# ViTAE-Transformer/LeMeViT

Measured on AMD Instinct MI355X. Metric: images/sec LeMeViT-Base 224^2 bf16 fwd+bwd, higher is better.
Workload: dtype bf16; 1 GPU; lemevit_base 224x224 bf16-autocast train step (fwd+bwd+AdamW), batch 128/GPU, drop_path 0.1, random-init weights; global_batch=128, parallelism=dp1, launch=eager, weight-gradient GEMMs on a side stream

## Files before the change

### include/lemevit_hip.h

```cpp
#ifndef LEMEVIT_HIP_H
#define LEMEVIT_HIP_H

#include <stddef.h>
#include <stdint.h>

#ifdef __cplusplus
extern "C" {
#endif

#define LMV_ABI_VERSION 14

enum { LMV_F32 = 0, LMV_BF16 = 1, LMV_U8 = 2  };
enum {
  LMV_OK = 0,
  LMV_ERR_SHAPE = -1,
  LMV_ERR_DTYPE = -2,
  LMV_ERR_WORKSPACE = -3,
  LMV_ERR_LAUNCH = -4
};

int lmv_abi_version(void);
const char* lmv_last_error(void);
int lmv_config_set(const char* key, int value);
int lmv_config_get(const char* key, int* value);
// ... 5 lines not shown
  const void* w;
  const float* bias;
  const void* res;
  const float* row_scale;
  const void* aux;
  void* out;
  void* out_pre;
  float* bias_grad;
  int64_t rows;
  int32_t rows_per_sample;
  int32_t _pad;
} lmv_linear_problem;

int lmv_linear_fwd(const lmv_linear_problem* p, int nproblems, int N, int K, int act, int dtype, void* stream);
int lmv_linear_dx(const lmv_linear_problem* p, int nproblems, int N, int K, int act, int dtype, void* stream);
size_t lmv_linear_dw_workspace_bytes(const lmv_linear_problem* p, int nproblems, int N, int K, int dtype);
int lmv_linear_dw(const lmv_linear_problem* p, int nproblems, int N, int K, void* workspace, size_t workspace_bytes, int dtype, void* stream);
#define LMV_REDUCE_MAX_SEGS 12
#define LMV_REDUCE_SLABS 0
#define LMV_REDUCE_ROWS  1
typedef struct {
  const float* ws;
  float* out_w;
  float* out_b;
  int64_t slab_stride;
  int64_t nw;
  int32_t nslabs, nb;
  int32_t kind, mode;
} lmv_reduce_seg;
int lmv_linear_dw_partial(const lmv_linear_problem* p, int nproblems, int N, int K, void* workspace, size_t workspace_bytes, int dtype, void* stream,
                          lmv_reduce_seg* segs, int* nsegs);
int lmv_reduce_batch(const lmv_reduce_seg* segs, int nsegs, void* stream);

int lmv_ln_fold(const float* w, const float* bias, const float* gamma, const float* beta, int N, int K, void* wf, float* colsum, float* bf,
                int dtype, void* stream);
int lmv_ln_linear_fwd(const lmv_linear_problem* p, int nproblems, int N, int K, float eps, int act, int dtype, void* stream);
typedef struct {
  const void* x;
  void* out;
  const float* row_scale;
  int64_t rows;
  int32_t rows_per_sample;
  int32_t _pad;
} lmv_mlp_problem;
typedef struct {
  const void* w1f; const float* colsum1; const float* b1f;
  const void* w2; const float* b2;
} lmv_mlp_weights;
int lmv_mlp_fused_supported(int C, int hidden, int dtype);
int lmv_gelu_poly_eval(const float* x, float* y, int64_t n, void* stream);
int lmv_mlp_fused_fwd(const lmv_mlp_problem* p, int nproblems, const lmv_mlp_weights* w, int C, int hidden, float eps, int dtype, void* stream);
typedef struct { const void* g; const void* u; void* dn2; int64_t rows; } lmv_mlp_dx_problem;
int lmv_mlp_dx_fused_supported(int C, int hidden, int dtype);
int lmv_mlp_dx_fused(const lmv_mlp_dx_problem* p, int nproblems, const void* fc2_wt, const void* fc1_wt, int C, int hidden, int dtype, void* stream);
int lmv_attn_out_proj_residual(const lmv_linear_problem* p, int nproblems, int C, int dtype, void* stream);

typedef struct {
  const void* x;
  void* y;
  float* stats;
  const void* dy;
  const void* dres;
  void* dx;
  int64_t rows;
  const float* dx_scale;
  void* dx_scaled;
  int64_t rows_per_sample;
} lmv_ln_segment;

int lmv_layernorm_fwd(const lmv_ln_segment* seg, int nseg, const float* gamma, const float* beta, int C, float eps,
                      int dtype, void* stream);
int lmv_layernorm_gelu_fwd(const lmv_ln_segment* seg, int nseg, const float* gamma, const float* beta, int C, float eps,
                           int dtype, void* stream);
int lmv_layernorm_gelu_bwd(const lmv_ln_segment* seg, int nseg, const float* gamma, const float* beta, float* dgamma, float* dbeta, int C,
                           void* workspace, size_t workspace_bytes, int dtype, void* stream);
size_t lmv_layernorm_bwd_workspace_bytes(int64_t total_rows, int C, int dtype);
int lmv_layernorm_bwd(const lmv_ln_segment* seg, int nseg, const float* gamma, float* dgamma, float* dbeta, int C,
                      void* workspace, size_t workspace_bytes, int dtype, void* stream);
int lmv_layernorm_bwd_partial(const lmv_ln_segment* seg, int nseg, const float* gamma, int C, void* workspace, size_t workspace_bytes,
                              int* partial_rows, int dtype, void* stream);
int lmv_layernorm_bwd_reduce(const void* workspace, int partial_rows, int C, float* dgamma, float* dbeta, void* stream);
int lmv_ln_linear_exact_fwd_supported(int N, int K, int dtype);
int lmv_ln_linear_exact_fwd(const lmv_linear_problem* p, const lmv_ln_segment* seg, int nproblems, int N, int K, const float* gamma, const float* beta,
                            float eps, int dtype, void* stream);
int lmv_linear_res_ln_fwd_supported(int N, int K, int dtype);
int lmv_linear_res_ln_fwd(const lmv_linear_problem* p, const lmv_ln_segment* seg, int nproblems, int N, int K, const float* gamma, const float* beta,
                          float eps, int dtype, void* stream);
int lmv_linear_dx_ln_bwd_supported(int C, int N, int dtype);
size_t lmv_linear_dx_ln_bwd_workspace_bytes(int64_t total_rows, int C);
int lmv_linear_dx_ln_bwd(const lmv_linear_problem* p, const lmv_ln_segment* seg, int nproblems, int C, int N, const float* gamma,
                         void* workspace, size_t workspace_bytes, int* partial_rows, int dtype, void* stream);

size_t lmv_batchnorm_workspace_bytes(int C);
int lmv_batchnorm_train_fwd(const void* x, const float* gamma, const float* beta, float* running_mean, float* running_var, float momentum,
                            float eps, int act, void* y, float* stats, int64_t rows, int C, void* workspace, size_t workspace_bytes,
                            int dtype, void* stream);
int lmv_batchnorm_train_bwd(const void* dy, const void* x, const float* gamma, const float* beta, const float* stats, int act, void* dx,
                            float* dgamma, float* dbeta, int64_t rows, int C, void* workspace, size_t workspace_bytes, int dtype,
                            void* stream);
int lmv_batchnorm_apply_fwd(const void* x, const float* gamma, const float* beta, const float* stats, int act, void* y, int64_t rows, int C,
                            int dtype, void* stream);

int lmv_dwconv3x3_residual_fwd(const void* x, const float* weight, const float* bias, void* y,
                               int B, int H, int W, int C, int dtype, void* stream);
int lmv_dwconv3x3_residual_bwd_data(const void* dy, const float* weight, void* dx,
                                    int B, int H, int W, int C, int dtype, void* stream);
size_t lmv_dwconv3x3_bwd_weight_workspace_bytes(int B, int H, int W, int C, int dtype);
int lmv_dwconv3x3_bwd_weight(const void* dy, const void* x, float* dweight, float* dbias,
                             int B, int H, int W, int C, void* workspace, size_t workspace_bytes, int dtype, void* stream);
int lmv_dwconv3x3_bwd_weight_partial(const void* dy, const void* x, int B, int H, int W, int C, void* workspace, size_t workspace_bytes,
                                     int* partial_rows, int dtype, void* stream);

typedef struct {
  const void* q; const void* k; const void* v;
  void* o;
  float* lse;
  const void* d_o;
  void* dq; void* dk; void* dv;
  int64_t q_bs, q_rs, k_bs, k_rs, v_bs, v_rs, o_bs, o_rs;
  int32_t B, H, Lq, Lk;
  float scale;
  int32_t _pad;
} lmv_attn_desc;

size_t lmv_attn_workspace_bytes(int B, int H, int Lq, int Lk, int backward);
int lmv_attn_fwd(const lmv_attn_desc* d, void* workspace, size_t workspace_bytes, int dtype, void* stream);
int lmv_attn_bwd(const lmv_attn_desc* d, void* workspace, size_t workspace_bytes, int dtype, void* stream);
int lmv_attn_fwd_pair(const lmv_attn_desc* d, void* workspace, size_t workspace_bytes, int dtype, void* stream);
int lmv_attn_bwd_pair(const lmv_attn_desc* d, void* workspace, size_t workspace_bytes, int dtype, void* stream);
int lmv_attn_probs(const lmv_attn_desc* d, float* p, int head_mean, int dtype, void* stream);

int lmv_sa_core_fwd(const void* qkv, void* o, float* lse, int B, int L, int C, void* ws, size_t ws_bytes, int dtype, void* stream);
int lmv_ca_core_fwd(const void* q, const void* kv, void* o, float* lse, int B, int M, int N, int C,
                    void* ws, size_t ws_bytes, int dtype, void* stream);
int lmv_dca_core_fwd(const void* qkv1, const void* qkv2, void* ox, void* oc, float* lse_x, float* lse_c,
                     int B, int N, int M, int C, void* ws, size_t ws_bytes, int dtype, void* stream);

int lmv_cast(const void* src, int src_dtype, void* dst, int dst_dtype, int64_t n, void* stream);
int lmv_im2col3x3s2_c3(const void* x, int x_dtype, void* patches, int dtype, int B, int H, int W, int64_t sb, int64_t sc, int64_t sh,
                       int64_t sw, void* stream);
int lmv_im2col3x3s2_nchw(const void* x, int x_dtype, void* patches, int dtype, int B, int Cin, int H, int W, int KP, int64_t sb, int64_t sc, int64_t sh, int64_t sw,
                         void* stream);
int lmv_conv3x3s2_nchw_dx(const void* dy, const void* wm, void* dx, int dx_dtype, int B, int Cin, int H, int W, int Co, int KP, int64_t sb, int64_t sc, int64_t sh,
                          int64_t sw, int dtype, void* stream);
int lmv_row_scale(const void* x, const float* scale, void* y, int64_t rows, int C, int rows_per_sample, int dtype, void* stream);
typedef struct lmv_row_scale_segment {
  const void* x; const float* scale; void* y;
  int64_t rows; int rows_per_sample;
} lmv_row_scale_segment;
int lmv_row_scale_multi(const lmv_row_scale_segment* seg, int nseg, int C, int dtype, void* stream);
#define LMV_TRANSPOSE_MAX_SEGS 48
typedef struct { const void* src; void* dst; int32_t rows, cols; } lmv_transpose_seg;
int lmv_transpose_batch(const lmv_transpose_seg* segs, int nsegs, int dtype, void* stream);
int lmv_im2col3x3s2_nhwc(const void* x, void* patches, int B, int H, int W, int C, int KP, int dtype, void* stream);
int lmv_col2im3x3s2_nhwc(const void* dpatches, void* dx, int B, int H, int W, int C, int KP, int dtype, void* stream);
int lmv_conv3x3s2_fwd(const void* x, const void* wm, const float* bias, void* y, int B, int H, int W, int Cin, int Cout, int KP, int act, int dtype, void* stream);
size_t lmv_conv3x3s2_dw_workspace_bytes(int B, int H, int W, int Cin, int Cout, int KP, int dtype);
int lmv_conv3x3s2_dw(const void* dy, const void* x, float* dwm, float* dbias, int B, int H, int W, int Cin, int Cout, int KP, void* workspace, size_t workspace_bytes, int dtype,
                     void* stream);
enum { LMV_FOLD_CI_TAP = 0, LMV_FOLD_TAP_CI = 1 };
int lmv_conv_bn_fold(const float* w, const float* b, const float* gamma, const float* beta, const float* mean, const float* var, float eps, int Co, int Cin, int KP,
                     int layout, void* wm, float* bf, float* sc, int dtype, void* stream);
int lmv_conv_bn_fold_bwd(const float* dwm, const float* dbf, const float* w, const float* b, const float* gamma, const float* mean, const float* var, float eps, int Co,
                         int Cin, int KP, int layout, float* dW, float* db, float* dgamma, float* dbeta, void* stream);
int lmv_token_mean2_fwd(const void* x, int L, const void* c, int M, int C, int B, void* out, int dtype, void* stream);
int lmv_token_mean2_bwd(const void* g, void* dx, int L, void* dc, int M, int C, int B, int dtype, void* stream);
int lmv_token_mean2_affine_fwd(const void* x, int L, const void* c, int M, int C, int B, const float* xscale, const float* xshift, void* out, int dtype,
                               void* stream);
int lmv_adamw_flat(float* param, const float* grad, float* exp_avg, float* exp_avg_sq, const float* wd_mask, void* shadow_bf16,
                   int64_t n, float lr, float beta1, float beta2, float eps, float weight_decay, int step, const int* step_dev,
                   void* stream);
typedef struct { const float* ptr; int64_t n; } lmv_norm_seg;
#define LMV_GRAD_STAT_FLOATS 8
#define LMV_NORM_CHUNK 16384
enum { LMV_NORM_SKIP_NONFINITE = 1 };
size_t lmv_grad_norm_workspace_bytes(const lmv_norm_seg* segs, int nsegs);
int lmv_grad_norm(const lmv_norm_seg* segs, int nsegs, float max_norm, int flags, float* stat, int* step_dev, void* ws, size_t ws_bytes,
                  void* stream);
int lmv_adamw_flat_clip(float* param, const float* grad, float* exp_avg, float* exp_avg_sq, const float* wd_mask, void* shadow_bf16,
                        int64_t n, float lr, float beta1, float beta2, float eps, float weight_decay, int step, const int* step_dev,
                        const float* stat, float clip_value, void* stream);
#define LMV_ADAMW_UNIT 8
#define LMV_ADAMW_MAX_GROUPS 256
typedef struct { float lr; float weight_decay; } lmv_adamw_group;
int lmv_adamw_flat_groups(float* param, const float* grad, float* exp_avg, float* exp_avg_sq, void* shadow_bf16, int64_t n,
                          const uint8_t* group_of_unit, const lmv_adamw_group* groups, int ngroups, float beta1, float beta2, float eps, int step,
                          const int* step_dev, const float* stat, float clip_value, void* stream);
int lmv_ema_flat(float* ema, const float* param, int64_t n, float decay, void* stream);

typedef struct lmv_mix_record { float w; int32_t yl, yh, xl, xh; float lam_t; } lmv_mix_record;
int lmv_mix_images(const void* x, int x_dtype, int64_t sb, int64_t sc, int64_t sh, int64_t sw, void* out, int out_dtype, int B, int C, int H, int W,
                   const lmv_mix_record* table, const lmv_mix_record* host_records, const float* scale, const float* shift, void* stream);
int lmv_soft_ce(const void* logits, int dtype, int64_t row_stride, int B, int N, const int64_t* labels, const lmv_mix_record* table, float smoothing,
                const void* target, int target_dtype, int64_t target_stride, float* row_loss, float* mean_loss, void* dlogits, void* stream);

enum { LMV_BLOCK_S = 0, LMV_BLOCK_D = 1, LMV_BLOCK_C = 2 };
enum { LMV_BLOCK_NO_JOIN = 1, LMV_BLOCK_FUSED = 2, LMV_BLOCK_DATA_ONLY = 4 };
typedef struct lmv_block_desc {
  int32_t kind, dtype, B, H, W, M, C, hidden;
  float eps;
  int32_t flags;
  const float* pos_w; const float* pos_b; const float* n1_w; const float* n1_b;
  const void* attn_w[4]; const float* attn_b[4];
  const float* n2_w; const float* n2_b; const void* fc1_w; const float* fc1_b; const void* fc2_w; const float* fc2_b;
  const float* masks[4];
  float* g_pos_w; float* g_pos_b; float* g_n1_w; float* g_n1_b;
  float* g_attn_w[4]; float* g_attn_b[4];
  float* g_n2_w; float* g_n2_b; float* g_fc1_w; float* g_fc1_b; float* g_fc2_w; float* g_fc2_b;
  const void* fold_attn_w[2]; const float* fold_attn_s[2]; const float* fold_attn_b[2];
  const void* fold_fc1_w; const float* fold_fc1_s; const float* fold_fc1_b;
  const void* fc2_wt;
  const void* fc1_wt; const void* attn_wt[2];
} lmv_block_desc;
size_t lmv_block_arena_bytes(const lmv_block_desc* d);
size_t lmv_block_bwd_scratch_bytes(const lmv_block_desc* d);
int lmv_block_fwd(const lmv_block_desc* d, const void* x, const void* c, void* x_out, void* c_out, void* arena, size_t arena_bytes, int save, void* stream);
int lmv_block_fwd_range(const lmv_block_desc* d, const void* x, const void* c, void* x_out, void* c_out, void* arena, size_t arena_bytes, int save,
                        int image0, int nimages, void* stream);
int lmv_block_bwd(const lmv_block_desc* d, const void* x, const void* c, const void* arena, size_t arena_bytes, const void* dx_out, const void* dc_out,
                  void* dx, void* dc, void* scratch, size_t scratch_bytes, void* stream, void* side_stream);
size_t lmv_block_fwd_scratch_bytes(const lmv_block_desc* d);
int lmv_block_fwd_range_scratch(const lmv_block_desc* d, const void* x, const void* c, void* x_out, void* c_out, void* arena, size_t arena_bytes, int save,
                                int image0, int nimages, void* scratch, size_t scratch_bytes, void* stream);
long long lmv_debug_wgrad_launches(void);

typedef struct lmv_sstage_block_params {
  int32_t C, heads, hidden, _pad;
  const void* qkv_w; const void* proj_w; const void* fc1_w; const void* fc2_w;
  const float* n1_w; const float* n1_b; const float* qkv_b; const float* proj_b;
  const float* n2_w; const float* n2_b; const float* fc1_b; const float* fc2_b;
  const float* pos_w; const float* pos_b;
} lmv_sstage_block_params;
typedef struct lmv_sstage_desc {
  int32_t B, H, W, M, C, heads, hidden, nblocks, dtype;
  float eps;
  const void* wpk; const float* vec;
  void* timing; int32_t timing_block, kind;
} lmv_sstage_desc;
int lmv_sstage_supported(int C, int heads, int hidden, int H, int W, int M, int dtype);
size_t lmv_sstage_wpk_bytes(int C, int hidden);
size_t lmv_sstage_vec_floats(int C, int hidden);
size_t lmv_sstage_workspace_bytes(int B, int C);
int lmv_sstage_max_images(int C);
int lmv_sstage_max_concurrent(int C);
int lmv_sstage_pack(const lmv_sstage_block_params* p, void* wpk_out, float* vec_out, void* stream);
int lmv_sstage_fwd(const lmv_sstage_desc* d, const void* x, const void* c, void* x_out, void* c_out, void* workspace, size_t workspace_bytes, void* stream);

typedef struct lmv_dstage_block_params {
  int32_t C, heads, hidden, _pad;
  const void* qkv1_w; const void* qkv2_w; const void* projx_w; const void* projc_w; const void* fc1_w; const void* fc2_w;
  const float* n1_w; const float* n1_b; const float* qkv1_b; const float* qkv2_b; const float* projx_b; const float* projc_b;
  const float* n2_w; const float* n2_b; const float* fc1_b; const float* fc2_b;
  const float* pos_w; const float* pos_b;
} lmv_dstage_block_params;
typedef lmv_sstage_desc lmv_dstage_desc;
int lmv_dstage_supported(int C, int heads, int hidden, int H, int W, int M, int dtype);
size_t lmv_dstage_wpk_bytes(int C, int hidden);
size_t lmv_dstage_vec_floats(int C, int hidden);
size_t lmv_dstage_workspace_bytes(int B, int C);
int lmv_dstage_max_concurrent(int C, int H, int kind);
int lmv_dstage_pack(const lmv_dstage_block_params* p, void* wpk_out, float* vec_out, void* stream);
int lmv_dstage_fwd(const lmv_dstage_desc* d, const void* x, const void* c, void* x_out, void* c_out, void* workspace, size_t workspace_bytes, void* stream);

int lmv_stem_supported(int H, int W, int Cm, int Co, int dtype);
size_t lmv_stem_wpk_bytes(int Cm, int Co);
int lmv_stem_pack(const void* w1m, const void* w2m, int ld2, int Cm, int Co, void* wpk_out, void* stream);
int lmv_stem_fwd(const void* x, int x_dtype, int64_t sb, int64_t sc, int64_t sh, int64_t sw, int B, int H, int W, int Cm, int Co, const void* wpk, const float* b1,
                 const float* b2, void* y, void* stream);
int lmv_stage_error_count(int reset);
int lmv_debug_stage_error_set(int value);

int lmv_debug_launch_timing(int capacity);
int lmv_debug_launch_timing_read(float* ms, double* flops, double* bytes, int* kinds, int capacity);
void lmv_stem_debug_timing(void* buf);

#ifdef __cplusplus
}
#endif
#endif
```

### lemevit_amd/_lib.py

```python
from __future__ import annotations

import ctypes as C
import os

import torch

_HERE = os.path.dirname(os.path.abspath(__file__))
LIB_PATH = os.environ.get("LMV_LIB_PATH") or os.path.join(_HERE, "csrc", "liblemevit_hip.so")

LMV_F32, LMV_BF16, LMV_U8 = 0, 1, 2
ACT_NONE, ACT_GELU, ACT_GELU_GRAD, ACT_GELU_BWD = 0, 1, 2, 3
FOLD_CI_TAP, FOLD_TAP_CI = 0, 1
ABI_VERSION = 14
BLOCK_NO_JOIN, BLOCK_FUSED, BLOCK_DATA_ONLY = 1, 2, 4
GRAD_STAT_FLOATS, NORM_CHUNK, NORM_SKIP_NONFINITE = 8, 16384, 1
ADAMW_UNIT, ADAMW_MAX_GROUPS = 8, 256


class LinearProblem(C.Structure):
    _fields_ = [("a", C.c_void_p), ("w", C.c_void_p), ("bias", C.c_void_p), ("res", C.c_void_p),
                ("row_scale", C.c_void_p), ("aux", C.c_void_p), ("out", C.c_void_p), ("out_pre", C.c_void_p),
                ("bias_grad", C.c_void_p), ("rows", C.c_int64), ("rows_per_sample", C.c_int32), ("_pad", C.c_int32)]


class MlpProblem(C.Structure):
    _fields_ = [("x", C.c_void_p), ("out", C.c_void_p), ("row_scale", C.c_void_p), ("rows", C.c_int64), ("rows_per_sample", C.c_int32), ("_pad", C.c_int32)]


class MlpDxProblem(C.Structure):
    _fields_ = [("g", C.c_void_p), ("u", C.c_void_p), ("dn2", C.c_void_p), ("rows", C.c_int64)]


class MlpWeights(C.Structure):
    _fields_ = [("w1f", C.c_void_p), ("colsum1", C.c_void_p), ("b1f", C.c_void_p), ("w2", C.c_void_p), ("b2", C.c_void_p)]


class ReduceSeg(C.Structure):
    _fields_ = [("ws", C.c_void_p), ("out_w", C.c_void_p), ("out_b", C.c_void_p), ("slab_stride", C.c_int64), ("nw", C.c_int64),
                ("nslabs", C.c_int32), ("nb", C.c_int32), ("kind", C.c_int32), ("mode", C.c_int32)]


class LnSegment(C.Structure):
    _fields_ = [("x", C.c_void_p), ("y", C.c_void_p), ("stats", C.c_void_p), ("dy", C.c_void_p), ("dres", C.c_void_p),
                ("dx", C.c_void_p), ("rows", C.c_int64), ("dx_scale", C.c_void_p), ("dx_scaled", C.c_void_p), ("rows_per_sample", C.c_int64)]


class RowScaleSegment(C.Structure):
    _fields_ = [("x", C.c_void_p), ("scale", C.c_void_p), ("y", C.c_void_p), ("rows", C.c_int64), ("rows_per_sample", C.c_int)]


class AttnDesc(C.Structure):
    _fields_ = [("q", C.c_void_p), ("k", C.c_void_p), ("v", C.c_void_p), ("o", C.c_void_p), ("lse", C.c_void_p),
                ("d_o", C.c_void_p), ("dq", C.c_void_p), ("dk", C.c_void_p), ("dv", C.c_void_p),
                ("q_bs", C.c_int64), ("q_rs", C.c_int64), ("k_bs", C.c_int64), ("k_rs", C.c_int64),
                ("v_bs", C.c_int64), ("v_rs", C.c_int64), ("o_bs", C.c_int64), ("o_rs", C.c_int64),
                ("B", C.c_int32), ("H", C.c_int32), ("Lq", C.c_int32), ("Lk", C.c_int32),
                ("scale", C.c_float), ("_pad", C.c_int32)]


class BlockDesc(C.Structure):
    _fields_ = ([(n, C.c_int32) for n in ("kind", "dtype", "B", "H", "W", "M", "C", "hidden")] + [("eps", C.c_float), ("flags", C.c_int32)] +
                [(n, C.c_void_p) for n in ("pos_w", "pos_b", "n1_w", "n1_b")] + [("attn_w", C.c_void_p * 4), ("attn_b", C.c_void_p * 4)] +
                [(n, C.c_void_p) for n in ("n2_w", "n2_b", "fc1_w", "fc1_b", "fc2_w", "fc2_b")] + [("masks", C.c_void_p * 4)] +
                [(n, C.c_void_p) for n in ("g_pos_w", "g_pos_b", "g_n1_w", "g_n1_b")] + [("g_attn_w", C.c_void_p * 4), ("g_attn_b", C.c_void_p * 4)] +
                [(n, C.c_void_p) for n in ("g_n2_w", "g_n2_b", "g_fc1_w", "g_fc1_b", "g_fc2_w", "g_fc2_b")] +
                [("fold_attn_w", C.c_void_p * 2), ("fold_attn_s", C.c_void_p * 2), ("fold_attn_b", C.c_void_p * 2)] +
                [(n, C.c_void_p) for n in ("fold_fc1_w", "fold_fc1_s", "fold_fc1_b", "fc2_wt", "fc1_wt")] + [("attn_wt", C.c_void_p * 2)])


class SStageBlockParams(C.Structure):
    _fields_ = ([(n, C.c_int32) for n in ("C", "heads", "hidden", "_pad")] +
                [(n, C.c_void_p) for n in ("qkv_w", "proj_w", "fc1_w", "fc2_w", "n1_w", "n1_b", "qkv_b", "proj_b", "n2_w", "n2_b", "fc1_b", "fc2_b", "pos_w", "pos_b")])


class SStageDesc(C.Structure):
    _fields_ = ([(n, C.c_int32) for n in ("B", "H", "W", "M", "C", "heads", "hidden", "nblocks", "dtype")] + [("eps", C.c_float), ("wpk", C.c_void_p), ("vec", C.c_void_p), ("timing", C.c_void_p), ("timing_block", C.c_int32), ("kind", C.c_int32)])


class DStageBlockParams(C.Structure):
    _fields_ = ([(n, C.c_int32) for n in ("C", "heads", "hidden", "_pad")] +
                [(n, C.c_void_p) for n in ("qkv1_w", "qkv2_w", "projx_w", "projc_w", "fc1_w", "fc2_w", "n1_w", "n1_b", "qkv1_b", "qkv2_b", "projx_b", "projc_b",
                                           "n2_w", "n2_b", "fc1_b", "fc2_b", "pos_w", "pos_b")])


class TransposeSeg(C.Structure):
    _fields_ = [("src", C.c_void_p), ("dst", C.c_void_p), ("rows", C.c_int32), ("cols", C.c_int32)]


class NormSeg(C.Structure):
    _fields_ = [("ptr", C.c_void_p), ("n", C.c_int64)]


class AdamWGroup(C.Structure):
    _fields_ = [("lr", C.c_float), ("weight_decay", C.c_float)]


class MixRecord(C.Structure):
    _fields_ = [("w", C.c_float), ("yl", C.c_int32), ("yh", C.c_int32), ("xl", C.c_int32), ("xh", C.c_int32), ("lam_t", C.c_float)]


_P, _I, _L, _F, _Z = C.c_void_p, C.c_int, C.c_int64, C.c_float, C.c_size_t

SIGNATURES = {
    "lmv_abi_version": (_I, []),
    "lmv_config_set": (_I, [C.c_char_p, _I]),
    "lmv_config_get": (_I, [C.c_char_p, C.POINTER(C.c_int)]),
    "lmv_last_error": (C.c_char_p, []),
    "lmv_linear_fwd": (_I, [C.POINTER(LinearProblem), _I, _I, _I, _I, _I, _P]),
    "lmv_linear_dx": (_I, [C.POINTER(LinearProblem), _I, _I, _I, _I, _I, _P]),
    "lmv_linear_dw_workspace_bytes": (_Z, [C.POINTER(LinearProblem), _I, _I, _I, _I]),
    "lmv_linear_dw": (_I, [C.POINTER(LinearProblem), _I, _I, _I, _P, _Z, _I, _P]),
    "lmv_linear_dw_partial": (_I, [C.POINTER(LinearProblem), _I, _I, _I, _P, _Z, _I, _P, C.POINTER(ReduceSeg), C.POINTER(C.c_int)]),
    "lmv_reduce_batch": (_I, [C.POINTER(ReduceSeg), _I, _P]),
    "lmv_ln_fold": (_I, [_P, _P, _P, _P, _I, _I, _P, _P, _P, _I, _P]),
    "lmv_ln_linear_fwd": (_I, [C.POINTER(LinearProblem), _I, _I, _I, _F, _I, _I, _P]),
    "lmv_mlp_fused_supported": (_I, [_I, _I, _I]),
    "lmv_gelu_poly_eval": (_I, [_P, _P, C.c_int64, _P]),
    "lmv_mlp_fused_fwd": (_I, [C.POINTER(MlpProblem), _I, C.POINTER(MlpWeights), _I, _I, _F, _I, _P]),
    "lmv_mlp_dx_fused_supported": (_I, [_I, _I, _I]),
    "lmv_mlp_dx_fused": (_I, [C.POINTER(MlpDxProblem), _I, _P, _P, _I, _I, _I, _P]),
    "lmv_attn_out_proj_residual": (_I, [C.POINTER(LinearProblem), _I, _I, _I, _P]),
    "lmv_layernorm_fwd": (_I, [C.POINTER(LnSegment), _I, _P, _P, _I, _F, _I, _P]),
    "lmv_layernorm_gelu_fwd": (_I, [C.POINTER(LnSegment), _I, _P, _P, _I, _F, _I, _P]),
    "lmv_layernorm_gelu_bwd": (_I, [C.POINTER(LnSegment), _I, _P, _P, _P, _P, _I, _P, _Z, _I, _P]),
    "lmv_layernorm_bwd_workspace_bytes": (_Z, [_L, _I, _I]),
    "lmv_layernorm_bwd": (_I, [C.POINTER(LnSegment), _I, _P, _P, _P, _I, _P, _Z, _I, _P]),
    "lmv_layernorm_bwd_partial": (_I, [C.POINTER(LnSegment), _I, _P, _I, _P, _Z, C.POINTER(C.c_int), _I, _P]),
    "lmv_layernorm_bwd_reduce": (_I, [_P, _I, _I, _P, _P, _P]),
    "lmv_ln_linear_exact_fwd_supported": (_I, [_I, _I, _I]),
    "lmv_ln_linear_exact_fwd": (_I, [C.POINTER(LinearProblem), C.POINTER(LnSegment), _I, _I, _I, _P, _P, _F, _I, _P]),
    "lmv_linear_res_ln_fwd_supported": (_I, [_I, _I, _I]),
    "lmv_linear_res_ln_fwd": (_I, [C.POINTER(LinearProblem), C.POINTER(LnSegment), _I, _I, _I, _P, _P, _F, _I, _P]),
    "lmv_linear_dx_ln_bwd_supported": (_I, [_I, _I, _I]),
    "lmv_linear_dx_ln_bwd_workspace_bytes": (_Z, [_L, _I]),
    "lmv_linear_dx_ln_bwd": (_I, [C.POINTER(LinearProblem), C.POINTER(LnSegment), _I, _I, _I, _P, _P, _Z, C.POINTER(C.c_int), _I, _P]),
    "lmv_batchnorm_workspace_bytes": (_Z, [_I]),
    "lmv_batchnorm_train_fwd": (_I, [_P, _P, _P, _P, _P, _F, _F, _I, _P, _P, _L, _I, _P, _Z, _I, _P]),
    "lmv_batchnorm_train_bwd": (_I, [_P, _P, _P, _P, _P, _I, _P, _P, _P, _L, _I, _P, _Z, _I, _P]),
    "lmv_batchnorm_apply_fwd": (_I, [_P, _P, _P, _P, _I, _P, _L, _I, _I, _P]),
    "lmv_dwconv3x3_residual_fwd": (_I, [_P, _P, _P, _P, _I, _I, _I, _I, _I, _P]),
    "lmv_dwconv3x3_residual_bwd_data": (_I, [_P, _P, _P, _I, _I, _I, _I, _I, _P]),
    "lmv_dwconv3x3_bwd_weight_workspace_bytes": (_Z, [_I, _I, _I, _I, _I]),
    "lmv_dwconv3x3_bwd_weight": (_I, [_P, _P, _P, _P, _I, _I, _I, _I, _P, _Z, _I, _P]),
    "lmv_dwconv3x3_bwd_weight_partial": (_I, [_P, _P, _I, _I, _I, _I, _P, _Z, C.POINTER(C.c_int), _I, _P]),
    "lmv_attn_workspace_bytes": (_Z, [_I, _I, _I, _I, _I]),
    "lmv_attn_fwd": (_I, [C.POINTER(AttnDesc), _P, _Z, _I, _P]),
    "lmv_attn_bwd": (_I, [C.POINTER(AttnDesc), _P, _Z, _I, _P]),
    "lmv_attn_fwd_pair": (_I, [C.POINTER(AttnDesc), _P, _Z, _I, _P]),
    "lmv_attn_bwd_pair": (_I, [C.POINTER(AttnDesc), _P, _Z, _I, _P]),
    "lmv_attn_probs": (_I, [C.POINTER(AttnDesc), _P, _I, _I, _P]),
    "lmv_sa_core_fwd": (_I, [_P, _P, _P, _I, _I, _I, _P, _Z, _I, _P]),
    "lmv_ca_core_fwd": (_I, [_P, _P, _P, _P, _I, _I, _I, _I, _P, _Z, _I, _P]),
    "lmv_dca_core_fwd": (_I, [_P, _P, _P, _P, _P, _P, _I, _I, _I, _I, _P, _Z, _I, _P]),
    "lmv_cast": (_I, [_P, _I, _P, _I, _L, _P]),
    "lmv_im2col3x3s2_c3": (_I, [_P, _I, _P, _I, _I, _I, _I, _L, _L, _L, _L, _P]),
    "lmv_im2col3x3s2_nchw": (_I, [_P, _I, _P, _I, _I, _I, _I, _I, _I, _L, _L, _L, _L, _P]),
    "lmv_conv3x3s2_nchw_dx": (_I, [_P, _P, _P, _I, _I, _I, _I, _I, _I, _I, _L, _L, _L, _L, _I, _P]),
    "lmv_row_scale_multi": (_I, [_P, _I, _I, _I, _P]),
    "lmv_transpose_batch": (_I, [C.POINTER(TransposeSeg), _I, _I, _P]),
    "lmv_row_scale": (_I, [_P, _P, _P, _L, _I, _I, _I, _P]),
    "lmv_im2col3x3s2_nhwc": (_I, [_P, _P, _I, _I, _I, _I, _I, _I, _P]),
    "lmv_conv3x3s2_fwd": (_I, [_P, _P, _P, _P, _I, _I, _I, _I, _I, _I, _I, _I, _P]),
    "lmv_conv3x3s2_dw_workspace_bytes": (_Z, [_I, _I, _I, _I, _I, _I, _I]),
    "lmv_conv3x3s2_dw": (_I, [_P, _P, _P, _P, _I, _I, _I, _I, _I, _I, _P, _Z, _I, _P]),
    "lmv_conv_bn_fold": (_I, [_P, _P, _P, _P, _P, _P, _F, _I, _I, _I, _I, _P, _P, _P, _I, _P]),
    "lmv_conv_bn_fold_bwd": (_I, [_P, _P, _P, _P, _P, _P, _P, _F, _I, _I, _I, _I, _P, _P, _P, _P, _P]),
    "lmv_col2im3x3s2_nhwc": (_I, [_P, _P, _I, _I, _I, _I, _I, _I, _P]),
    "lmv_token_mean2_fwd": (_I, [_P, _I, _P, _I, _I, _I, _P, _I, _P]),
    "lmv_token_mean2_affine_fwd": (_I, [_P, _I, _P, _I, _I, _I, _P, _P, _P, _I, _P]),
    "lmv_token_mean2_bwd": (_I, [_P, _P, _I, _P, _I, _I, _I, _I, _P]),
    "lmv_adamw_flat": (_I, [_P, _P, _P, _P, _P, _P, _L, _F, _F, _F, _F, _F, _I, _P, _P]),
    "lmv_grad_norm_workspace_bytes": (_Z, [C.POINTER(NormSeg), _I]),
    "lmv_grad_norm": (_I, [C.POINTER(NormSeg), _I, _F, _I, _P, _P, _P, _Z, _P]),
    "lmv_adamw_flat_clip": (_I, [_P, _P, _P, _P, _P, _P, _L, _F, _F, _F, _F, _F, _I, _P, _P, _F, _P]),
    "lmv_adamw_flat_groups": (_I, [_P, _P, _P, _P, _P, _L, _P, _P, _I, _F, _F, _F, _I, _P, _P, _F, _P]),
    "lmv_ema_flat": (_I, [_P, _P, _L, _F, _P]),
    "lmv_mix_images": (_I, [_P, _I, _L, _L, _L, _L, _P, _I, _I, _I, _I, _I, _P, _P, _P, _P, _P]),
    "lmv_soft_ce": (_I, [_P, _I, _L, _I, _I, _P, _P, _F, _P, _I, _L, _P, _P, _P, _P]),
    "lmv_block_arena_bytes": (_Z, [C.POINTER(BlockDesc)]),
    "lmv_block_bwd_scratch_bytes": (_Z, [C.POINTER(BlockDesc)]),
    "lmv_block_fwd": (_I, [C.POINTER(BlockDesc), _P, _P, _P, _P, _P, _Z, _I, _P]),
    "lmv_block_fwd_range": (_I, [C.POINTER(BlockDesc), _P, _P, _P, _P, _P, _Z, _I, _I, _I, _P]),
    "lmv_block_bwd": (_I, [C.POINTER(BlockDesc), _P, _P, _P, _Z, _P, _P, _P, _P, _P, _Z, _P, _P]),
    "lmv_block_fwd_scratch_bytes": (_Z, [C.POINTER(BlockDesc)]),
    "lmv_block_fwd_range_scratch": (_I, [C.POINTER(BlockDesc), _P, _P, _P, _P, _P, _Z, _I, _I, _I, _P, _Z, _P]),
    "lmv_debug_wgrad_launches": (C.c_longlong, []),
    "lmv_sstage_supported": (_I, [_I, _I, _I, _I, _I, _I, _I]),
    "lmv_sstage_wpk_bytes": (_Z, [_I, _I]),
    "lmv_sstage_vec_floats": (_Z, [_I, _I]),
    "lmv_sstage_workspace_bytes": (_Z, [_I, _I]),
    "lmv_sstage_max_images": (_I, [_I]),
    "lmv_sstage_max_concurrent": (_I, [_I]),
    "lmv_sstage_pack": (_I, [C.POINTER(SStageBlockParams), _P, _P, _P]),
    "lmv_sstage_fwd": (_I, [C.POINTER(SStageDesc), _P, _P, _P, _P, _P, _Z, _P]),
    "lmv_stem_supported": (_I, [_I, _I, _I, _I, _I]),
    "lmv_stem_wpk_bytes": (_Z, [_I, _I]),
    "lmv_stem_pack": (_I, [_P, _P, _I, _I, _I, _P, _P]),
    "lmv_stem_fwd": (_I, [_P, _I, _L, _L, _L, _L, _I, _I, _I, _I, _I, _P, _P, _P, _P, _P]),
    "lmv_stem_debug_timing": (None, [_P]),
    "lmv_stage_error_count": (_I, [_I]),
    "lmv_debug_stage_error_set": (_I, [_I]),
    "lmv_debug_launch_timing": (_I, [_I]),
    "lmv_debug_launch_timing_read": (_I, [_P, _P, _P, _P, _I]),
    "lmv_dstage_supported": (_I, [_I, _I, _I, _I, _I, _I, _I]),
    "lmv_dstage_wpk_bytes": (_Z, [_I, _I]),
    "lmv_dstage_vec_floats": (_Z, [_I, _I]),
    "lmv_dstage_workspace_bytes": (_Z, [_I, _I]),
    "lmv_dstage_max_concurrent": (_I, [_I, _I, _I]),
    "lmv_dstage_pack": (_I, [C.POINTER(DStageBlockParams), _P, _P, _P]),
    "lmv_dstage_fwd": (_I, [C.POINTER(SStageDesc), _P, _P, _P, _P, _P, _Z, _P]),
}


def _load():
    if not os.path.exists(LIB_PATH):
        raise RuntimeError(
            f"lemevit_amd: HIP kernel library not found at {LIB_PATH}. There is no CPU/PyTorch fallback; "
            "build it with `make -C lemevit_amd/csrc` (hipcc, --offload-arch=gfx950).")
    try:
        lib = C.CDLL(LIB_PATH)
    except OSError as e:
        raise RuntimeError(f"lemevit_amd: cannot load {LIB_PATH}: {e}") from e
    for name, (res, args) in SIGNATURES.items():
        fn = getattr(lib, name)
        fn.restype = res
        fn.argtypes = args
    v = lib.lmv_abi_version()
    if v != ABI_VERSION:
        raise RuntimeError(f"lemevit_amd: ABI version mismatch (library {v}, binding {ABI_VERSION}); rebuild csrc")
    return lib


lib = _load()


def config_set(key: str, value: int) -> None:
    if lib.lmv_config_set(key.encode(), int(value)):
        raise RuntimeError(f"lmv_config_set: {lib.lmv_last_error().decode(errors='replace')}")


def config_get(key: str) -> int:
    v = C.c_int(0)
    if lib.lmv_config_get(key.encode(), C.byref(v)):
        raise RuntimeError(f"lmv_config_get: {lib.lmv_last_error().decode(errors='replace')}")
    return int(v.value)


def check(rc: int, what: str) -> None:
    if rc != 0:
        raise RuntimeError(f"{what} failed (code {rc}): {lib.lmv_last_error().decode(errors='replace')}")
```

### lemevit_amd/csrc/block.hip

```cpp
#include <math.h>
#include <mutex>
#include "common.h"

namespace {

struct Bump {
  unsigned char* base; size_t off, cap;
  void* take(size_t n) {
    const size_t a = (off + 255) & ~(size_t)255;
    off = a + n;
    return base ? (void*)(base + a) : (void*)(uintptr_t)256;
  }
};

struct Dims {
  int kind, dtype, B, H, W, N, M, C, Hd, heads;
  size_t es;
  int64_t rows[2];
};

int dims_of(const lmv_block_desc* d, Dims* o) {
  if (!d) LMV_FAIL(LMV_ERR_SHAPE, "block: null descriptor");
  if (d->kind < LMV_BLOCK_S || d->kind > LMV_BLOCK_C) LMV_FAIL(LMV_ERR_SHAPE, "block: kind %d (0 = S, 1 = D, 2 = C)", d->kind);
  if (d->dtype != LMV_F32 && d->dtype != LMV_BF16) LMV_FAIL(LMV_ERR_DTYPE, "block: unsupported dtype %d", d->dtype);
  if (d->B <= 0 || d->H <= 0 || d->W <= 0 || d->M <= 0 || d->C <= 0 || (d->C % 32)) LMV_FAIL(LMV_ERR_SHAPE, "block: bad dims B=%d H=%d W=%d M=%d C=%d", d->B, d->H, d->W, d->M, d->C);
  o->kind = d->kind; o->dtype = d->dtype; o->B = d->B; o->H = d->H; o->W = d->W; o->N = d->H * d->W; o->M = d->M; o->C = d->C;
  o->Hd = d->hidden > 0 ? d->hidden : 4 * d->C; o->heads = d->C / 32;
  o->es = d->dtype == LMV_BF16 ? 2 : 4;
  o->rows[0] = (int64_t)d->B * o->N; o->rows[1] = (int64_t)d->B * d->M;
  return LMV_OK;
}

inline int proj_w(const Dims& D, int s) { return D.kind == LMV_BLOCK_C ? (s == 0 ? 2 * D.C : D.C) : 3 * D.C; }

struct Fwd {
  void *xp, *n1[2], *pj[2], *ao[2], *t2[2], *n2[2], *u[2], *h[2], *ws;
  float *st1[2], *lse[2], *st2[2];
  size_t ws_bytes;
};

inline size_t fwd_ws_attn(const Dims& D, int b) {
  size_t w, w2 = 0;
  if (D.kind == LMV_BLOCK_C) w = lmv_attn_workspace_bytes(b, D.heads, D.M, D.N, 0);
  else if (D.kind == LMV_BLOCK_D) { w = lmv_attn_workspace_bytes(b, D.heads, D.N, D.M, 0); w2 = lmv_attn_workspace_bytes(b, D.heads, D.M, D.N, 0); }
  else { w = lmv_attn_workspace_bytes(b, D.heads, D.N, D.N, 0); w2 = lmv_attn_workspace_bytes(b, D.heads, D.M, D.M, 0); }
  if (w2 > w) w = w2;
  return w < 256 ? 256 : w;
}
inline size_t fwd_ws_off(const Dims& D, int i0) { return i0 <= 0 ? 0 : fwd_ws_attn(D, i0) + (size_t)512 * i0; }
inline size_t fwd_ws_bytes(const Dims& D, int b) { return fwd_ws_attn(D, b) + (size_t)512 * b + 256; }

inline bool data_only(const lmv_block_desc* d) { return (d->flags & LMV_BLOCK_DATA_ONLY) != 0; }

void layout_transient(const Dims& D, Bump& t, Fwd* f) {
  const bool cb = D.kind == LMV_BLOCK_C;
  for (int s = 0; s < 2; ++s) {
    const bool has = !(cb && s == 0);
    f->n1[s] = t.take(D.rows[s] * D.C * D.es);
    f->n2[s] = has ? t.take(D.rows[s] * D.C * D.es) : nullptr;
    f->h[s] = has ? t.take(D.rows[s] * D.Hd * D.es) : nullptr;
  }
}

void layout_fwd(const Dims& D, Bump& a, Fwd* f, bool dataonly = false, Bump* tr = nullptr) {
  const bool cb = D.kind == LMV_BLOCK_C;
  if (dataonly) {
    for (int s = 0; s < 2; ++s) f->n1[s] = f->n2[s] = f->h[s] = nullptr;
    if (tr) layout_transient(D, *tr, f);
    f->xp = a.take(D.rows[0] * D.C * D.es);
    for (int s = 0; s < 2; ++s) {
      f->st1[s] = (float*)a.take(D.rows[s] * 2 * sizeof(float));
      f->pj[s] = a.take(D.rows[s] * proj_w(D, s) * D.es);
      const bool has = !(cb && s == 0);
      f->ao[s] = has ? a.take(D.rows[s] * D.C * D.es) : nullptr;
      f->lse[s] = has ? (float*)a.take((size_t)D.B * D.heads * (s == 0 ? D.N : D.M) * sizeof(float)) : nullptr;
      f->t2[s] = has ? a.take(D.rows[s] * D.C * D.es) : nullptr;
      f->st2[s] = has ? (float*)a.take(D.rows[s] * 2 * sizeof(float)) : nullptr;
      f->u[s] = has ? a.take(D.rows[s] * D.Hd * D.es) : nullptr;
    }
    f->ws_bytes = fwd_ws_bytes(D, D.B);
    f->ws = a.take(f->ws_bytes);
    return;
  }
  f->xp = a.take(D.rows[0] * D.C * D.es);
  for (int s = 0; s < 2; ++s) {
    f->n1[s] = a.take(D.rows[s] * D.C * D.es);
    f->st1[s] = (float*)a.take(D.rows[s] * 2 * sizeof(float));
    f->pj[s] = a.take(D.rows[s] * proj_w(D, s) * D.es);
    const bool has = !(cb && s == 0);
    f->ao[s] = has ? a.take(D.rows[s] * D.C * D.es) : nullptr;
    f->lse[s] = has ? (float*)a.take((size_t)D.B * D.heads * (s == 0 ? D.N : D.M) * sizeof(float)) : nullptr;
    f->t2[s] = has ? a.take(D.rows[s] * D.C * D.es) : nullptr;
    f->n2[s] = has ? a.take(D.rows[s] * D.C * D.es) : nullptr;
    f->st2[s] = has ? (float*)a.take(D.rows[s] * 2 * sizeof(float)) : nullptr;
    f->u[s] = has ? a.take(D.rows[s] * D.Hd * D.es) : nullptr;
    f->h[s] = has ? a.take(D.rows[s] * D.Hd * D.es) : nullptr;
  }
  f->ws_bytes = fwd_ws_bytes(D, D.B);
  f->ws = a.take(f->ws_bytes);
}

void attn_desc(lmv_attn_desc* a, const Dims& D, const void* q, int qw, int qo, const void* k, int kw, int ko, const void* v, int vw, int vo,
               void* o, float* lse, int Lq, int Lk, float scale) {
  *a = lmv_attn_desc{};
  a->q = (const unsigned char*)q + qo * D.es; a->k = (const unsigned char*)k + ko * D.es; a->v = (const unsigned char*)v + vo * D.es;
  a->o = o; a->lse = lse;
  a->q_bs = (int64_t)Lq * qw; a->q_rs = qw; a->k_bs = (int64_t)Lk * kw; a->k_rs = kw; a->v_bs = (int64_t)Lk * vw; a->v_rs = vw;
  a->o_bs = (int64_t)Lq * D.C; a->o_rs = D.C;
  a->B = D.B; a->H = D.heads; a->Lq = Lq; a->Lk = Lk; a->scale = scale;
}
void attn_grads(lmv_attn_desc* a, const Dims& D, const void* d_o, void* dq, int qo, void* dk, int ko, void* dv, int vo) {
  a->d_o = d_o;
  a->dq = (unsigned char*)dq + qo * D.es; a->dk = (unsigned char*)dk + ko * D.es; a->dv = (unsigned char*)dv + vo * D.es;
}

lmv_linear_problem prob(const void* a, const void* w, void* out, int64_t rows) {
  lmv_linear_problem p{};
  p.a = a; p.w = w; p.out = out; p.rows = rows;
  return p;
}

#define LMV_TRY(expr) do { const int rc__ = (expr); if (rc__) return rc__; } while (0)

const float SDPA_SCALE = 0.17677669529663687f;
inline void dca_scales(const Dims& D, float* sx, float* sc) {
  const double base = pow((double)D.C, -0.5);
  *sx = (float)(log((double)D.M) / log((double)D.N) * base);
  *sc = (float)base;
}

inline bool fused_on(const lmv_block_desc* d, const Dims& D, int save) {
  return (d->flags & LMV_BLOCK_FUSED) && !save && D.dtype == LMV_BF16 && d->fold_fc1_w && d->fold_fc1_s && d->fold_fc1_b && d->fold_attn_w[0] && d->fold_attn_s[0] &&
         d->fold_attn_b[0] && (D.kind == LMV_BLOCK_S || (d->fold_attn_w[1] && d->fold_attn_s[1] && d->fold_attn_b[1]));
}
inline bool fold_qkv(const Dims& D) { return D.C >= 192; }

inline bool mlp_split384(const Dims& D) { const int64_t r = D.rows[0] + D.rows[1]; return D.C == 384 && D.Hd == 1536 && r >= 16384 && r <= 65536; }
inline bool res_ln_ok(const lmv_block_desc* d, const Dims& D, int save) {
  if (D.kind != LMV_BLOCK_S || D.dtype != LMV_BF16 || D.rows[0] + D.rows[1] < 16384 || D.rows[0] + D.rows[1] > 32768) return false;
  if (!lmv_linear_res_ln_fwd_supported(D.C, D.C, D.dtype)) return false;
  return !(fused_on(d, D, save) && !mlp_split384(D));
}

int mlp_fwd(const lmv_block_desc* d, const Dims& D, const Fwd& f, int s0, void* const* outs, const float* const* ds, int save, void* st, bool ln_done = false) {
  const int ns = 2 - s0;
  const bool split384 = mlp_split384(D);
  if (fused_on(d, D, save) && !split384) {
    if (lmv_mlp_fused_supported(D.C, D.Hd, D.dtype)) {
      lmv_mlp_problem q[2] = {};
      for (int i = 0; i < ns; ++i) { const int s = s0 + i; q[i].x = f.t2[s]; q[i].out = outs[s]; q[i].row_scale = ds[s]; q[i].rows = D.rows[s]; q[i].rows_per_sample = s == 0 ? D.N : D.M; }
      lmv_mlp_weights w{d->fold_fc1_w, d->fold_fc1_s, d->fold_fc1_b, d->fc2_w, d->fc2_b};
      return lmv_mlp_fused_fwd(q, ns, &w, D.C, D.Hd, d->eps, D.dtype, st);
    }
    lmv_linear_problem p[2];
    for (int i = 0; i < ns; ++i) { const int s = s0 + i; p[i] = prob(f.t2[s], d->fold_fc1_w, f.h[s], D.rows[s]); p[i].bias = d->fold_fc1_b; p[i].aux = d->fold_fc1_s; }
    LMV_TRY(lmv_ln_linear_fwd(p, ns, D.Hd, D.C, d->eps, LMV_ACT_GELU, D.dtype, st));
    for (int i = 0; i < ns; ++i) {
      const int s = s0 + i;
      p[i] = prob(f.h[s], d->fc2_w, outs[s], D.rows[s]); p[i].bias = d->fc2_b; p[i].res = f.t2[s]; p[i].row_scale = ds[s];
      p[i].rows_per_sample = s == 0 ? D.N : D.M;
    }
    return lmv_linear_fwd(p, ns, D.C, D.Hd, LMV_ACT_NONE, D.dtype, st);
  }
  if (!ln_done) {
    lmv_ln_segment seg[2] = {};
    for (int i = 0; i < ns; ++i) { const int s = s0 + i; seg[i].x = f.t2[s]; seg[i].y = f.n2[s]; seg[i].stats = save ? f.st2[s] : nullptr; seg[i].rows = D.rows[s]; }
    LMV_TRY(lmv_layernorm_fwd(seg, ns, d->n2_w, d->n2_b, D.C, d->eps, D.dtype, st));
  }
  lmv_linear_problem p[2];
  for (int i = 0; i < ns; ++i) { const int s = s0 + i; p[i] = prob(f.n2[s], d->fc1_w, f.h[s], D.rows[s]); p[i].bias = d->fc1_b; p[i].out_pre = save ? f.u[s] : nullptr; }
  LMV_TRY(lmv_linear_fwd(p, ns, D.Hd, D.C, LMV_ACT_GELU, D.dtype, st));
  for (int i = 0; i < ns; ++i) {
    const int s = s0 + i;
    p[i] = prob(f.h[s], d->fc2_w, outs[s], D.rows[s]); p[i].bias = d->fc2_b; p[i].res = f.t2[s]; p[i].row_scale = ds[s];
    p[i].rows_per_sample = s == 0 ? D.N : D.M;
  }
  return lmv_linear_fwd(p, ns, D.C, D.Hd, LMV_ACT_NONE, D.dtype, st);
}

struct Side {
  hipStream_t main, side; hipEvent_t fork, join; bool used;
  void* ws; size_t ws_bytes;
  void* ws_tail; size_t ws_tail_bytes;
  lmv_reduce_seg segs[LMV_REDUCE_MAX_SEGS]; int nsegs = 0;
  bool dataonly = false;
  hipStream_t begin() {
    if (!side) return main;
    lmv_count_wgrad();
    (void)hipEventRecord(fork, main);
    (void)hipStreamWaitEvent(side, fork, 0);
    used = true;
    return side;
  }
  void finish() {
    if (side && used) { (void)hipEventRecord(join, side); (void)hipStreamWaitEvent(main, join, 0); used = false; }
  }
};

struct EventPool {
  std::mutex mu;
  hipEvent_t free_ev[64][32];
  int nfree[64] = {};
  int take(hipEvent_t* fork, hipEvent_t* join) {
    int dev = 0;
    (void)hipGetDevice(&dev);
    dev &= 63;
    hipEvent_t out[2];
    int got = 0;
    {
      std::lock_guard<std::mutex> lk(mu);
      while (got < 2 && nfree[dev] > 0) out[got++] = free_ev[dev][--nfree[dev]];
    }
    for (; got < 2; ++got)
      if (hipEventCreateWithFlags(&out[got], hipEventDisableTiming) != hipSuccess) {
        give(dev, out, got);
        LMV_FAIL(LMV_ERR_LAUNCH, "block_bwd: cannot create stream events");
      }
    *fork = out[0]; *join = out[1];
    return LMV_OK;
  }
  void give(int dev, const hipEvent_t* ev, int n) {
    std::lock_guard<std::mutex> lk(mu);
    for (int i = 0; i < n; ++i) {
      if (nfree[dev] < 32) free_ev[dev][nfree[dev]++] = ev[i];
      else (void)hipEventDestroy(ev[i]);
    }
  }
  void give(hipEvent_t fork, hipEvent_t join) {
    int dev = 0;
    (void)hipGetDevice(&dev);
    const hipEvent_t ev[2] = {fork, join};
    give(dev & 63, ev, 2);
  }
};
EventPool& event_pool() { static EventPool p; return p; }

int dw(Side& sd, const lmv_linear_problem* p, int np, int N, int K, int dtype) {
  lmv_count_wgrad();
  const size_t need = lmv_linear_dw_workspace_bytes(p, np, N, K, dtype);
  if (need > sd.ws_bytes) LMV_FAIL(LMV_ERR_WORKSPACE, "block_bwd: weight-gradient workspace %zu > %zu bytes", need, sd.ws_bytes);
  return lmv_linear_dw(p, np, N, K, sd.ws, sd.ws_bytes, dtype, sd.begin());
}
int flush_reduces(Side& sd) {
  if (!sd.nsegs) return LMV_OK;
  lmv_count_wgrad();
  const int rc = lmv_reduce_batch(sd.segs, sd.nsegs, sd.begin());
  sd.nsegs = 0;
  return rc;
}

struct Bwd {
  void *g[2], *du[2], *dn2[2], *dt2[2], *g2[2], *dao[2], *dpj[2], *dn1[2], *dxp, *ws_main, *ws_side, *ws_conv, *ws_ln[2];
  size_t ws_main_bytes, ws_side_bytes, ws_conv_bytes, ws_ln_bytes;
};

size_t max_dw_ws(const Dims& D) {
  const void* fake = (const void*)(uintptr_t)256;
  size_t m = 256;
  auto one = [&](int np, int64_t r0, int64_t r1, int N, int K, bool shared) {
    lmv_linear_problem p[2];
    float* o0 = (float*)(uintptr_t)256; float* o1 = shared ? o0 : (float*)(uintptr_t)512;
    p[0] = prob(fake, fake, o0, r0); p[0].bias_grad = (float*)(uintptr_t)1024;
    p[1] = prob(fake, fake, o1, r1); p[1].bias_grad = shared ? p[0].bias_grad : (float*)(uintptr_t)2048;
    const size_t w = lmv_linear_dw_workspace_bytes(p, np, N, K, D.dtype);
    if (w > m) m = w;
  };
  const int C = D.C, Hd = D.Hd;
  if (D.kind == LMV_BLOCK_C) {
    one(1, D.rows[1], 0, C, Hd, true); one(1, D.rows[1], 0, Hd, C, true);
    one(1, D.rows[1], 0, C, C, true); one(1, D.rows[1], 0, C, C, true); one(1, D.rows[0], 0, 2 * C, C, true);
  } else {
    const bool sh = D.kind == LMV_BLOCK_S;
    one(2, D.rows[0], D.rows[1], C, Hd, true); one(2, D.rows[0], D.rows[1], Hd, C, true);
    one(2, D.rows[0], D.rows[1], C, C, sh); one(2, D.rows[0], D.rows[1], 3 * C, C, sh);
  }
  return (m + 255) & ~(size_t)255;
}

void layout_bwd(const Dims& D, Bump& a, Bwd* b) {
  const bool cb = D.kind == LMV_BLOCK_C;
  for (int s = 0; s < 2; ++s) {
    const bool has = !(cb && s == 0);
    b->g[s] = has ? a.take(D.rows[s] * D.C * D.es) : nullptr;
    b->du[s] = has ? a.take(D.rows[s] * D.Hd * D.es) : nullptr;
    b->dn2[s] = has ? a.take(D.rows[s] * D.C * D.es) : nullptr;
    b->dt2[s] = has ? a.take(D.rows[s] * D.C * D.es) : nullptr;
    b->g2[s] = has ? a.take(D.rows[s] * D.C * D.es) : nullptr;
    b->dao[s] = has ? a.take(D.rows[s] * D.C * D.es) : nullptr;
    b->dpj[s] = a.take(D.rows[s] * proj_w(D, s) * D.es);
    b->dn1[s] = a.take(D.rows[s] * D.C * D.es);
  }
  b->dxp = a.take(D.rows[0] * D.C * D.es);
  size_t w = lmv_layernorm_bwd_workspace_bytes(D.rows[0] + D.rows[1], D.C, D.dtype);
  size_t w2;
  if (cb) w2 = lmv_attn_workspace_bytes(D.B, D.heads, D.M, D.N, 1);
  else if (D.kind == LMV_BLOCK_D) { w2 = lmv_attn_workspace_bytes(D.B, D.heads, D.N, D.M, 1); const size_t w3 = lmv_attn_workspace_bytes(D.B, D.heads, D.M, D.N, 1); if (w3 > w2) w2 = w3; }
  else { w2 = lmv_attn_workspace_bytes(D.B, D.heads, D.N, D.N, 1); const size_t w3 = lmv_attn_workspace_bytes(D.B, D.heads, D.M, D.M, 1); if (w3 > w2) w2 = w3; }
  if (w2 > w) w = w2;
  if (w < 256) w = 256;
  b->ws_main_bytes = w; b->ws_main = a.take(w);
  b->ws_side_bytes = max_dw_ws(D); b->ws_side = a.take(b->ws_side_bytes);
  b->ws_conv_bytes = lmv_dwconv3x3_bwd_weight_workspace_bytes(D.B, D.H, D.W, D.C, D.dtype); b->ws_conv = a.take(b->ws_conv_bytes);
  b->ws_ln_bytes = lmv_layernorm_bwd_workspace_bytes(D.rows[0] + D.rows[1], D.C, D.dtype);
  { const size_t w2 = lmv_linear_dx_ln_bwd_workspace_bytes(D.rows[0] + D.rows[1], D.C); if (w2 > b->ws_ln_bytes) b->ws_ln_bytes = w2; }
  for (int i = 0; i < 2; ++i) b->ws_ln[i] = a.take(b->ws_ln_bytes);
}

int ln_bwd(Side& sd, const lmv_ln_segment* seg, int nseg, const float* gamma, float* dgamma, float* dbeta, const Dims& D, void* ws, size_t ws_bytes) {
  if (sd.dataonly) return lmv_layernorm_bwd_partial(seg, nseg, gamma, D.C, nullptr, 0, nullptr, D.dtype, sd.main);
  int rows = 0;
  LMV_TRY(lmv_layernorm_bwd_partial(seg, nseg, gamma, D.C, ws, ws_bytes, &rows, D.dtype, sd.main));
  if (sd.nsegs + 1 > LMV_REDUCE_MAX_SEGS) LMV_FAIL(LMV_ERR_WORKSPACE, "block_bwd: too many deferred reductions");
  lmv_reduce_seg& sg = sd.segs[sd.nsegs++];
  sg = lmv_reduce_seg{};
  sg.ws = (const float*)ws; sg.out_w = dgamma; sg.out_b = dbeta; sg.slab_stride = 2 * D.C; sg.nw = D.C; sg.nslabs = rows; sg.nb = D.C;
  sg.kind = LMV_REDUCE_ROWS; sg.mode = 0;
  return LMV_OK;
}

inline bool dx_ln_fused_ok(const Dims& D, const void* wt, int N) {
  const int64_t rows = D.rows[0] + D.rows[1];
  return wt && D.dtype == LMV_BF16 && lmv_linear_dx_ln_bwd_supported(D.C, N, D.dtype) && rows >= 16384 && rows <= 32768;
}
int dx_ln_bwd(Side& sd, const lmv_linear_problem* p, const lmv_ln_segment* seg, int nseg, int N, const float* gamma, float* dgamma, float* dbeta, const Dims& D,
              void* ws, size_t ws_bytes) {
  if (sd.dataonly) return lmv_linear_dx_ln_bwd(p, seg, nseg, D.C, N, gamma, nullptr, 0, nullptr, D.dtype, sd.main);
  int rows = 0;
  LMV_TRY(lmv_linear_dx_ln_bwd(p, seg, nseg, D.C, N, gamma, ws, ws_bytes, &rows, D.dtype, sd.main));
  if (sd.nsegs + 1 > LMV_REDUCE_MAX_SEGS) LMV_FAIL(LMV_ERR_WORKSPACE, "block_bwd: too many deferred reductions");
  lmv_reduce_seg& sg = sd.segs[sd.nsegs++];
  sg = lmv_reduce_seg{};
  sg.ws = (const float*)ws; sg.out_w = dgamma; sg.out_b = dbeta; sg.slab_stride = 2 * D.C; sg.nw = D.C; sg.nslabs = rows; sg.nb = D.C;
  sg.kind = LMV_REDUCE_ROWS; sg.mode = 0;
  return LMV_OK;
}

inline bool mlp_dx_fused_on(const lmv_block_desc* d, const Dims& D) {
  const int mode = lmv_config().mlp_dx_fused;
  if (mode == 0 || D.dtype != LMV_BF16 || !d->fc2_wt || !d->fc1_wt || !lmv_mlp_dx_fused_supported(D.C, D.Hd, D.dtype)) return false;
  return mode == 2;
}

int mlp_bwd(const lmv_block_desc* d, const Dims& D, const Fwd& f, const Bwd& b, int s0, const void* const* douts, const float* const* ds, const float* const* nds,
            const void** g2_out, Side& sd) {
  const int ns = 2 - s0;
  hipStream_t st = sd.main;
  const void* g[2];
  lmv_row_scale_segment rs[2]; int nrs = 0;
  for (int s = s0; s < 2; ++s) {
    g[s] = douts[s];
    if (ds[s]) { rs[nrs].x = douts[s]; rs[nrs].scale = ds[s]; rs[nrs].y = b.g[s]; rs[nrs].rows = D.rows[s]; rs[nrs].rows_per_sample = s == 0 ? D.N : D.M; ++nrs; g[s] = b.g[s]; }
  }
  if (nrs) LMV_TRY(lmv_row_scale_multi(rs, nrs, D.C, D.dtype, st));
  lmv_linear_problem p[2];
  lmv_ln_segment seg[2] = {};
  for (int i = 0; i < ns; ++i) {
    const int s = s0 + i;
    seg[i].x = f.t2[s]; seg[i].dy = b.dn2[s]; seg[i].stats = f.st2[s]; seg[i].dres = douts[s]; seg[i].dx = b.dt2[s]; seg[i].rows = D.rows[s];
    g2_out[s] = b.dt2[s];
    if (nds && nds[s]) { seg[i].dx_scale = nds[s]; seg[i].dx_scaled = b.g2[s]; seg[i].rows_per_sample = s == 0 ? D.N : D.M; g2_out[s] = b.g2[s]; }
  }
  if (sd.dataonly && mlp_dx_fused_on(d, D)) {
    lmv_mlp_dx_problem q[2] = {};
    for (int i = 0; i < ns; ++i) { const int s = s0 + i; q[i].g = g[s]; q[i].u = f.u[s]; q[i].dn2 = b.dn2[s]; q[i].rows = D.rows[s]; }
    LMV_TRY(lmv_mlp_dx_fused(q, ns, d->fc2_wt, d->fc1_wt, D.C, D.Hd, D.dtype, st));
    return ln_bwd(sd, seg, ns, d->n2_w, d->g_n2_w, d->g_n2_b, D, b.ws_ln[0], b.ws_ln_bytes);
  }
  if (!sd.dataonly) {
    for (int i = 0; i < ns; ++i) { const int s = s0 + i; p[i] = prob(g[s], f.h[s], d->g_fc2_w, D.rows[s]); p[i].bias_grad = d->g_fc2_b; }
    LMV_TRY(dw(sd, p, ns, D.C, D.Hd, D.dtype));
  }
  if (d->fc2_wt && D.dtype == LMV_BF16) {
    for (int i = 0; i < ns; ++i) { const int s = s0 + i; p[i] = prob(g[s], d->fc2_wt, b.du[s], D.rows[s]); p[i].aux = f.u[s]; }
    LMV_TRY(lmv_linear_fwd(p, ns, D.Hd, D.C, LMV_ACT_GELU_GRAD, D.dtype, st));
  } else {
    for (int i = 0; i < ns; ++i) { const int s = s0 + i; p[i] = prob(g[s], d->fc2_w, b.du[s], D.rows[s]); p[i].aux = f.u[s]; }
    LMV_TRY(lmv_linear_dx(p, ns, D.C, D.Hd, LMV_ACT_GELU_GRAD, D.dtype, st));
  }
  if (!sd.dataonly) {
    for (int i = 0; i < ns; ++i) { const int s = s0 + i; p[i] = prob(b.du[s], f.n2[s], d->g_fc1_w, D.rows[s]); p[i].bias_grad = d->g_fc1_b; }
    LMV_TRY(dw(sd, p, ns, D.Hd, D.C, D.dtype));
  }
  const bool fuse2 = dx_ln_fused_ok(D, d->fc1_wt, D.Hd);
  if (fuse2) {
  } else if (d->fc1_wt && D.dtype == LMV_BF16) {
    for (int i = 0; i < ns; ++i) { const int s = s0 + i; p[i] = prob(b.du[s], d->fc1_wt, b.dn2[s], D.rows[s]); }
    LMV_TRY(lmv_linear_fwd(p, ns, D.C, D.Hd, LMV_ACT_NONE, D.dtype, st));
  } else {
// ... 49 lines not shown
  Bwd b;
  layout_bwd(D, a, &b);
  return a.off + 256;
}

namespace {
int block_fwd_body(const lmv_block_desc* d, const Dims& D, const Fwd& f, const void* x, const void* c, void* x_out, void* c_out, int save, void* stream);
}

extern "C" int lmv_block_fwd_range(const lmv_block_desc* d, const void* x, const void* c, void* x_out, void* c_out, void* arena, size_t arena_bytes, int save,
                                   int image0, int nimages, void* stream) {
  return lmv_block_fwd_range_scratch(d, x, c, x_out, c_out, arena, arena_bytes, save, image0, nimages, nullptr, 0, stream);
}

extern "C" int lmv_block_fwd_range_scratch(const lmv_block_desc* d, const void* x, const void* c, void* x_out, void* c_out, void* arena, size_t arena_bytes, int save,
                                           int image0, int nimages, void* scratch, size_t scratch_bytes, void* stream) {
  Dims DF;
  LMV_TRY(dims_of(d, &DF));
  LMV_TRY(check_ptrs(d, false));
  const bool cb = DF.kind == LMV_BLOCK_C;
  if (!x || !c || !c_out || (!cb && !x_out) || !arena || !lmv_aligned16(arena)) LMV_FAIL(LMV_ERR_SHAPE, "block_fwd: null / misaligned tensor");
  if (image0 < 0 || nimages <= 0 || image0 + nimages > DF.B) LMV_FAIL(LMV_ERR_SHAPE, "block_fwd: images [%d, %d) outside the batch of %d", image0, image0 + nimages, DF.B);
  const bool dataonly = data_only(d);
  if (dataonly && (!scratch || !lmv_aligned16(scratch))) LMV_FAIL(LMV_ERR_SHAPE, "block_fwd: LMV_BLOCK_DATA_ONLY needs the transient buffer of lmv_block_fwd_range_scratch");
  Bump a{(unsigned char*)arena, 0, arena_bytes};
  Bump t{(unsigned char*)scratch, 0, scratch_bytes};
  Fwd f;
  layout_fwd(DF, a, &f, dataonly, &t);
  if (a.off > arena_bytes) LMV_FAIL(LMV_ERR_WORKSPACE, "block_fwd: arena %zu < %zu bytes", arena_bytes, a.off);
  if (dataonly && t.off > scratch_bytes) LMV_FAIL(LMV_ERR_WORKSPACE, "block_fwd: transient buffer %zu < %zu bytes", scratch_bytes, t.off);
  if (image0 == 0 && nimages == DF.B) return block_fwd_body(d, DF, f, x, c, x_out, c_out, save, stream);
  lmv_block_desc dr = *d;
  dr.B = nimages;
  for (int k = 0; k < 4; ++k) if (dr.masks[k]) dr.masks[k] += image0;
  Dims D;
  LMV_TRY(dims_of(&dr, &D));
  const size_t es = D.es;
  auto adv = [&](void* ptr, int s, size_t width_bytes) -> void* { return ptr ? (void*)((unsigned char*)ptr + (size_t)image0 * (s == 0 ? D.N : D.M) * width_bytes) : nullptr; };
  f.xp = adv(f.xp, 0, D.C * es);
  for (int s = 0; s < 2; ++s) {
    f.n1[s] = adv(f.n1[s], s, D.C * es); f.st1[s] = (float*)adv(f.st1[s], s, 2 * sizeof(float)); f.pj[s] = adv(f.pj[s], s, proj_w(D, s) * es);
    f.ao[s] = adv(f.ao[s], s, D.C * es); f.lse[s] = (float*)adv(f.lse[s], s, D.heads * sizeof(float)); f.t2[s] = adv(f.t2[s], s, D.C * es);
    f.n2[s] = adv(f.n2[s], s, D.C * es); f.st2[s] = (float*)adv(f.st2[s], s, 2 * sizeof(float)); f.u[s] = adv(f.u[s], s, D.Hd * es); f.h[s] = adv(f.h[s], s, D.Hd * es);
  }
  const size_t w0 = fwd_ws_off(DF, image0), w1 = fwd_ws_attn(DF, nimages);
  if (w0 + w1 > f.ws_bytes) LMV_FAIL(LMV_ERR_WORKSPACE, "block_fwd: attention workspace slice [%zu, %zu) outside %zu bytes", w0, w0 + w1, f.ws_bytes);
  f.ws = (unsigned char*)f.ws + w0; f.ws_bytes = w1;
  return block_fwd_body(&dr, D, f, adv(const_cast<void*>(x), 0, D.C * es), adv(const_cast<void*>(c), 1, D.C * es), adv(x_out, 0, D.C * es), adv(c_out, 1, D.C * es), save, stream);
}

extern "C" int lmv_block_fwd(const lmv_block_desc* d, const void* x, const void* c, void* x_out, void* c_out, void* arena, size_t arena_bytes, int save, void* stream) {
  return lmv_block_fwd_range(d, x, c, x_out, c_out, arena, arena_bytes, save, 0, d ? d->B : 0, stream);
}

namespace {

int block_fwd_body(const lmv_block_desc* d, const Dims& D, const Fwd& f, const void* x, const void* c, void* x_out, void* c_out, int save, void* stream) {
  const bool cb = D.kind == LMV_BLOCK_C;
  const int C = D.C, N = D.N, M = D.M;
  LMV_TRY(lmv_dwconv3x3_residual_fwd(x, d->pos_w, d->pos_b, f.xp, D.B, D.H, D.W, C, D.dtype, stream));
  const bool fq = fused_on(d, D, save) && fold_qkv(D);
  const bool ex = !fq && D.dtype == LMV_BF16 && D.kind != LMV_BLOCK_S &&
                  lmv_ln_linear_exact_fwd_supported(cb ? 2 * D.C : 3 * D.C, D.C, D.dtype) && lmv_ln_linear_exact_fwd_supported(D.C, D.C, D.dtype);
  const void* src[2] = {f.xp, c};
  if (!fq && !ex) {
    lmv_ln_segment seg[2] = {};
    seg[0].x = f.xp; seg[0].y = f.n1[0]; seg[0].stats = save ? f.st1[0] : nullptr; seg[0].rows = D.rows[0];
    seg[1].x = c; seg[1].y = f.n1[1]; seg[1].stats = save ? f.st1[1] : nullptr; seg[1].rows = D.rows[1];
    LMV_TRY(lmv_layernorm_fwd(seg, 2, d->n1_w, d->n1_b, C, d->eps, D.dtype, stream));
    src[0] = f.n1[0]; src[1] = f.n1[1];
  }
  auto project = [&](lmv_linear_problem* p, int np, const int* streams, const int* slots, int width) -> int {
    for (int i = 0; i < np; ++i) {
      const int s = streams[i], k = slots[i];
      p[i] = prob(src[s], fq ? d->fold_attn_w[k] : d->attn_w[k], f.pj[s], D.rows[s]);
      p[i].bias = fq ? d->fold_attn_b[k] : d->attn_b[k];
      if (fq) p[i].aux = d->fold_attn_s[k];
    }
    if (ex) {
      lmv_ln_segment seg[2] = {};
      for (int i = 0; i < np; ++i) { const int s = streams[i]; seg[i].y = save ? f.n1[s] : nullptr; seg[i].stats = save ? f.st1[s] : nullptr; seg[i].rows = D.rows[s]; }
      return lmv_ln_linear_exact_fwd(p, seg, np, width, C, d->n1_w, d->n1_b, d->eps, D.dtype, stream);
    }
    return fq ? lmv_ln_linear_fwd(p, np, width, C, d->eps, LMV_ACT_NONE, D.dtype, stream) : lmv_linear_fwd(p, np, width, C, LMV_ACT_NONE, D.dtype, stream);
  };
  lmv_linear_problem p[2];
  lmv_attn_desc ad[2];
  void* outs[2] = {x_out, c_out};
  bool ln2_done = false;
  if (D.kind == LMV_BLOCK_S) {
    { const int st_[2] = {0, 1}, sl_[2] = {0, 0}; LMV_TRY(project(p, 2, st_, sl_, 3 * C)); }
    for (int s = 0; s < 2; ++s) { const int L = s == 0 ? N : M; attn_desc(&ad[s], D, f.pj[s], 3 * C, 0, f.pj[s], 3 * C, C, f.pj[s], 3 * C, 2 * C, f.ao[s], save ? f.lse[s] : nullptr, L, L, SDPA_SCALE); }
    LMV_TRY(lmv_attn_fwd_pair(ad, f.ws, f.ws_bytes, D.dtype, stream));
    for (int s = 0; s < 2; ++s) {
      p[s] = prob(f.ao[s], d->attn_w[1], f.t2[s], D.rows[s]); p[s].bias = d->attn_b[1]; p[s].res = s == 0 ? f.xp : c;
      p[s].row_scale = d->masks[s == 0 ? 0 : 2]; p[s].rows_per_sample = s == 0 ? N : M;
    }
    if (res_ln_ok(d, D, save)) {
      lmv_ln_segment seg[2] = {};
      for (int s = 0; s < 2; ++s) { seg[s].y = f.n2[s]; seg[s].stats = save ? f.st2[s] : nullptr; seg[s].rows = D.rows[s]; }
      LMV_TRY(lmv_linear_res_ln_fwd(p, seg, 2, C, C, d->n2_w, d->n2_b, d->eps, D.dtype, stream));
      ln2_done = true;
    } else {
      LMV_TRY(lmv_linear_fwd(p, 2, C, C, LMV_ACT_NONE, D.dtype, stream));
    }
  } else if (D.kind == LMV_BLOCK_D) {
    float sx, sc;
    dca_scales(D, &sx, &sc);
    { const int st_[2] = {0, 1}, sl_[2] = {0, 1}; LMV_TRY(project(p, 2, st_, sl_, 3 * C)); }
    attn_desc(&ad[0], D, f.pj[0], 3 * C, 0, f.pj[1], 3 * C, C, f.pj[1], 3 * C, 2 * C, f.ao[0], save ? f.lse[0] : nullptr, N, M, sx);
    attn_desc(&ad[1], D, f.pj[1], 3 * C, 0, f.pj[0], 3 * C, C, f.pj[0], 3 * C, 2 * C, f.ao[1], save ? f.lse[1] : nullptr, M, N, sc);
    LMV_TRY(lmv_attn_fwd(&ad[0], f.ws, f.ws_bytes, D.dtype, stream));
    LMV_TRY(lmv_attn_fwd(&ad[1], f.ws, f.ws_bytes, D.dtype, stream));
    for (int s = 0; s < 2; ++s) {
      p[s] = prob(f.ao[s], d->attn_w[2 + s], f.t2[s], D.rows[s]); p[s].bias = d->attn_b[2 + s]; p[s].res = s == 0 ? f.xp : c;
      p[s].row_scale = d->masks[s == 0 ? 0 : 2]; p[s].rows_per_sample = s == 0 ? N : M;
    }
    LMV_TRY(lmv_linear_fwd(p, 2, C, C, LMV_ACT_NONE, D.dtype, stream));
  } else {
    { const int st_[1] = {0}, sl_[1] = {1}; LMV_TRY(project(p, 1, st_, sl_, 2 * C)); }
    { const int st_[1] = {1}, sl_[1] = {0}; LMV_TRY(project(p, 1, st_, sl_, C)); }
    attn_desc(&ad[0], D, f.pj[1], C, 0, f.pj[0], 2 * C, 0, f.pj[0], 2 * C, C, f.ao[1], save ? f.lse[1] : nullptr, M, N, SDPA_SCALE);
    LMV_TRY(lmv_attn_fwd(&ad[0], f.ws, f.ws_bytes, D.dtype, stream));
    p[0] = prob(f.ao[1], d->attn_w[2], f.t2[1], D.rows[1]); p[0].bias = d->attn_b[2]; p[0].res = c; p[0].row_scale = d->masks[0]; p[0].rows_per_sample = M;
    LMV_TRY(lmv_linear_fwd(p, 1, C, C, LMV_ACT_NONE, D.dtype, stream));
  }
  const float* ds[2] = {cb ? nullptr : d->masks[1], cb ? d->masks[1] : d->masks[3]};
  return mlp_fwd(d, D, f, cb ? 1 : 0, outs, ds, save, stream, ln2_done);
}

}

extern "C" int lmv_block_bwd(const lmv_block_desc* d, const void* x, const void* c, const void* arena, size_t arena_bytes, const void* dx_out, const void* dc_out, void* dx, void* dc,
                             void* scratch, size_t scratch_bytes, void* stream, void* side_stream) {
  Dims D;
  LMV_TRY(dims_of(d, &D));
  const bool dataonly = data_only(d);
  LMV_TRY(check_ptrs(d, !dataonly));
  const bool cb = D.kind == LMV_BLOCK_C;
  if (dataonly) side_stream = nullptr;
  if ((!x && !dataonly) || !c || !arena || !dc_out || (!cb && !dx_out) || !dx || !dc || !scratch || !lmv_aligned16(scratch)) LMV_FAIL(LMV_ERR_SHAPE, "block_bwd: null / misaligned tensor");
  Bump a{(unsigned char*)const_cast<void*>(arena), 0, arena_bytes};
  Fwd f;
  layout_fwd(D, a, &f, dataonly);
  if (a.off > arena_bytes) LMV_FAIL(LMV_ERR_WORKSPACE, "block_bwd: arena %zu < %zu bytes", arena_bytes, a.off);
  Bump s{(unsigned char*)scratch, 0, scratch_bytes};
  Bwd b;
  layout_bwd(D, s, &b);
  if (s.off > scratch_bytes) LMV_FAIL(LMV_ERR_WORKSPACE, "block_bwd: scratch %zu < %zu bytes", scratch_bytes, s.off);
  Side sd{};
  sd.main = (hipStream_t)stream; sd.side = (hipStream_t)side_stream; sd.ws = b.ws_side; sd.ws_bytes = b.ws_side_bytes;
  sd.ws_tail = b.ws_conv; sd.ws_tail_bytes = b.ws_conv_bytes;
  sd.dataonly = dataonly;
  if (side_stream) LMV_TRY(event_pool().take(&sd.fork, &sd.join));
  hipStream_t st = sd.main;
  const int C = D.C, N = D.N, M = D.M;
  lmv_linear_problem p[2];
  lmv_attn_desc ad[2];
  const void* g2[2] = {nullptr, nullptr};
  int rc = LMV_OK;
  auto body = [&]() -> int {
    if (cb) {
      const void* douts[2] = {nullptr, dc_out};
      const float* ds[2] = {nullptr, d->masks[1]};
      LMV_TRY(mlp_bwd(d, D, f, b, 1, douts, ds, nullptr, g2, sd));
      const void* dc1 = b.dt2[1];
      const void* g = dc1;
      if (d->masks[0]) { LMV_TRY(lmv_row_scale(dc1, d->masks[0], b.g2[1], D.rows[1], C, M, D.dtype, st)); g = b.g2[1]; }
      if (!dataonly) {
        p[0] = prob(g, f.ao[1], d->g_attn_w[2], D.rows[1]); p[0].bias_grad = d->g_attn_b[2];
        LMV_TRY(dw(sd, p, 1, C, C, D.dtype));
      }
      p[0] = prob(g, d->attn_w[2], b.dao[1], D.rows[1]);
      LMV_TRY(lmv_linear_dx(p, 1, C, C, LMV_ACT_NONE, D.dtype, st));
      attn_desc(&ad[0], D, f.pj[1], C, 0, f.pj[0], 2 * C, 0, f.pj[0], 2 * C, C, f.ao[1], f.lse[1], M, N, SDPA_SCALE);
      attn_grads(&ad[0], D, b.dao[1], b.dpj[1], 0, b.dpj[0], 0, b.dpj[0], C);
      LMV_TRY(lmv_attn_bwd(&ad[0], b.ws_main, b.ws_main_bytes, D.dtype, st));
      if (!dataonly) {
        p[0] = prob(b.dpj[1], f.n1[1], d->g_attn_w[0], D.rows[1]); p[0].bias_grad = d->g_attn_b[0];
        LMV_TRY(dw(sd, p, 1, C, C, D.dtype));
        p[0] = prob(b.dpj[0], f.n1[0], d->g_attn_w[1], D.rows[0]); p[0].bias_grad = d->g_attn_b[1];
        LMV_TRY(dw(sd, p, 1, 2 * C, C, D.dtype));
      }
      p[0] = prob(b.dpj[1], d->attn_w[0], b.dn1[1], D.rows[1]);
      LMV_TRY(lmv_linear_dx(p, 1, C, C, LMV_ACT_NONE, D.dtype, st));
      p[0] = prob(b.dpj[0], d->attn_w[1], b.dn1[0], D.rows[0]);
      LMV_TRY(lmv_linear_dx(p, 1, 2 * C, C, LMV_ACT_NONE, D.dtype, st));
      lmv_ln_segment seg[2] = {};
      seg[0].x = c; seg[0].dy = b.dn1[1]; seg[0].stats = f.st1[1]; seg[0].dres = dc1; seg[0].dx = dc; seg[0].rows = D.rows[1];
      seg[1].x = f.xp; seg[1].dy = b.dn1[0]; seg[1].stats = f.st1[0]; seg[1].dres = nullptr; seg[1].dx = b.dxp; seg[1].rows = D.rows[0];
      LMV_TRY(ln_bwd(sd, seg, 2, d->n1_w, d->g_n1_w, d->g_n1_b, D, b.ws_ln[1], b.ws_ln_bytes));
    } else {
      const void* douts[2] = {dx_out, dc_out};
      const float* ds[2] = {d->masks[1], d->masks[3]};
      const float* nds[2] = {d->masks[0], d->masks[2]};
      LMV_TRY(mlp_bwd(d, D, f, b, 0, douts, ds, nds, g2, sd));
      const bool sh = D.kind == LMV_BLOCK_S;
      if (!dataonly) {
        for (int s2 = 0; s2 < 2; ++s2) { p[s2] = prob(g2[s2], f.ao[s2], sh ? d->g_attn_w[1] : d->g_attn_w[2 + s2], D.rows[s2]); p[s2].bias_grad = sh ? d->g_attn_b[1] : d->g_attn_b[2 + s2]; }
        LMV_TRY(dw(sd, p, 2, C, C, D.dtype));
      }
      if (sh && d->attn_wt[1] && D.dtype == LMV_BF16) {
        for (int s2 = 0; s2 < 2; ++s2) p[s2] = prob(g2[s2], d->attn_wt[1], b.dao[s2], D.rows[s2]);
        LMV_TRY(lmv_linear_fwd(p, 2, C, C, LMV_ACT_NONE, D.dtype, st));
      } else {
        for (int s2 = 0; s2 < 2; ++s2) p[s2] = prob(g2[s2], sh ? d->attn_w[1] : d->attn_w[2 + s2], b.dao[s2], D.rows[s2]);
        LMV_TRY(lmv_linear_dx(p, 2, C, C, LMV_ACT_NONE, D.dtype, st));
      }
      if (sh) {
        for (int s2 = 0; s2 < 2; ++s2) {
          const int L = s2 == 0 ? N : M;
          attn_desc(&ad[s2], D, f.pj[s2], 3 * C, 0, f.pj[s2], 3 * C, C, f.pj[s2], 3 * C, 2 * C, f.ao[s2], f.lse[s2], L, L, SDPA_SCALE);
          attn_grads(&ad[s2], D, b.dao[s2], b.dpj[s2], 0, b.dpj[s2], C, b.dpj[s2], 2 * C);
        }
        LMV_TRY(lmv_attn_bwd_pair(ad, b.ws_main, b.ws_main_bytes, D.dtype, st));
      } else {
        float sx, sc;
        dca_scales(D, &sx, &sc);
        attn_desc(&ad[0], D, f.pj[0], 3 * C, 0, f.pj[1], 3 * C, C, f.pj[1], 3 * C, 2 * C, f.ao[0], f.lse[0], N, M, sx);
        attn_grads(&ad[0], D, b.dao[0], b.dpj[0], 0, b.dpj[1], C, b.dpj[1], 2 * C);
        attn_desc(&ad[1], D, f.pj[1], 3 * C, 0, f.pj[0], 3 * C, C, f.pj[0], 3 * C, 2 * C, f.ao[1], f.lse[1], M, N, sc);
        attn_grads(&ad[1], D, b.dao[1], b.dpj[1], 0, b.dpj[0], C, b.dpj[0], 2 * C);
        LMV_TRY(lmv_attn_bwd(&ad[0], b.ws_main, b.ws_main_bytes, D.dtype, st));
        LMV_TRY(lmv_attn_bwd(&ad[1], b.ws_main, b.ws_main_bytes, D.dtype, st));
      }
      if (!dataonly) {
        for (int s2 = 0; s2 < 2; ++s2) { p[s2] = prob(b.dpj[s2], f.n1[s2], sh ? d->g_attn_w[0] : d->g_attn_w[s2], D.rows[s2]); p[s2].bias_grad = sh ? d->g_attn_b[0] : d->g_attn_b[s2]; }
        LMV_TRY(dw(sd, p, 2, 3 * C, C, D.dtype));
      }
      const bool fuse1 = sh && dx_ln_fused_ok(D, d->attn_wt[0], 3 * C);
      if (fuse1) {
      } else if (sh && d->attn_wt[0] && D.dtype == LMV_BF16) {
        for (int s2 = 0; s2 < 2; ++s2) p[s2] = prob(b.dpj[s2], d->attn_wt[0], b.dn1[s2], D.rows[s2]);
        LMV_TRY(lmv_linear_fwd(p, 2, C, 3 * C, LMV_ACT_NONE, D.dtype, st));
      } else {
        for (int s2 = 0; s2 < 2; ++s2) p[s2] = prob(b.dpj[s2], sh ? d->attn_w[0] : d->attn_w[s2], b.dn1[s2], D.rows[s2]);
        LMV_TRY(lmv_linear_dx(p, 2, 3 * C, C, LMV_ACT_NONE, D.dtype, st));
      }
      lmv_ln_segment seg[2] = {};
      seg[0].x = f.xp; seg[0].dy = b.dn1[0]; seg[0].stats = f.st1[0]; seg[0].dres = b.dt2[0]; seg[0].dx = b.dxp; seg[0].rows = D.rows[0];
      seg[1].x = c; seg[1].dy = b.dn1[1]; seg[1].stats = f.st1[1]; seg[1].dres = b.dt2[1]; seg[1].dx = dc; seg[1].rows = D.rows[1];
      if (fuse1) {
        for (int s2 = 0; s2 < 2; ++s2) p[s2] = prob(b.dpj[s2], d->attn_wt[0], b.dn1[s2], D.rows[s2]);
        LMV_TRY(dx_ln_bwd(sd, p, seg, 2, 3 * C, d->n1_w, d->g_n1_w, d->g_n1_b, D, b.ws_ln[1], b.ws_ln_bytes));
      } else {
        LMV_TRY(ln_bwd(sd, seg, 2, d->n1_w, d->g_n1_w, d->g_n1_b, D, b.ws_ln[1], b.ws_ln_bytes));
      }
    }
    if (!dataonly) {
      void* ws = sd.ws_tail;
      if (sd.nsegs + 1 > LMV_REDUCE_MAX_SEGS) LMV_FAIL(LMV_ERR_WORKSPACE, "block_bwd: too many deferred reductions");
      int rows = 0;
      lmv_count_wgrad();
      LMV_TRY(lmv_dwconv3x3_bwd_weight_partial(b.dxp, x, D.B, D.H, D.W, C, ws, sd.ws_tail_bytes, &rows, D.dtype, sd.begin()));
      lmv_reduce_seg& sg = sd.segs[sd.nsegs++];
      sg = lmv_reduce_seg{};
      sg.ws = (const float*)ws; sg.out_w = d->g_pos_w; sg.out_b = d->g_pos_b; sg.slab_stride = 10 * C; sg.nw = C; sg.nslabs = rows; sg.nb = C;
      sg.kind = LMV_REDUCE_ROWS; sg.mode = 1;
    }
    LMV_TRY(flush_reduces(sd));
    return lmv_dwconv3x3_residual_bwd_data(b.dxp, d->pos_w, dx, D.B, D.H, D.W, C, D.dtype, st);
  };
  rc = body();
  if (rc || !(d->flags & LMV_BLOCK_NO_JOIN)) sd.finish();
  if (side_stream) event_pool().give(sd.fork, sd.join);
  return rc;
}
```

### lemevit_amd/csrc/misc.hip

```cpp
#include <stdarg.h>
#include <string.h>
#include <atomic>
#include <mutex>
#include <vector>
#include "common.h"

static thread_local char g_err[512] = "";

void lmv_set_error(const char* fmt, ...) {
  va_list ap;
  va_start(ap, fmt);
  vsnprintf(g_err, sizeof(g_err), fmt, ap);
  va_end(ap);
}
extern "C" const char* lmv_last_error(void) { return g_err; }

namespace {
struct ErrWord { unsigned* host = nullptr; unsigned* dev = nullptr; };
ErrWord g_errword[64];
std::mutex g_errword_mu;
}
unsigned* lmv_stage_errword(void* stream) {
  int dev = 0;
  (void)hipGetDevice(&dev);
// ... 651 lines not shown
  const float bc1 = 1.f - powf(beta1, t);
  const float bc2_sqrt = sqrtf(1.f - powf(beta2, t));
  hipLaunchKernelGGL(adamw_kernel, dim3(grid_for(n / 4)), dim3(TPB), 0, (hipStream_t)stream, param, grad, exp_avg, exp_avg_sq, wd_mask,
                     reinterpret_cast<bf16_t*>(shadow_bf16), step_dev, n, lr, beta1, beta2, eps, weight_decay, bc1, bc2_sqrt);
  LMV_CHECK_LAUNCH("adamw_flat");
  return LMV_OK;
}

static int64_t grad_norm_chunks(const lmv_norm_seg* segs, int nsegs) {
  if (!segs) LMV_FAIL(-1, "grad_norm: segs is NULL");
  if (nsegs < 1) LMV_FAIL(-1, "grad_norm: nsegs=%d must be >= 1", nsegs);
  int64_t chunks = 0;
  for (int i = 0; i < nsegs; ++i) {
    if (segs[i].n < 0) LMV_FAIL(-1, "grad_norm: segment %d has negative length %lld", i, (long long)segs[i].n);
    if (segs[i].n > 0 && (!segs[i].ptr || ((uintptr_t)segs[i].ptr & 3u))) LMV_FAIL(-1, "grad_norm: segment %d is null or not 4-byte aligned", i);
    chunks += (segs[i].n + LMV_NORM_CHUNK - 1) / LMV_NORM_CHUNK;
  }
  if (chunks >= (int64_t)1 << 31) LMV_FAIL(-1, "grad_norm: too many elements");
  return chunks;
}

extern "C" size_t lmv_grad_norm_workspace_bytes(const lmv_norm_seg* segs, int nsegs) {
  const int64_t chunks = grad_norm_chunks(segs, nsegs);
  return chunks < 0 ? 0 : (size_t)chunks * sizeof(float);
}

extern "C" int lmv_grad_norm(const lmv_norm_seg* segs, int nsegs, float max_norm, int flags, float* stat, int* step_dev, void* ws, size_t ws_bytes,
                             void* stream) {
  const int64_t chunks = grad_norm_chunks(segs, nsegs);
  if (chunks < 0) return LMV_ERR_SHAPE;
  if (!stat || !lmv_aligned16(stat)) LMV_FAIL(LMV_ERR_SHAPE, "grad_norm: stat is null or not 16-byte aligned");
  if (max_norm != max_norm) LMV_FAIL(LMV_ERR_SHAPE, "grad_norm: max_norm is NaN");
  if (ws_bytes < (size_t)chunks * sizeof(float) || (chunks > 0 && (!ws || ((uintptr_t)ws & 3u))))
    LMV_FAIL(LMV_ERR_SHAPE, "grad_norm: workspace of %zu bytes is null, misaligned or shorter than the %zu bytes of lmv_grad_norm_workspace_bytes", ws_bytes,
             (size_t)chunks * sizeof(float));
  hipStream_t st = (hipStream_t)stream;
  float* partial = reinterpret_cast<float*>(ws);
  int64_t part0 = 0;
  for (int s0 = 0; s0 < nsegs; s0 += NORM_MAX_SEGS) {
    NormTable tb{};
    tb.n = nsegs - s0 < NORM_MAX_SEGS ? nsegs - s0 : NORM_MAX_SEGS;
    tb.part0 = (int)part0;
    int64_t c = 0;
    for (int i = 0; i < tb.n; ++i) {
      tb.s[i].p = segs[s0 + i].ptr; tb.s[i].n = segs[s0 + i].n; tb.s[i].chunk0 = c;
      c += (segs[s0 + i].n + LMV_NORM_CHUNK - 1) / LMV_NORM_CHUNK;
    }
    if (c > 0) hipLaunchKernelGGL(grad_norm_partial_kernel, dim3((unsigned)c), dim3(TPB), 0, st, tb, partial);
    part0 += c;
  }
  hipLaunchKernelGGL(grad_norm_final_kernel, dim3(1), dim3(TPB), 0, st, partial, (int)chunks, max_norm, flags, stat, step_dev);
  LMV_CHECK_LAUNCH("grad_norm");
  return LMV_OK;
}

extern "C" int lmv_adamw_flat_clip(float* param, const float* grad, float* exp_avg, float* exp_avg_sq, const float* wd_mask, void* shadow_bf16,
                                   int64_t n, float lr, float beta1, float beta2, float eps, float weight_decay, int step, const int* step_dev,
                                   const float* stat, float clip_value, void* stream) {
  if (n <= 0) return LMV_OK;
  if (n % 4) LMV_FAIL(LMV_ERR_SHAPE, "adamw_flat_clip: n=%lld must be a multiple of 4 (pad the flat buffer)", (long long)n);
  if (!step_dev && step < 1) LMV_FAIL(LMV_ERR_SHAPE, "adamw_flat_clip: step must be >= 1");
  if (!param || !grad || !exp_avg || !exp_avg_sq || !lmv_aligned16(param) || !lmv_aligned16(grad) || !lmv_aligned16(exp_avg) || !lmv_aligned16(exp_avg_sq) ||
      !lmv_aligned16(wd_mask) || ((uintptr_t)shadow_bf16 & 7u) || ((uintptr_t)stat & 3u))
    LMV_FAIL(LMV_ERR_SHAPE, "adamw_flat_clip: null or misaligned buffer");
  if (!(clip_value >= 0.f)) LMV_FAIL(LMV_ERR_SHAPE, "adamw_flat_clip: clip_value must be >= 0 (0: no clamp)");
  const float t = step_dev ? 1.f : (float)step;
  const float bc1 = 1.f - powf(beta1, t);
  const float bc2_sqrt = sqrtf(1.f - powf(beta2, t));
  hipLaunchKernelGGL(adamw_clip_kernel, dim3(grid_for(n / 4)), dim3(TPB), 0, (hipStream_t)stream, param, grad, exp_avg, exp_avg_sq, wd_mask,
                     reinterpret_cast<bf16_t*>(shadow_bf16), step_dev, n, lr, beta1, beta2, eps, weight_decay, bc1, bc2_sqrt, stat, clip_value);
  LMV_CHECK_LAUNCH("adamw_flat_clip");
  return LMV_OK;
}

extern "C" int lmv_adamw_flat_groups(float* param, const float* grad, float* exp_avg, float* exp_avg_sq, void* shadow_bf16, int64_t n,
                                     const uint8_t* group_of_unit, const lmv_adamw_group* groups, int ngroups, float beta1, float beta2, float eps,
                                     int step, const int* step_dev, const float* stat, float clip_value, void* stream) {
  if (n <= 0) return LMV_OK;
  if (n % LMV_ADAMW_UNIT) LMV_FAIL(LMV_ERR_SHAPE, "adamw_flat_groups: n=%lld must be a multiple of %d (one group byte per %d elements)", (long long)n, LMV_ADAMW_UNIT, LMV_ADAMW_UNIT);
  if (ngroups < 1 || ngroups > LMV_ADAMW_MAX_GROUPS) LMV_FAIL(LMV_ERR_SHAPE, "adamw_flat_groups: ngroups=%d must be 1..%d", ngroups, LMV_ADAMW_MAX_GROUPS);
  if (!step_dev && step < 1) LMV_FAIL(LMV_ERR_SHAPE, "adamw_flat_groups: step must be >= 1");
  if (!param || !grad || !exp_avg || !exp_avg_sq || !group_of_unit || !groups || !lmv_aligned16(param) || !lmv_aligned16(grad) || !lmv_aligned16(exp_avg) ||
      !lmv_aligned16(exp_avg_sq) || ((uintptr_t)groups & 7u) || ((uintptr_t)shadow_bf16 & 7u) || ((uintptr_t)stat & 3u) || ((uintptr_t)step_dev & 3u))
    LMV_FAIL(LMV_ERR_SHAPE, "adamw_flat_groups: null or misaligned buffer");
  if (!(clip_value >= 0.f)) LMV_FAIL(LMV_ERR_SHAPE, "adamw_flat_groups: clip_value must be >= 0 (0: no clamp)");
  const float t = step_dev ? 1.f : (float)step;
  const float bc1 = 1.f - powf(beta1, t);
  const float bc2_sqrt = sqrtf(1.f - powf(beta2, t));
  if (stat || clip_value > 0.f)
    hipLaunchKernelGGL(adamw_groups_clip_kernel, dim3(grid_for(n / 4)), dim3(TPB), 0, (hipStream_t)stream, param, grad, exp_avg, exp_avg_sq,
                       reinterpret_cast<bf16_t*>(shadow_bf16), step_dev, n, group_of_unit, groups, ngroups, beta1, beta2, eps, bc1, bc2_sqrt, stat, clip_value);
  else
    hipLaunchKernelGGL(adamw_groups_kernel, dim3(grid_for(n / 4)), dim3(TPB), 0, (hipStream_t)stream, param, grad, exp_avg, exp_avg_sq,
                       reinterpret_cast<bf16_t*>(shadow_bf16), step_dev, n, group_of_unit, groups, ngroups, beta1, beta2, eps, bc1, bc2_sqrt);
  LMV_CHECK_LAUNCH("adamw_flat_groups");
  return LMV_OK;
}

extern "C" int lmv_ema_flat(float* ema, const float* param, int64_t n, float decay, void* stream) {
  if (!ema || !param || n <= 0 || (n % 4) || !lmv_aligned16(ema) || !lmv_aligned16(param)) LMV_FAIL(LMV_ERR_SHAPE, "ema_flat: null / misaligned buffer or n %% 4 != 0");
  if (!(decay >= 0.f && decay <= 1.f)) LMV_FAIL(LMV_ERR_SHAPE, "ema_flat: decay must be in [0, 1]");
  hipLaunchKernelGGL(ema_kernel, dim3(grid_for(n / 4)), dim3(TPB), 0, (hipStream_t)stream, ema, param, n, decay);
  LMV_CHECK_LAUNCH("ema_flat");
  return LMV_OK;
}

namespace {
struct TrSegDev { const unsigned short* src; unsigned short* dst; int rows, cols, tiles_c, tile0; };
struct TrBatch { TrSegDev s[LMV_TRANSPOSE_MAX_SEGS]; int n; };
__global__ __launch_bounds__(256) void transpose16_batch_kernel(const TrBatch tb) {
  __shared__ unsigned short tile[64][66];
  int si = 0;
#pragma unroll 1
  for (int k = 1; k < tb.n; ++k) if ((int)blockIdx.x >= tb.s[k].tile0) si = k;
  const TrSegDev g = tb.s[si];
  const int t = blockIdx.x - g.tile0, tr = t / g.tiles_c, tc = t % g.tiles_c;
  const int r0 = tr * 64, c0 = tc * 64;
  const int tx = threadIdx.x & 63, ty = threadIdx.x >> 6;
#pragma unroll
  for (int i = 0; i < 16; ++i) {
    const int r = r0 + ty * 16 + i, c = c0 + tx;
    tile[ty * 16 + i][tx] = (r < g.rows && c < g.cols) ? g.src[(int64_t)r * g.cols + c] : (unsigned short)0;
  }
  __syncthreads();
#pragma unroll
  for (int i = 0; i < 16; ++i) {
    const int c = c0 + ty * 16 + i, r = r0 + tx;
    if (r < g.rows && c < g.cols) g.dst[(int64_t)c * g.rows + r] = tile[tx][ty * 16 + i];
  }
}
}
extern "C" int lmv_transpose_batch(const lmv_transpose_seg* segs, int nsegs, int dtype, void* stream) {
  if (nsegs <= 0) return LMV_OK;
  if (!segs) LMV_FAIL(LMV_ERR_SHAPE, "transpose_batch: segs is NULL");
  if (dtype != LMV_BF16) LMV_FAIL(LMV_ERR_DTYPE, "transpose_batch: 2-byte elements (bf16) only");
  hipStream_t st = (hipStream_t)stream;
  for (int s0 = 0; s0 < nsegs; s0 += LMV_TRANSPOSE_MAX_SEGS) {
    TrBatch tb{};
    tb.n = nsegs - s0 < LMV_TRANSPOSE_MAX_SEGS ? nsegs - s0 : LMV_TRANSPOSE_MAX_SEGS;
    int tiles = 0;
    for (int i = 0; i < tb.n; ++i) {
      const lmv_transpose_seg& q = segs[s0 + i];
      if (!q.src || !q.dst || q.rows <= 0 || q.cols <= 0 || q.src == q.dst) LMV_FAIL(LMV_ERR_SHAPE, "transpose_batch: bad segment %d", s0 + i);
      TrSegDev& d = tb.s[i];
      d.src = (const unsigned short*)q.src; d.dst = (unsigned short*)q.dst; d.rows = q.rows; d.cols = q.cols;
      d.tiles_c = (q.cols + 63) / 64; d.tile0 = tiles;
      tiles += ((q.rows + 63) / 64) * d.tiles_c;
    }
    hipLaunchKernelGGL(transpose16_batch_kernel, dim3(tiles), dim3(256), 0, st, tb);
  }
  LMV_CHECK_LAUNCH("transpose_batch");
  return LMV_OK;
}
```

### lemevit_amd/model.py

```python
from __future__ import annotations

import math
import operator
import os
import threading
import weakref
from collections import OrderedDict
from typing import Dict, List, Optional, Sequence, Tuple

import torch
import torch.nn as nn
import torch.nn.functional as F

from . import ops
from .blocks import BLOCK_LN_EPS, PARAM_NAMES, attention_state, block_backward, block_forward
from .ops import Prob

Tensor = torch.Tensor


def _cfg(url: str = "", **kwargs) -> dict:
    return dict(url=url, num_classes=1000, input_size=(3, 224, 224), pool_size=None, crop_pct=0.9, interpolation="bicubic",
                fixed_input_size=True, mean=(0.485, 0.456, 0.406), std=(0.229, 0.224, 0.225),
                first_conv="patch_embed.proj", classifier="head", **kwargs)
# ... 244 lines not shown
        conv, bn = ctx.mods
        need_x = ctx.needs_input_grad[0]
        sv = list(ctx.saved_tensors)
        saved = sv.pop(0) if need_p or gelu else None
        Wm, bf = (sv.pop(0), sv.pop(0)) if need_x or gelu else (None, None)
        Co = conv.weight.shape[0]
        g = dy.permute(0, 2, 3, 1).contiguous().view(-1, Co)
        if g.dtype != cd:
            g = g.to(cd)
        if gelu:
            dz = torch.empty_like(g)
            ops.linear_fwd([Prob(saved, Wm, dz, bias=bf, aux=g)], Co, KP, ops.ACT_GELU_BWD)
            g = dz
        grads = [None, None, None, None]
        if need_p:
            dwm = torch.zeros(Co, KP, device=g.device, dtype=torch.float32)
            dbf = torch.zeros(Co, device=g.device, dtype=torch.float32)
            if implicit:
                ops.conv3x3s2_dw(g, saved, dwm, dbf)
            else:
                ops.linear_dw([Prob(g, saved, dwm, bias_grad=dbf)], Co, KP)
            want = [bool(n) for n in ctx.needs_input_grad[1:5]]
            want[1] = want[1] and conv.bias is not None
            grads = list(ops.conv_bn_fold_bwd(dwm, dbf, conv.weight.detach(), None if conv.bias is None else conv.bias.detach(), bn.weight.detach(), bn.running_mean,
                                              bn.running_var, eps, layout, want))
        dx = None
        if need_x and stem1:
            dx = ops.conv3x3s2_nchw_dx(g, Wm, like=sv.pop(0))
        elif need_x:
            dp = torch.empty(g.shape[0], KP, device=g.device, dtype=g.dtype)
            ops.linear_dx([Prob(g, Wm, dp)], Co, KP)
            dx = ops.col2im3x3s2_nhwc(dp, B, H, W, Ci).permute(0, 3, 1, 2).to(xdt)
        return (dx, *grads, None, None, None, None)


class _BNActFn(torch.autograd.Function):

    @staticmethod
    def forward(ctx, x, weight, bias, running_mean, running_var, momentum, eps, gelu):
        y, x2d, stats, g32, b32 = _bn_train_fwd(x, weight, bias, running_mean, running_var, momentum, eps, gelu)
        ctx.save_for_backward(x2d, stats, g32, b32)
        ctx.meta = (gelu, tuple(x.shape), weight.dtype, bias.dtype)
        return y

    @staticmethod
    def backward(ctx, dy):
        return _bn_bwd(ctx, dy) + (None, None, None, None, None)


def _bn_train_fwd(x, weight, bias, running_mean, running_var, momentum, eps, gelu):
    B, C, H, W = x.shape
    x2d = x.detach().permute(0, 2, 3, 1).contiguous().view(B * H * W, C)
    g32, b32 = compute_copy(weight, torch.float32), compute_copy(bias, torch.float32)
    y, stats = ops.batchnorm_train_fwd(x2d, g32, b32, running_mean, running_var, momentum, eps, gelu)
    return y.view(B, H, W, C).permute(0, 3, 1, 2), x2d, stats, g32, b32


def _bn_bwd(ctx, dy):
    x2d, stats, g32, b32 = ctx.saved_tensors
    gelu, (B, C, H, W), wdt, bdt = ctx.meta
    g = dy.permute(0, 2, 3, 1).contiguous().view(B * H * W, C)
    if g.dtype != x2d.dtype:
        g = g.to(x2d.dtype)
    dx, dgamma, dbeta = ops.batchnorm_train_bwd(g, x2d, g32, b32, stats, gelu)
    return dx.view(B, H, W, C).permute(0, 3, 1, 2), dgamma.to(wdt), dbeta.to(bdt)


class _BNApplyFn(torch.autograd.Function):

    @staticmethod
    def forward(ctx, x, weight, bias, stats, gelu):
        B, C, H, W = x.shape
        x2d = x.detach().permute(0, 2, 3, 1).contiguous().view(B * H * W, C)
        g32, b32 = compute_copy(weight, torch.float32), compute_copy(bias, torch.float32)
        y = ops.batchnorm_apply_fwd(x2d, g32, b32, stats, gelu)
        ctx.save_for_backward(x2d, stats, g32, b32)
        ctx.meta = (gelu, (B, C, H, W), weight.dtype, bias.dtype)
        return y.view(B, H, W, C).permute(0, 3, 1, 2)

    @staticmethod
    def backward(ctx, dy):
        return _bn_bwd(ctx, dy) + (None, None)



def _bn_native(m: nn.Module, x: Tensor) -> bool:
    return (isinstance(m, nn.BatchNorm2d) and m.training and m.affine and m.track_running_stats and m.momentum is not None and x.is_cuda
            and x.dim() == 4 and x.dtype in (torch.float32, torch.bfloat16) and x.shape[1] % 8 == 0 and x.shape[1] <= 1024
            and x.shape[0] * x.shape[2] * x.shape[3] > 1 and m.weight.dtype == torch.float32)


def _bn_train(m: nn.BatchNorm2d, x: Tensor, gelu: bool = False, ck: Optional[dict] = None, key: int = 0) -> Tensor:
    if ck is not None and ck["recompute"]:
        return _BNApplyFn.apply(x, m.weight, m.bias, ck["stats"][key], gelu)
    if m.num_batches_tracked is not None:
        m.num_batches_tracked.add_(1)
    if ck is not None:
        y, _, ck["stats"][key], _, _ = _bn_train_fwd(x, m.weight, m.bias, m.running_mean, m.running_var, float(m.momentum), float(m.eps), gelu)
        return y
    return _BNActFn.apply(x, m.weight, m.bias, m.running_mean, m.running_var, float(m.momentum), float(m.eps), gelu)


class _MetaMLPFn(torch.autograd.Function):

    @staticmethod
    def forward(ctx, c, w1, b1, g1, be1, w2, b2, g2, be2, eps1, eps2, cd):
        cin, hid, cout = w1.shape[1], w1.shape[0], w2.shape[0]
        x = c.detach().to(cd).contiguous().view(-1, cin)
        R = x.shape[0]
        W1, W2 = compute_copy(w1, cd), compute_copy(w2, cd)
        f32 = lambda p: compute_copy(p, torch.float32)
        h1 = torch.empty(R, hid, device=x.device, dtype=cd)
        ops.linear_fwd([Prob(x, W1, h1, bias=f32(b1))], hid, cin)
        (a1,), (st1,) = ops.layernorm_fwd_multi([h1], f32(g1), f32(be1), eps1, want_stats=True, gelu=True)
        h2 = torch.empty(R, cout, device=x.device, dtype=cd)
        ops.linear_fwd([Prob(a1, W2, h2, bias=f32(b2))], cout, hid)
        (y,), (st2,) = ops.layernorm_fwd_multi([h2], f32(g2), f32(be2), eps2, want_stats=True)
        ctx.saved = (x, h1, st1, a1, h2, st2, W1, W2, f32(g1), f32(be1), f32(g2))
        ctx.meta = (c.shape, c.dtype, [(p.shape, p.dtype) for p in (w1, b1, g1, be1, w2, b2, g2, be2)])
        return y.view(c.shape[:-1] + (cout,))

    @staticmethod
    def backward(ctx, dy):
        x, h1, st1, a1, h2, st2, W1, W2, g1, be1, g2 = ctx.saved
        cshape, cdtype, pmeta = ctx.meta
        cin, hid, cout = W1.shape[1], W1.shape[0], W2.shape[0]
        dy = dy.contiguous().view(-1, cout)
        if dy.dtype != x.dtype:
            dy = dy.to(x.dtype)
        need = ctx.needs_input_grad[1:9]
        pairs = [any(need[i:i + 2]) for i in (0, 2, 4, 6)]
        sizes = [int(torch.Size(sh).numel()) if pairs[i // 2] else 0 for i, (sh, _) in enumerate(pmeta)]
        pad = [(n + 3) // 4 * 4 for n in sizes]
        flat = torch.zeros(sum(pad), device=x.device, dtype=torch.float32) if any(pairs) else None
        G, off = [], 0
        for (sh, _), n, pd in zip(pmeta, sizes, pad):
            G.append(flat[off:off + n].view(sh) if n else None); off += pd
        dW1, db1, dg1, dbe1, dW2, db2, dg2, dbe2 = G
        (dh2,) = ops.layernorm_bwd_multi([dy], [h2], [st2], g2, dg2, dbe2, [None])
        if pairs[2]:
            ops.linear_dw([Prob(dh2, a1, dW2, bias_grad=db2)], cout, hid)
        da1 = torch.empty_like(a1)
        ops.linear_dx([Prob(dh2, W2, da1)], cout, hid)
        (dh1,) = ops.layernorm_bwd_multi([da1], [h1], [st1], g1, dg1, dbe1, [None], gelu_beta=be1)
        if pairs[0]:
            ops.linear_dw([Prob(dh1, x, dW1, bias_grad=db1)], hid, cin)
        dc = None
        if ctx.needs_input_grad[0]:
            dx = torch.empty_like(x)
            ops.linear_dx([Prob(dh1, W1, dx)], hid, cin)
            dc = dx.view(cshape).to(cdtype)
        ctx.saved = None
        return (dc, *[None if not nd else (g if dt == torch.float32 else g.to(dt)) for g, (_, dt), nd in zip(G, pmeta, need)], None, None, None)


class _TailFn(torch.autograd.Function):

    @staticmethod
    def forward(ctx, x, c, g, b, eps, hw, hb, cd, bn_w=None, bn_b=None, bn_mean=None, bn_var=None, bn_eps=0.0):
        xc = x.detach().to(cd).contiguous()
        cc = c.detach().to(cd).contiguous()
        f32 = lambda p: compute_copy(p, torch.float32)
        (cn,), (st,) = ops.layernorm_fwd_multi([cc], f32(g), f32(b), eps, want_stats=True)
        ctx.bn = None
        if bn_w is not None:
            r = torch.rsqrt(bn_var + bn_eps)
            a = (bn_w.detach() * r).contiguous()
            pooled = ops.token_mean2_affine_fwd(xc, cn, a, (bn_b.detach() - bn_mean * a).contiguous())
            ctx.bn = (xc if (ctx.needs_input_grad[8] or ctx.needs_input_grad[9]) else None, a, r, bn_mean)
        else:
            pooled = ops.token_mean2_fwd(xc, cn)
        ctx.dims = (xc.shape[1], cc.shape[1])
        ctx.meta = (x.dtype, c.dtype, g.dtype, b.dtype, None if hw is None else hw.dtype, None if hb is None else hb.dtype, None if hw is None else hw.shape)
        if hw is None:
            ctx.saved = (cc, st, f32(g), None, None)
            return pooled
        W = compute_copy(hw, cd)
        N, K = W.shape
        Np = (N + 7) // 8 * 8
        if Np != N:
            Wp = torch.zeros((Np, K), device=W.device, dtype=cd); Wp[:N] = W
            bp = None
            if hb is not None:
                bp = torch.zeros((Np,), device=W.device, dtype=torch.float32); bp[:N] = f32(hb)
        else:
            Wp, bp = W, (None if hb is None else f32(hb))
        out = torch.empty((pooled.shape[0], Np), device=pooled.device, dtype=cd)
        ops.linear_fwd([Prob(pooled, Wp, out, bias=bp)], Np, K)
        ctx.saved = (cc, st, f32(g), pooled, Wp)
        return out[:, :N] if Np != N else out

    @staticmethod
    def backward(ctx, dout):
        cc, st, g32, pooled, Wp = ctx.saved
        L, M = ctx.dims
        xdt, cdt, gdt, bdt, hwdt, hbdt, hwshape = ctx.meta
        dW = db = None
        if Wp is not None:
            Np, K = Wp.shape
            N = hwshape[0]
            d = dout.contiguous()
            if d.dtype != pooled.dtype:
                d = d.to(pooled.dtype)
            if Np != N:
                dp = torch.zeros((d.shape[0], Np), device=d.device, dtype=d.dtype); dp[:, :N] = d
                d = dp
            need_w, need_b = ctx.needs_input_grad[5], hbdt is not None and ctx.needs_input_grad[6]
            if need_w or need_b:
                dWf = torch.zeros((Np, K), device=d.device, dtype=torch.float32); dbf = torch.zeros((Np,), device=d.device, dtype=torch.float32)
                ops.linear_dw([Prob(d, pooled, dWf, bias_grad=dbf)], Np, K)
                dW = dWf[:N].to(hwdt) if need_w else None
                db = dbf[:N].to(hbdt) if need_b else None
            dpooled = torch.empty_like(pooled)
            ops.linear_dx([Prob(d, Wp, dpooled)], Np, K)
        else:
            dpooled = dout.contiguous().to(cc.dtype)
        dbn_w = dbn_b = None
        if ctx.bn is not None:
            xc, a, r, mu = ctx.bn
            dp32 = dpooled.float()
            dx, _ = ops.token_mean2_bwd((dp32 * a).to(dpooled.dtype), L, 0)
            _, dcn = ops.token_mean2_bwd(dpooled, 1, M)
            if ctx.needs_input_grad[8]:
                dbn_w = (dp32 * (ops.token_mean2_fwd(xc, None).float() - mu) * r).sum(0)
            if ctx.needs_input_grad[9]:
                dbn_b = dp32.sum(0)
            ctx.bn = None
        else:
            dx, dcn = ops.token_mean2_bwd(dpooled, L, M)
        dg = dbeta = None
        if ctx.needs_input_grad[2] or ctx.needs_input_grad[3]:
            dg = torch.zeros_like(g32); dbeta = torch.zeros_like(g32)
        (dc,) = ops.layernorm_bwd_multi([dcn], [cc], [st], g32, dg, dbeta, [None])
        ctx.saved = None
        dg = dg.to(gdt) if ctx.needs_input_grad[2] else None
        dbeta = dbeta.to(bdt) if ctx.needs_input_grad[3] else None
        return dx.to(xdt), dc.to(cdt), dg, dbeta, None, dW, db, None, dbn_w, dbn_b, None, None, None


def _tail_infer(norm_c: nn.LayerNorm, bn: nn.BatchNorm2d, head: nn.Linear, xt: Tensor, c: Tensor, cd: torch.dtype) -> Tensor:
    def build():
        a = torch.rsqrt(bn.running_var.float() + bn.eps)
        if bn.weight is not None:
            a = a * bn.weight.float()
        b = -bn.running_mean.float() * a
        if bn.bias is not None:
            b = b + bn.bias.float()
        N, K = head.weight.shape
        Np = (N + 7) // 8 * 8
        Wp = torch.zeros((Np, K), device=xt.device, dtype=cd); Wp[:N] = head.weight.detach().to(cd)
        bp = torch.zeros((Np,), device=xt.device, dtype=torch.float32)
        if head.bias is not None:
            bp[:N] = head.bias.detach().float()
        return a.contiguous(), b.contiguous(), norm_c.weight.detach().float().contiguous(), norm_c.bias.detach().float().contiguous(), Wp, bp, N
    src = (bn.weight, bn.bias, bn.running_mean, bn.running_var, norm_c.weight, norm_c.bias, head.weight, head.bias)
    a, b, g32, b32, Wp, bp, N = derived(head, ("tail", cd), src, build)
    cc = c.detach().to(cd).contiguous()
    (cn,), _ = ops.layernorm_fwd_multi([cc], g32, b32, float(norm_c.eps), want_stats=False)
    pooled = ops.token_mean2_affine_fwd(xt.detach().to(cd).contiguous(), cn, a, b)
    Np, K = Wp.shape
    out = torch.empty((pooled.shape[0], Np), device=pooled.device, dtype=cd)
    ops.linear_fwd([Prob(pooled, Wp, out, bias=bp)], Np, K)
    return out[:, :N] if Np != N else out


def _tail_native(norm_c: nn.Module, head: Optional[nn.Module], xt: Tensor, c: Tensor, cd: torch.dtype) -> bool:
    ok = (isinstance(norm_c, nn.LayerNorm) and norm_c.elementwise_affine and norm_c.bias is not None and xt.is_cuda and cd in (torch.float32, torch.bfloat16)
          and xt.shape[-1] % 8 == 0 and norm_c.weight.dtype == torch.float32)
    if head is not None:
        ok = ok and isinstance(head, nn.Linear) and head.in_features % 8 == 0 and head.weight.dtype == torch.float32
    return ok


def _is_meta_mlp(seq: nn.Module, c: Tensor, cd: torch.dtype) -> bool:
    if not (isinstance(seq, nn.Sequential) and len(seq) == 5 and c.is_cuda and cd in (torch.float32, torch.bfloat16)):
        return False
    l1, n1, act, l2, n2 = seq
    return (isinstance(l1, nn.Linear) and isinstance(n1, nn.LayerNorm) and isinstance(act, nn.GELU) and getattr(act, "approximate", "none") == "none"
            and isinstance(l2, nn.Linear) and isinstance(n2, nn.LayerNorm) and l1.bias is not None and l2.bias is not None
            and n1.elementwise_affine and n2.elementwise_affine and n1.bias is not None and n2.bias is not None
            and l1.in_features % 8 == 0 and l1.out_features % 8 == 0 and l2.out_features % 8 == 0 and l1.out_features <= 2048
            and l1.weight.dtype == torch.float32 and c.dtype in (torch.float32, torch.bfloat16))


def _meta_mlp(mlp: nn.Module, c: Tensor, cd: torch.dtype) -> Tensor:
    if _is_meta_mlp(mlp, c, cd):
        l1, n1, _, l2, n2 = mlp
        return _MetaMLPFn.apply(c, l1.weight, l1.bias, n1.weight, n1.bias, l2.weight, l2.bias, n2.weight, n2.bias, n1.eps, n2.eps, cd)
    return mlp(c)


def _is_stem_conv1(m: nn.Module, x: Tensor) -> bool:
    return (isinstance(m, nn.Conv2d) and 1 <= m.in_channels <= 32 and m.in_channels % 8 != 0 and m.kernel_size == (3, 3) and m.stride == (2, 2) and m.padding == (1, 1)
            and m.dilation == (1, 1) and m.groups == 1 and m.out_channels % 8 == 0 and m.padding_mode == "zeros"
            and x.dtype in (torch.float32, torch.bfloat16))


def _conv_bn_sources(conv: nn.Conv2d, bn: nn.BatchNorm2d):
    return conv.weight, conv.bias, bn.weight, bn.bias, bn.running_mean, bn.running_var


def _fold_conv_bn(conv: nn.Conv2d, bn: nn.BatchNorm2d, dtype: torch.dtype):
    s = (bn.running_var.float() + bn.eps).rsqrt()
    if bn.weight is not None:
        s = s * bn.weight.float()
    w = conv.weight.float() * s[:, None, None, None]
# ... 990 lines not shown
        dps = [grads.pop(0) if n else None for n in need_p]
        ctx.mods = ctx.ck = ctx.params = None
        return (None, dx, None, None, *dps)


class LeMeViT(nn.Module):

    def __init__(self, depth=[2, 3, 4, 8, 3], in_chans=3, num_classes=1000, embed_dim=[64, 64, 128, 320, 512], head_dim=64,
                 mlp_ratios=[4, 4, 4, 4, 4], qkv_bias=True, qk_scale=None, drop_rate=0.0, attn_drop=0.0, drop_path_rate=0.0,
                 attn_type=["C", "D", "D", "S", "S"], queries_len=128, qk_dims=None, cpe_ks=3, pre_norm=True, mlp_dwconv=False,
                 representation_size=None, layer_scale_init_value=-1, use_checkpoint_stages=[], dense_blocks=False):
        super().__init__()
        if representation_size:
            raise NotImplementedError("representation_size is unused by every registered variant")
        if head_dim != ops.HEAD_DIM:
            raise NotImplementedError("lemevit_amd kernels are built for head_dim 32 (all registered variants)")
        if queries_len > 16:
            raise NotImplementedError("lemevit_amd kernels are built for <= 16 meta tokens (all registered variants use 16)")
        self.num_classes = num_classes
        self.num_features = self.embed_dim = embed_dim
        qk_dims = qk_dims or embed_dim
        self.num_stages = len(attn_type)
        self.attn_type = list(attn_type)
        self.depth = list(depth)

        self.downsample_layers = nn.ModuleList()
        self.downsample_layers.append(nn.Sequential(
            nn.Conv2d(in_chans, embed_dim[0] // 2, kernel_size=(3, 3), stride=(2, 2), padding=(1, 1)), nn.BatchNorm2d(embed_dim[0] // 2), nn.GELU(),
            nn.Conv2d(embed_dim[0] // 2, embed_dim[0], kernel_size=(3, 3), stride=(2, 2), padding=(1, 1)), nn.BatchNorm2d(embed_dim[0])))
        for i in range(self.num_stages - 1):
            if attn_type[i] == "C":
                self.downsample_layers.append(nn.Identity())
            else:
                self.downsample_layers.append(nn.Sequential(
                    nn.Conv2d(embed_dim[i], embed_dim[i + 1], kernel_size=(3, 3), stride=(2, 2), padding=(1, 1)), nn.BatchNorm2d(embed_dim[i + 1])))

        self.queries_len = queries_len
        self.meta_tokens = nn.Parameter(torch.randn(self.queries_len, embed_dim[0]), requires_grad=True)
        self.meta_token_downsample = nn.ModuleList()
        for i in range(self.num_stages):
            cin = embed_dim[0] if i == 0 else embed_dim[i - 1]
            self.meta_token_downsample.append(nn.Sequential(
                nn.Linear(cin, cin * 4), nn.LayerNorm(cin * 4), nn.GELU(), nn.Linear(cin * 4, embed_dim[i]), nn.LayerNorm(embed_dim[i])))

        self.stages = nn.ModuleList()
        nheads = [dim // head_dim for dim in qk_dims]
        dp_rates = [x.item() for x in torch.linspace(0, drop_path_rate, sum(depth))]
        cur = 0
        for i in range(self.num_stages):
            self.stages.append(nn.ModuleList([
                LeMeBlock(dim=embed_dim[i], attn_drop=attn_drop, proj_drop=drop_rate, drop_path=dp_rates[cur + j], attn_type=attn_type[i],
                          layer_scale_init_value=layer_scale_init_value, num_heads=nheads[i], qk_dim=qk_dims[i], mlp_ratio=mlp_ratios[i],
                          mlp_dwconv=mlp_dwconv, cpe_ks=cpe_ks, pre_norm=pre_norm, dense=dense_blocks) for j in range(depth[i])]))
            cur += depth[i]

        self.norm = nn.BatchNorm2d(embed_dim[-1])
        self.norm_c = nn.LayerNorm(embed_dim[-1])
        self.pre_logits = nn.Identity()
        self.head = nn.Linear(embed_dim[-1], num_classes) if num_classes > 0 else nn.Identity()
        self.apply(self._init_weights)
        self.default_cfg = _cfg()
        self._set_checkpoint_stages(use_checkpoint_stages)

    def _set_checkpoint_stages(self, stages) -> None:
        idx = []
        for i in stages:
            try:
                j = None if isinstance(i, bool) else operator.index(i)
            except TypeError:
                j = None
            if j is None or not 0 <= j < self.num_stages:
                raise ValueError(f"use_checkpoint_stages: {i!r} is not a stage index in range({self.num_stages})")
            idx.append(j)
        self.use_checkpoint_stages = sorted(set(idx))
        self.grad_checkpointing = bool(idx)
        for i, stage in enumerate(self.stages):
            for blk in stage:
                blk.grad_checkpointing = i in idx

    @torch.jit.ignore
    def set_grad_checkpointing(self, enable: bool = True) -> None:
        self._set_checkpoint_stages(range(self.num_stages) if enable else [])

    def _init_weights(self, m):
        if isinstance(m, nn.Linear):
            nn.init.trunc_normal_(m.weight, mean=0.0, std=0.02, a=-2.0, b=2.0)
            if m.bias is not None:
                nn.init.constant_(m.bias, 0)
        elif isinstance(m, nn.LayerNorm):
            nn.init.constant_(m.bias, 0)
            nn.init.constant_(m.weight, 1.0)

    @torch.jit.ignore
    def no_weight_decay(self):
        return {"pos_embed", "cls_token"}

    def get_classifier(self):
        return self.head

    def reset_classifier(self, num_classes, global_pool=""):
        self.num_classes = num_classes
        self.head = nn.Linear(self.embed_dim[-1], num_classes) if num_classes > 0 else nn.Identity()

    @staticmethod
    def _to_tokens(x: Tensor, dtype) -> Tuple[Tensor, int, int]:
        B, C, H, W = x.shape
        return x.permute(0, 2, 3, 1).reshape(B, H * W, C).to(dtype).contiguous(), H, W

    @staticmethod
    def _to_nchw(xt: Tensor, H: int, W: int) -> Tensor:
        B, N, C = xt.shape
        return xt.view(B, H, W, C).permute(0, 3, 1, 2)

    def _run_downsample(self, seq: nn.Module, x: Tensor) -> Tensor:
        if not isinstance(seq, nn.Sequential):
            return seq(x)
        cd = x.dtype if not torch.is_autocast_enabled() else torch.get_autocast_dtype("cuda")
        fold = not (self.training or torch.is_grad_enabled())
        mods = list(seq)
        if fold and _stem_applies(mods, x, cd):
            return _stem_fused(mods, x, cd)
        if getattr(self, "grad_checkpointing", False) and torch.is_grad_enabled():
            params = [p for m in mods for p in m.parameters(recurse=False)]
            if x.requires_grad or any(p.requires_grad for p in params):
                return _CkptDownsampleFn.apply(mods, x, cd, torch.is_autocast_enabled(), *params)
        return _downsample_mods(mods, x, cd, fold)

    def _draw_drop_path(self, B: int, device) -> Dict[int, List[Optional[Tensor]]]:
        if not self.training:
            return {}
        plan = [(blk, 2 if blk.kind in ("C", "Sx") else 4) for st in self.stages for blk in st if blk.drop_prob > 0.0 and type(blk)._masks is LeMeBlock._masks
                and "_masks" not in blk.__dict__]
        if not plan:
            return {}
        probs = [1.0 - blk.drop_prob for blk, n in plan for _ in range(n)]
        ent = self.__dict__.get("_dp_keep")
        if ent is None or ent[0] != probs or ent[1].device != torch.device(device):
            ent = self._dp_keep = (probs, torch.tensor(probs, dtype=torch.float32, device=device))
        keep = ent[1]
        u = torch.rand((keep.shape[0], B), device=device, dtype=torch.float32)
        scale = (u < keep[:, None]).to(torch.float32) / keep[:, None]
        out, r = {}, 0
        for blk, n in plan:
            out[id(blk)] = [scale[r + q] for q in range(n)] + [None] * (4 - n)
            r += n
        return out

    def forward_features(self, x: Tensor, c: Optional[Tensor] = None, head=False) -> Tensor:
        cd = _resolve_dtype(x)
        self._tail_done = False
        B = x.shape[0]
        if torch.is_grad_enabled():
            new_training_pass()
        hoist = c is None
        if hoist:
            c = self.meta_tokens.unsqueeze(0)
        infer = not (self.training or torch.is_grad_enabled())
        mapping = _map_pass.rec is not None
        st = {"cd": cd, "masks": self._draw_drop_path(B, x.device), "head": head, "checked": False, "infer": infer,
              "side": infer and _INFER_SIDE and launches.concurrent == 1 and x.is_cuda and not mapping,
              "tail_parts": _INFER_TAIL_PARTS if (infer and launches.concurrent == 1 and x.is_cuda and B >= 32 and not mapping) else 1,
              "key": (tuple(x.shape[1:]), cd), "whole": [False] * self.num_stages}
        out = self._stages_from(0, x, None, 0, 0, c, hoist, st)
        if infer and launches.concurrent == 1 and not mapping:
            self.__dict__.setdefault("_whole_seen", {})[st["key"]] = tuple(st["whole"])
        return out

    def _meta_tokens_for(self, i: int, c: Tensor, hoist: bool, B: int, cd: torch.dtype) -> Tensor:
        mlp = self.meta_token_downsample[i]
        if hoist and not torch.is_grad_enabled() and not self.training:
            c = derived(self, ("meta0", cd), [self.meta_tokens, *mlp.parameters()], lambda: _meta_mlp(mlp, c, cd).detach())
        else:
            c = _meta_mlp(mlp, c, cd)
        if hoist:
            c = c.expand(B, -1, -1)
        return c.to(cd).contiguous()

    def _stages_from(self, i0: int, x: Optional[Tensor], xt: Optional[Tensor], H: int, W: int, c: Tensor, hoist: bool, st: dict) -> Tensor:
        cd, head = st["cd"], st["head"]
        B = x.shape[0] if xt is None else xt.shape[0]
        for i in range(i0, self.num_stages):
            down = i == 0 or not isinstance(self.downsample_layers[i], nn.Identity)
            if st["tail_parts"] > 1 and i > i0 and xt is not None:
                seen = self.__dict__.get("_whole_seen", {}).get(st["key"])
                if seen is not None and seen[i - 1] and not any(seen[i:]):
                    return self._tail_split(i, xt, H, W, c, st)
            cur = torch.cuda.current_stream(c.device) if st["side"] else None
            if st["side"] and down and i > 0 and not hoist:
                from .blocks import aux_streams
                side = aux_streams(c.device, 1)[0]
                side.wait_stream(cur)
                with torch.cuda.stream(side):
                    c_in, c = c, self._meta_tokens_for(i, c, False, B, cd)
                    c_in.record_stream(side)
                x = self._run_downsample(self.downsample_layers[i], self._to_nchw(xt, H, W))
                xt, H, W = self._to_tokens(x, cd)
                cur.wait_stream(side)
                c.record_stream(cur)
            else:
                if down:
                    x = self._run_downsample(self.downsample_layers[i], x if xt is None else self._to_nchw(xt, H, W))
                    xt, H, W = self._to_tokens(x, cd)
                c = self._meta_tokens_for(i, c, hoist, B, cd)
            hoist = False
            whole = _sstage_applies(self.stages[i], xt, c, H, W)
            if whole is not None:
                st["whole"][i] = True
                if not st["checked"]:
                    ops.check_stage_errors("found by LeMeViT.forward_features; raised by an earlier call", sync=False)
                    st["checked"] = True
                xt, c = _whole_stage_fwd(whole, xt.contiguous(), c, _sstage_packed(self.stages[i], whole), H, W)
                continue
            all_masks = st["masks"]
            with image_ranges(xt.device, B):
                for blk in self.stages[i]:
                    xt, c = blk.forward_tokens(xt, c, H, W, masks=all_masks.get(id(blk)) if all_masks else None)
        return self._tail(xt, H, W, c, st)

    def _tail_split(self, i: int, xt: Tensor, H: int, W: int, c: Tensor, st: dict) -> Tensor:
        from .blocks import aux_streams
        parts = max(1, min(st["tail_parts"], xt.shape[0]))
        cur = torch.cuda.current_stream(xt.device)
        xs, cs = xt.chunk(parts), c.chunk(parts)
        streams = aux_streams(xt.device, len(xs) - 1)
        sub = dict(st, tail_parts=1, side=False)
        fork = cur.record_event()
        fills = cache_fills()
        ys = [self._stages_from(i, None, xs[0].contiguous(), H, W, cs[0].contiguous(), False, sub)]
        cold = cache_fills() != fills
        for k, s in enumerate(streams):
            if cold:
                s.wait_stream(cur)
            else:
                s.wait_event(fork)
            with torch.cuda.stream(s):
                ys.append(self._stages_from(i, None, xs[k + 1].contiguous(), H, W, cs[k + 1].contiguous(), False, sub))
            xt.record_stream(s); c.record_stream(s)
        for s, y in zip(streams, ys[1:]):
            cur.wait_stream(s)
            y.record_stream(cur)
        return torch.cat(ys)

    def _tail(self, xt: Tensor, H: int, W: int, c: Tensor, st: dict) -> Tensor:
        cd, head = st["cd"], st["head"]
        B = xt.shape[0]
        bn = self.norm
        if head is not False and isinstance(self.pre_logits, nn.Identity) and (self.training or torch.is_grad_enabled()) and _tail_native(self.norm_c, head, xt, c, cd):
            hw, hb = (None, None) if head is None else (head.weight, head.bias)
            if _bn_frozen(bn) and bn.num_features == xt.shape[-1]:
                self._tail_done = head is not None
                return _TailFn.apply(xt, c, self.norm_c.weight, self.norm_c.bias, float(self.norm_c.eps), hw, hb, cd, bn.weight, bn.bias, bn.running_mean, bn.running_var,
                                     float(bn.eps))
            xn = self._to_nchw(xt, H, W)
            xn = _bn_train(bn, xn) if _bn_native(bn, xn) else bn(xn)
            xb = xn.permute(0, 2, 3, 1).reshape(B, H * W, -1)
            self._tail_done = head is not None
            return _TailFn.apply(xb, c, self.norm_c.weight, self.norm_c.bias, float(self.norm_c.eps), hw, hb, cd)
        if (head is not False and head is not None and not bn.training and bn.track_running_stats and isinstance(self.pre_logits, nn.Identity)
                and not torch.is_grad_enabled() and _tail_native(self.norm_c, head, xt, c, cd) and bn.running_var is not None):
            self._tail_done = True
            return _tail_infer(self.norm_c, bn, head, xt, c, cd)
        cn = self.pre_logits(self.norm_c(c))
        if not bn.training and bn.track_running_stats and isinstance(self.pre_logits, nn.Identity):
            pooled = xt.float().mean(dim=1)
            scale = bn.weight.float() * torch.rsqrt(bn.running_var.float() + bn.eps) if bn.affine else torch.rsqrt(bn.running_var.float() + bn.eps)
            xm = (pooled - bn.running_mean.float()) * scale + (bn.bias.float() if bn.affine else 0.0)
            return xm.to(cn.dtype) + cn.mean(dim=1)
        xn = self._to_nchw(xt, H, W)
        xn = _bn_train(bn, xn) if _bn_native(bn, xn) else bn(xn)
        xn = self.pre_logits(xn)
        return xn.flatten(2).mean(-1) + cn.mean(dim=1)

    def _map_plan(self, img_shape, blocks=None, heads: str = "mean", image_queries=None):
        if heads not in ("mean", "all"):
            raise ValueError(f"attention_maps: heads must be 'mean' or 'all', got {heads!r}")
        if len(img_shape) != 4:
            raise ValueError(f"attention_maps: the image must be [B, C, H, W], got shape {tuple(img_shape)}")
        names = OrderedDict((f"stages.{i}.{j}", (i, blk)) for i, stage in enumerate(self.stages) for j, blk in enumerate(stage))
        if blocks is None:
            want = set(names)
        else:
            want = set([blocks] if isinstance(blocks, str) else blocks)
            unknown = sorted(n for n in want if n not in names)
            if unknown:
                raise ValueError(f"attention_maps: unknown block name(s) {unknown}; blocks are named 'stages.<stage>.<block>', e.g. {list(names)[:3]}")
        B, _, H, W = (int(v) for v in img_shape)
        grids = []
        for i in range(self.num_stages):
            if i == 0:
                H, W = ((H + 1) // 2 + 1) // 2, ((W + 1) // 2 + 1) // 2
            elif not isinstance(self.downsample_layers[i], nn.Identity):
                H, W = (H + 1) // 2, (W + 1) // 2
            grids.append((H, W))
        plan, total = [], 0
        for name, (i, blk) in names.items():
            if name not in want:
                continue
            h, w = grids[i]
            shapes = map_shapes(blk.kind, B, None if heads == "mean" else blk.attn.num_heads, self.queries_len, h, w, map_query_rows(image_queries, h, w))
            total += 4 * sum(math.prod(s) for s in shapes.values())
            plan.append((name, blk, (h, w), shapes))
        return plan, total

    def attention_maps(self, img: Tensor, blocks=None, heads: str = "mean", image_queries=None, max_bytes: int = 1 << 30):
        plan, total = self._map_plan(tuple(img.shape), blocks, heads, image_queries)
        if total > max_bytes:
            raise ValueError(f"attention_maps: the requested maps take {total} bytes (max_bytes = {max_bytes}); pass blocks= to select blocks or image_queries= "
                             "a short list of query positions instead of 'all', or raise max_bytes")
        rec = _MapRecorder(plan, heads == "mean")
        rec.queries = image_queries
        training = [m for m in self.modules() if m.training]
        prev = _map_pass.rec
        try:
            for m in training:
                m.training = False
            _map_pass.rec = rec
            with torch.no_grad():
                out = self(img)
        finally:
            _map_pass.rec = prev
            for m in training:
                m.training = True
        return out, rec.maps

    def forward(self, x: Tensor) -> Tensor:
        head = self.head if isinstance(self.head, nn.Linear) else None
        x = self.forward_features(x, None, head=head)
        return x if self._tail_done else self.head(x)


class LayerNorm2d(nn.LayerNorm):

    def forward(self, x: Tensor) -> Tensor:
        return F.layer_norm(x.permute(0, 2, 3, 1), self.normalized_shape, self.weight, self.bias, self.eps).permute(0, 3, 1, 2)


class LeMeViTBackbone(LeMeViT):

    def __init__(self, depth=[2, 3, 4, 8, 3], in_chans=3, num_classes=1000, embed_dim=[64, 64, 128, 320, 512], head_dim=64,
                 mlp_ratios=[4, 4, 4, 4, 4], qkv_bias=True, qk_scale=None, drop_rate=0.0, attn_drop=0.0, drop_path_rate=0.0,
                 attn_type=["C", "D", "D", "S", "S"], queries_len=128, qk_dims=None, cpe_ks=3, pre_norm=True, mlp_dwconv=False,
                 representation_size=None, layer_scale_init_value=-1, use_checkpoint_stages=[], frozen_stages=[-1], pretrained=None):
        super().__init__(depth=depth, in_chans=in_chans, num_classes=0, embed_dim=embed_dim, head_dim=head_dim, mlp_ratios=mlp_ratios,
                         qkv_bias=qkv_bias, qk_scale=qk_scale, drop_rate=drop_rate, attn_drop=attn_drop, drop_path_rate=drop_path_rate,
                         attn_type=attn_type, queries_len=queries_len, qk_dims=qk_dims, cpe_ks=cpe_ks, pre_norm=pre_norm, mlp_dwconv=mlp_dwconv,
                         representation_size=representation_size, layer_scale_init_value=layer_scale_init_value,
                         use_checkpoint_stages=use_checkpoint_stages, dense_blocks=True)
        self.num_classes = num_classes
        self.frozen_stages = list(frozen_stages)
        self.extra_norms = nn.ModuleList([LayerNorm2d(embed_dim[i + 1]) for i in range(self.num_stages - 1)])
        del self.head
# ... 45 lines not shown
```

### lemevit_amd/ops.py

```python
from __future__ import annotations

import ctypes as C
import math
from typing import List, Optional, Sequence, Tuple

import torch

from . import _lib
from ._lib import ACT_GELU, ACT_GELU_BWD, ACT_GELU_GRAD, ACT_NONE, FOLD_CI_TAP, FOLD_TAP_CI, AttnDesc, LinearProblem, LnSegment, check, lib

Tensor = torch.Tensor
HEAD_DIM = 32


def dtype_code(t: Tensor) -> int:
    if t.dtype == torch.float32:
        return _lib.LMV_F32
    if t.dtype == torch.bfloat16:
        return _lib.LMV_BF16
    raise TypeError(f"lemevit_amd: unsupported dtype {t.dtype} (float32 and bfloat16 only)")


_raw_stream = getattr(torch._C, "_cuda_getCurrentRawStream", None)

# ... 417 lines not shown
def cast(src: Tensor, dtype: torch.dtype) -> Tensor:
    dst = torch.empty(src.shape, device=src.device, dtype=dtype)
    check(lib.lmv_cast(_ptr(src), dtype_code(src), _ptr(dst), dtype_code(dst), src.numel(), _stream()), "lmv_cast")
    return dst


def im2col3x3s2_c3(x: Tensor, dtype: torch.dtype) -> Tensor:
    B, C, H, W = x.shape
    if C != 3:
        raise ValueError("im2col3x3s2_c3: 3 input channels expected")
    out = torch.empty(B * ((H + 1) // 2) * ((W + 1) // 2), 32, device=x.device, dtype=dtype)
    sb, sc, sh, sw = x.stride()
    if not x.is_cuda:
        raise RuntimeError("lemevit_amd: tensors must be on the GPU (no CPU fallback exists)")
    check(lib.lmv_im2col3x3s2_c3(x.data_ptr(), dtype_code(x), _ptr(out), dtype_code(out), B, H, W, sb, sc, sh, sw, _stream()), "lmv_im2col3x3s2_c3")
    return out


def im2col3x3s2_nchw(x: Tensor, dtype: torch.dtype, KP: Optional[int] = None) -> Tensor:
    B, C_, H, W = x.shape
    KP = (9 * C_ + 31) // 32 * 32 if KP is None else KP
    if not x.is_cuda:
        raise RuntimeError("lemevit_amd: tensors must be on the GPU (no CPU fallback exists)")
    out = torch.empty(B * ((H + 1) // 2) * ((W + 1) // 2), KP, device=x.device, dtype=dtype)
    sb, sc, sh, sw = x.stride()
    check(lib.lmv_im2col3x3s2_nchw(x.data_ptr(), dtype_code(x), _ptr(out), dtype_code(out), B, C_, H, W, KP, sb, sc, sh, sw, _stream()), "lmv_im2col3x3s2_nchw")
    return out


def conv3x3s2_nchw_dx(dy: Tensor, wm: Tensor, like: Tensor) -> Tensor:
    B, C_, H, W = like.shape
    Co, KP = wm.shape
    if dy.dtype != wm.dtype or dy.shape != (B * ((H + 1) // 2) * ((W + 1) // 2), Co):
        raise ValueError(f"conv3x3s2_nchw_dx: dy {tuple(dy.shape)} {dy.dtype} does not match wm {tuple(wm.shape)} {wm.dtype} and the image {tuple(like.shape)}")
    dx = torch.empty_like(like, memory_format=torch.preserve_format)
    sb, sc, sh, sw = dx.stride()
    check(lib.lmv_conv3x3s2_nchw_dx(_ptr(dy), _ptr(wm), dx.data_ptr(), dtype_code(dx), B, C_, H, W, Co, KP, sb, sc, sh, sw, dtype_code(dy), _stream()), "lmv_conv3x3s2_nchw_dx")
    return dx


def im2col3x3s2_nhwc(x: Tensor, KP: int) -> Tensor:
    B, H, W, C_ = x.shape
    out = torch.empty(B * ((H + 1) // 2) * ((W + 1) // 2), KP, device=x.device, dtype=x.dtype)
    check(lib.lmv_im2col3x3s2_nhwc(_ptr(x), _ptr(out), B, H, W, C_, KP, dtype_code(x), _stream()), "lmv_im2col3x3s2_nhwc")
    return out


def conv3x3s2_implicit_ok(x: Tensor, Cout: int, KP: int) -> bool:
    B, H, W, C_ = x.shape
    Ho, Wo = (H + 1) // 2, (W + 1) // 2
    rows = B * Ho * Wo
    return (x.is_cuda and x.dtype == torch.bfloat16 and x.is_contiguous() and x.data_ptr() % 16 == 0 and min(B, H, W, C_, Cout) > 0 and C_ % 8 == 0 and Cout % 8 == 0
            and KP % 64 == 0 and KP >= 9 * C_ and rows % 64 == 0 and rows < (1 << 22) and KP < (1 << 13) and Ho * Wo < (1 << 19) and x.numel() < (1 << 31))


def conv3x3s2_fwd(x: Tensor, wm: Tensor, bias: Optional[Tensor], act: int = ACT_NONE) -> Tensor:
    B, H, W, C_ = x.shape
    Co, KP = wm.shape
    y = torch.empty(B * ((H + 1) // 2) * ((W + 1) // 2), Co, device=x.device, dtype=x.dtype)
    check(lib.lmv_conv3x3s2_fwd(_ptr(x), _ptr(wm), None if bias is None else _f32(bias), _ptr(y), B, H, W, C_, Co, KP, act, dtype_code(x), _stream()), "lmv_conv3x3s2_fwd")
    return y


def conv3x3s2_dw(dy: Tensor, x: Tensor, dwm: Tensor, dbias: Optional[Tensor]) -> None:
    B, H, W, C_ = x.shape
    Co, KP = dwm.shape
    st = _stream()
    ws = _workspace(lib.lmv_conv3x3s2_dw_workspace_bytes(B, H, W, C_, Co, KP, dtype_code(x)), x.device, st)
    check(lib.lmv_conv3x3s2_dw(_ptr(dy), _ptr(x), _f32(dwm), None if dbias is None else _f32(dbias), B, H, W, C_, Co, KP, ws.data_ptr(), ws.numel(), dtype_code(x), st), "lmv_conv3x3s2_dw")


def conv_bn_fold(weight: Tensor, bias: Optional[Tensor], gamma: Tensor, beta: Tensor, mean: Tensor, var: Tensor, eps: float, dtype: torch.dtype, KP: int,
                 layout: int) -> Tuple[Tensor, Tensor, Tensor]:
    Co, Cin = weight.shape[0], weight.shape[1]
    if weight.dtype != torch.float32 or tuple(weight.shape[2:]) != (3, 3):
        raise TypeError("conv_bn_fold: takes the fp32 master weight [Co, Cin, 3, 3]")
    wm = torch.empty((Co, KP), device=weight.device, dtype=dtype)
    bf = torch.empty(Co, device=weight.device, dtype=torch.float32)
    s = torch.empty(Co, device=weight.device, dtype=torch.float32)
    check(lib.lmv_conv_bn_fold(_f32(weight), _f32(bias), _f32(gamma), _f32(beta), _f32(mean), _f32(var), eps, Co, Cin, KP, layout, _ptr(wm), _ptr(bf), _ptr(s),
                               dtype_code(wm), _stream()), "lmv_conv_bn_fold")
    return wm, bf, s


def conv_bn_fold_bwd(dwm: Tensor, dbf: Tensor, weight: Tensor, bias: Optional[Tensor], gamma: Tensor, mean: Tensor, var: Tensor, eps: float, layout: int,
                     want: Sequence[bool] = (True, True, True, True)):
    Co, Cin = weight.shape[0], weight.shape[1]
    if dwm.shape[0] != Co or dbf.numel() != Co:
        raise ValueError(f"conv_bn_fold_bwd: dwm {tuple(dwm.shape)} / dbf {tuple(dbf.shape)} do not match the weight {tuple(weight.shape)}")
    new = lambda w, shape: torch.empty(shape, device=weight.device, dtype=torch.float32) if w else None
    dW, db, dg, dbe = new(want[0], weight.shape), new(want[1], (Co,)), new(want[2], (Co,)), new(want[3], (Co,))
    check(lib.lmv_conv_bn_fold_bwd(_f32(dwm), _f32(dbf), _f32(weight), _f32(bias), _f32(gamma), _f32(mean), _f32(var), eps, Co, Cin, dwm.shape[1], layout,
                                   _ptr(dW), _ptr(db), _ptr(dg), _ptr(dbe), _stream()), "lmv_conv_bn_fold_bwd")
    return dW, db, dg, dbe


def col2im3x3s2_nhwc(dpatches: Tensor, B: int, H: int, W: int, C_: int) -> Tensor:
    dx = torch.empty((B, H, W, C_), device=dpatches.device, dtype=dpatches.dtype)
    check(lib.lmv_col2im3x3s2_nhwc(_ptr(dpatches), _ptr(dx), B, H, W, C_, dpatches.shape[1], dtype_code(dpatches), _stream()), "lmv_col2im3x3s2_nhwc")
    return dx


def token_mean2_fwd(x: Tensor, c: Optional[Tensor]) -> Tensor:
    B, L, C_ = x.shape
    out = torch.empty((B, C_), device=x.device, dtype=x.dtype)
    check(lib.lmv_token_mean2_fwd(_ptr(x), L, _ptr(c), 0 if c is None else c.shape[1], C_, B, _ptr(out), dtype_code(x), _stream()), "lmv_token_mean2_fwd")
    return out


def token_mean2_affine_fwd(x: Tensor, c: Optional[Tensor], xscale: Tensor, xshift: Tensor) -> Tensor:
    B, L, C_ = x.shape
    if xscale.dtype != torch.float32 or xshift.dtype != torch.float32 or xscale.numel() != C_ or xshift.numel() != C_:
        raise TypeError("token_mean2_affine_fwd: xscale / xshift must be float32 [C]")
    out = torch.empty((B, C_), device=x.device, dtype=x.dtype)
    check(lib.lmv_token_mean2_affine_fwd(_ptr(x), L, _ptr(c), 0 if c is None else c.shape[1], C_, B, _ptr(xscale), _ptr(xshift), _ptr(out), dtype_code(x), _stream()),
          "lmv_token_mean2_affine_fwd")
    return out


def token_mean2_bwd(g: Tensor, L: int, M: int) -> Tuple[Tensor, Optional[Tensor]]:
    B, C_ = g.shape
    dx = torch.empty((B, L, C_), device=g.device, dtype=g.dtype)
    dc = torch.empty((B, M, C_), device=g.device, dtype=g.dtype) if M else None
    check(lib.lmv_token_mean2_bwd(_ptr(g), _ptr(dx), L, _ptr(dc), M, C_, B, dtype_code(g), _stream()), "lmv_token_mean2_bwd")
    return dx, dc


def row_scale(x: Tensor, scale: Tensor, rows_per_sample: int) -> Tensor:
    y = torch.empty_like(x)
    C_ = x.shape[-1]
    check(lib.lmv_row_scale(_ptr(x), _f32(scale), _ptr(y), x.numel() // C_, C_, rows_per_sample, dtype_code(x), _stream()), "lmv_row_scale")
    return y


def row_scale_multi(xs: Sequence[Tensor], scales: Sequence[Optional[Tensor]]) -> List[Tensor]:
    todo = [(x, s) for x, s in zip(xs, scales) if s is not None]
    if not todo:
        return list(xs)
    if len(todo) > 2 or len({x.shape[-1] for x, _ in todo}) != 1 or len({x.dtype for x, _ in todo}) != 1:
        return [x if s is None else row_scale(x, s, x.shape[1]) for x, s in zip(xs, scales)]
    from ._lib import RowScaleSegment
    arr = (RowScaleSegment * len(todo))()
    outs = []
    for seg, (x, s) in zip(arr, todo):
        y = torch.empty_like(x)
        seg.x, seg.scale, seg.y = _ptr(x), _f32(s), _ptr(y)
        seg.rows, seg.rows_per_sample = x.numel() // x.shape[-1], x.shape[1]
        outs.append(y)
    check(lib.lmv_row_scale_multi(arr, len(todo), todo[0][0].shape[-1], dtype_code(todo[0][0]), _stream()), "lmv_row_scale_multi")
    it = iter(outs)
    return [x if s is None else next(it) for x, s in zip(xs, scales)]


def transpose_batch(pairs: Sequence[Tuple[Tensor, Tensor]]) -> None:
    if not pairs:
        return
    arr = (_lib.TransposeSeg * len(pairs))()
    for sg, (src, dst) in zip(arr, pairs):
        if src.dtype != torch.bfloat16 or dst.dtype != torch.bfloat16 or src.dim() != 2 or dst.shape != (src.shape[1], src.shape[0]) \
                or not src.is_contiguous() or not dst.is_contiguous():
            raise TypeError("transpose_batch: contiguous bfloat16 [R, C] -> [C, R] pairs")
        sg.src, sg.dst, sg.rows, sg.cols = _ptr(src), _ptr(dst), src.shape[0], src.shape[1]
    check(lib.lmv_transpose_batch(arr, len(pairs), _lib.LMV_BF16, _stream()), "lmv_transpose_batch")


def adamw_flat(param: Tensor, grad: Tensor, exp_avg: Tensor, exp_avg_sq: Tensor, wd_mask: Optional[Tensor], lr: float, beta1: float,
               beta2: float, eps: float, weight_decay: float, step: int, shadow: Optional[Tensor] = None, step_dev: Optional[Tensor] = None,
               stat: Optional[Tensor] = None, clip_value: float = 0.0) -> None:
    if shadow is not None and (shadow.dtype != torch.bfloat16 or shadow.numel() != param.numel()):
        raise TypeError("adamw_flat: shadow must be a bfloat16 tensor of the parameter buffer's length")
    if step_dev is not None and step_dev.dtype != torch.int32:
        raise TypeError("adamw_flat: step_dev must be an int32 device scalar")
    if stat is not None or clip_value:
        if stat is not None and (stat.dtype != torch.float32 or stat.numel() < GRAD_STAT_FLOATS):
            raise TypeError(f"adamw_flat: stat must be a float32 tensor of {GRAD_STAT_FLOATS} elements")
        check(lib.lmv_adamw_flat_clip(_f32(param), _f32(grad), _f32(exp_avg), _f32(exp_avg_sq), _f32(wd_mask), _ptr(shadow), param.numel(), lr, beta1, beta2, eps,
                                      weight_decay, step, _ptr(step_dev), _ptr(stat), float(clip_value), _stream()), "lmv_adamw_flat_clip")
        return
    check(lib.lmv_adamw_flat(_f32(param), _f32(grad), _f32(exp_avg), _f32(exp_avg_sq), _f32(wd_mask), _ptr(shadow), param.numel(), lr, beta1, beta2, eps,
                             weight_decay, step, _ptr(step_dev), _stream()), "lmv_adamw_flat")


def adamw_flat_groups(param: Tensor, grad: Tensor, exp_avg: Tensor, exp_avg_sq: Tensor, group_of_unit: Tensor, groups: Tensor, beta1: float, beta2: float,
                      eps: float, step: int, shadow: Optional[Tensor] = None, step_dev: Optional[Tensor] = None, stat: Optional[Tensor] = None,
                      clip_value: float = 0.0) -> None:
    n = param.numel()
    if n % ADAMW_UNIT:
        raise ValueError(f"adamw_flat_groups: the buffer length {n} must be a multiple of {ADAMW_UNIT}")
    if group_of_unit.dtype != torch.uint8 or group_of_unit.numel() != n // ADAMW_UNIT:
        raise TypeError(f"adamw_flat_groups: group_of_unit must be a uint8 tensor of n / {ADAMW_UNIT} = {n // ADAMW_UNIT} elements")
    if groups.dtype != torch.float32 or groups.dim() != 2 or groups.shape[1] != 2 or not 1 <= groups.shape[0] <= ADAMW_MAX_GROUPS:
        raise TypeError(f"adamw_flat_groups: groups must be a float32 tensor [G, 2] (lr, weight_decay) with 1 <= G <= {ADAMW_MAX_GROUPS}")
    if any(t.numel() != n for t in (grad, exp_avg, exp_avg_sq)):
        raise TypeError("adamw_flat_groups: grad, exp_avg and exp_avg_sq must have the parameter buffer's length")
    if shadow is not None and (shadow.dtype != torch.bfloat16 or shadow.numel() != n):
        raise TypeError("adamw_flat_groups: shadow must be a bfloat16 tensor of the parameter buffer's length")
    if step_dev is not None and step_dev.dtype != torch.int32:
        raise TypeError("adamw_flat_groups: step_dev must be an int32 device scalar")
    if stat is not None and (stat.dtype != torch.float32 or stat.numel() < GRAD_STAT_FLOATS):
        raise TypeError(f"adamw_flat_groups: stat must be a float32 tensor of {GRAD_STAT_FLOATS} elements")
    check(lib.lmv_adamw_flat_groups(_f32(param), _f32(grad), _f32(exp_avg), _f32(exp_avg_sq), _ptr(shadow), n, _ptr(group_of_unit), _ptr(groups),
                                    groups.shape[0], beta1, beta2, eps, step, _ptr(step_dev), _ptr(stat), float(clip_value), _stream()), "lmv_adamw_flat_groups")


GRAD_STAT_FLOATS = _lib.GRAD_STAT_FLOATS
ADAMW_UNIT, ADAMW_MAX_GROUPS = _lib.ADAMW_UNIT, _lib.ADAMW_MAX_GROUPS
NORM_CHUNK = _lib.NORM_CHUNK


def grad_norm(segments: Sequence[Tensor], max_norm: float, stat: Tensor, skip_nonfinite: bool = False, step_dev: Optional[Tensor] = None) -> Tensor:
    if stat.dtype != torch.float32 or stat.numel() != GRAD_STAT_FLOATS:
        raise TypeError(f"grad_norm: stat must be a float32 tensor of {GRAD_STAT_FLOATS} elements")
    if step_dev is not None and step_dev.dtype != torch.int32:
        raise TypeError("grad_norm: step_dev must be an int32 device scalar")
    if not segments:
        raise ValueError("grad_norm: no segments")
    arr = (_lib.NormSeg * len(segments))()
    for sg, t in zip(arr, segments):
        sg.ptr, sg.n = _f32(t), t.numel()
    ws = _workspace(int(lib.lmv_grad_norm_workspace_bytes(arr, len(arr))), stat.device)
    check(lib.lmv_grad_norm(arr, len(arr), float(max_norm), _lib.NORM_SKIP_NONFINITE if skip_nonfinite else 0, _ptr(stat), _ptr(step_dev), _ptr(ws),
                            ws.numel(), _stream()), "lmv_grad_norm")
    return stat


def ema_flat(ema: Tensor, param: Tensor, decay: float) -> None:
    if ema.dtype != torch.float32 or param.dtype != torch.float32 or ema.numel() != param.numel():
        raise TypeError("lemevit_amd: ema_flat takes two fp32 buffers of the same length")
    check(lib.lmv_ema_flat(_ptr(ema), _ptr(param), ema.numel(), float(decay), _stream()), "lmv_ema_flat")


MIX_RECORD_WORDS = C.sizeof(_lib.MixRecord) // 4


def _mix_table(table: Tensor, B: int, fn: str) -> int:
    if table.dtype != torch.int32 or table.dim() != 2 or tuple(table.shape) != (B, MIX_RECORD_WORDS):
        raise TypeError(f"{fn}: table must be an int32 tensor [{B}, {MIX_RECORD_WORDS}] (lemevit_amd.recipe.pack_records), got {tuple(table.shape)} {table.dtype}")
    return _ptr(table)


def mix_images(x: Tensor, table: Tensor, out_dtype: Optional[torch.dtype] = None, scale: Optional[Tensor] = None, shift: Optional[Tensor] = None,
               records: Optional[Tensor] = None) -> Tensor:
    if x.dim() != 4:
        raise ValueError(f"mix_images: [B, C, H, W] images expected, got {tuple(x.shape)}")
    if not x.is_cuda:
        raise RuntimeError("lemevit_amd: tensors must be on the GPU (no CPU fallback exists)")
    codes = {torch.float32: _lib.LMV_F32, torch.bfloat16: _lib.LMV_BF16, torch.uint8: _lib.LMV_U8}
    if x.dtype not in codes:
        raise TypeError(f"mix_images: unsupported image dtype {x.dtype} (uint8, float32 and bfloat16 only)")
    if out_dtype is None:
        out_dtype = torch.float32 if x.dtype == torch.uint8 else x.dtype
    if out_dtype not in (torch.float32, torch.bfloat16):
        raise TypeError(f"mix_images: unsupported output dtype {out_dtype} (float32 and bfloat16 only)")
    B, C_, H, W = x.shape
    if (scale is None) != (shift is None):
        raise ValueError("mix_images: scale and shift come together")
    if scale is not None and (scale.numel() != C_ or shift.numel() != C_):
        raise ValueError(f"mix_images: scale and shift must have one element per channel ({C_})")
    tp = _mix_table(table, B, "mix_images")
    hp = None
    if records is not None:
        if records.is_cuda or not records.is_contiguous() or records.dtype != torch.int32 or tuple(records.shape) != (B, MIX_RECORD_WORDS):
            raise TypeError(f"mix_images: records must be a contiguous int32 CPU tensor [{B}, {MIX_RECORD_WORDS}]")
        hp = records.data_ptr()
    out = torch.empty((B, C_, H, W), device=x.device, dtype=out_dtype)
    sb, sc, sh, sw = x.stride()
    check(lib.lmv_mix_images(x.data_ptr(), codes[x.dtype], sb, sc, sh, sw, _ptr(out), codes[out_dtype], B, C_, H, W, tp, hp, _f32(scale), _f32(shift), _stream()),
          "lmv_mix_images")
    return out


def soft_ce(logits: Tensor, labels: Optional[Tensor] = None, table: Optional[Tensor] = None, smoothing: float = 0.0, target: Optional[Tensor] = None,
            want_grad: bool = True) -> Tuple[Tensor, Tensor, Optional[Tensor]]:
    if logits.dim() != 2:
        raise ValueError(f"soft_ce: [B, N] logits expected, got {tuple(logits.shape)}")
    if not logits.is_cuda:
        raise RuntimeError("lemevit_amd: tensors must be on the GPU (no CPU fallback exists)")
    code = dtype_code(logits)
    B, N = logits.shape
    if N > 1 and logits.stride(1) != 1:
        raise ValueError("soft_ce: the logits must have unit stride along the classes")
    ls = logits.stride(0) if B > 1 else N
    if ls < N:
        raise ValueError("soft_ce: overlapping logit rows")
    if (labels is None) == (target is None):
        raise ValueError("soft_ce: exactly one of labels (sparse form) and target (dense form) must be given")
    lp = tp = gp = None
    tcode, ts = 0, 0
    if labels is not None:
        if labels.dtype != torch.int64 or tuple(labels.shape) != (B,):
            raise TypeError(f"soft_ce: labels must be an int64 tensor [{B}], got {tuple(labels.shape)} {labels.dtype}")
        if not 0.0 <= float(smoothing) < 1.0:
            raise ValueError("soft_ce: smoothing must be in [0, 1)")
        lp = _ptr(labels)
        if table is not None:
            tp = _mix_table(table, B, "soft_ce")
    else:
        if table is not None:
            raise ValueError("soft_ce: the table belongs to the sparse form")
        if tuple(target.shape) != (B, N) or (N > 1 and target.stride(1) != 1) or not target.is_cuda:
            raise ValueError(f"soft_ce: target must be a [{B}, {N}] GPU tensor with unit stride along the classes")
        tcode, ts, gp = dtype_code(target), (target.stride(0) if B > 1 else N), target.data_ptr()
    row = torch.empty((B,), device=logits.device, dtype=torch.float32)
    loss = torch.empty((), device=logits.device, dtype=torch.float32)
    dlog = torch.empty((B, N), device=logits.device, dtype=logits.dtype) if want_grad else None
    check(lib.lmv_soft_ce(logits.data_ptr(), code, ls, B, N, lp, tp, float(smoothing), gp, tcode, ts, _ptr(row), _ptr(loss), _ptr(dlog), _stream()), "lmv_soft_ce")
# ... 237 lines not shown
```

Baseline: 4323 images/sec.

## Fuse stage-transition downsample conv+BN with meta-token MLP and batch weight derivation

Adds a native transition op that runs the stride-2 conv downsample with training BatchNorm and the meta-token MLP in one fwd/bwd call, using auxiliary streams so the two branches can overlap. Also batches the per-step fp32-to-bf16 weight casts and conv-matrix repacks for non-block weights into a single kernel launch. The aim is fewer launches and less serialization at the stage transitions, at the cost of a large new code path with its own BN running-stat and gradient handling.

```diff
diff --git a/include/lemevit_hip.h b/include/lemevit_hip.h
--- a/include/lemevit_hip.h
+++ b/include/lemevit_hip.h
@@ -181,6 +181,10 @@
 #define LMV_TRANSPOSE_MAX_SEGS 48
 typedef struct { const void* src; void* dst; int32_t rows, cols; } lmv_transpose_seg;
 int lmv_transpose_batch(const lmv_transpose_seg* segs, int nsegs, int dtype, void* stream);
+#define LMV_DERIVE_MAX_RECS 16
+enum { LMV_DERIVE_CAST = 0, LMV_DERIVE_CONV_MATRIX = 1 };
+typedef struct lmv_derive_rec { const float* src; void* dst; int64_t n; int32_t kind, dst_dtype, Co, Ci, KP, _pad; } lmv_derive_rec;
+int lmv_derive_batch(const lmv_derive_rec* recs, int nrecs, void* stream);
 int lmv_im2col3x3s2_nhwc(const void* x, void* patches, int B, int H, int W, int C, int KP, int dtype, void* stream);
 int lmv_col2im3x3s2_nhwc(const void* dpatches, void* dx, int B, int H, int W, int C, int KP, int dtype, void* stream);
 int lmv_conv3x3s2_fwd(const void* x, const void* wm, const float* bias, void* y, int B, int H, int W, int Cin, int Cout, int KP, int act, int dtype, void* stream);
@@ -253,6 +257,30 @@
                                 int image0, int nimages, void* scratch, size_t scratch_bytes, void* stream);
 long long lmv_debug_wgrad_launches(void);
 
+typedef struct lmv_transition_desc {
+  int32_t dtype, B, H, W, Cin, Cout, KP;
+  int32_t implicit, gelu;
+  int32_t rows_c, c_in, c_hid, c_out;
+  float momentum, bn_eps, eps1, eps2;
+  const void* x; const void* wm; const float* conv_b;
+  void* patches;
+  void* y_conv;
+  const float* bn_w; const float* bn_b; float* running_mean; float* running_var;
+  float* bn_stats;
+  void* y;
+  const void* c; const void* w1; const float* b1; const float* g1; const float* be1; const void* w2; const float* b2; const float* g2; const float* be2;
+  void* h1; float* st1; void* a1; void* h2; float* st2;
+  void* c_y;
+  const void* dy; const void* dc_y;
+  void* dx; void* dc;
+  float* g_wm; float* g_conv_b; float* g_bn_w; float* g_bn_b;
+  float* g_w1; float* g_b1; float* g_g1; float* g_be1; float* g_w2; float* g_b2; float* g_g2; float* g_be2;
+} lmv_transition_desc;
+size_t lmv_transition_fwd_workspace_bytes(const lmv_transition_desc* d);
+size_t lmv_transition_bwd_workspace_bytes(const lmv_transition_desc* d);
+int lmv_transition_fwd(const lmv_transition_desc* d, void* workspace, size_t workspace_bytes, void* stream, void* aux_stream);
+int lmv_transition_bwd(const lmv_transition_desc* d, void* workspace, size_t workspace_bytes, void* stream, void* aux_stream0, void* aux_stream1);
+
 typedef struct lmv_sstage_block_params {
   int32_t C, heads, hidden, _pad;
   const void* qkv_w; const void* proj_w; const void* fc1_w; const void* fc2_w;
diff --git a/lemevit_amd/_lib.py b/lemevit_amd/_lib.py
--- a/lemevit_amd/_lib.py
+++ b/lemevit_amd/_lib.py
@@ -11,6 +11,7 @@
 LMV_F32, LMV_BF16, LMV_U8 = 0, 1, 2
 ACT_NONE, ACT_GELU, ACT_GELU_GRAD, ACT_GELU_BWD = 0, 1, 2, 3
 FOLD_CI_TAP, FOLD_TAP_CI = 0, 1
+DERIVE_CAST, DERIVE_CONV_MATRIX = 0, 1
 ABI_VERSION = 14
 BLOCK_NO_JOIN, BLOCK_FUSED, BLOCK_DATA_ONLY = 1, 2, 4
 GRAD_STAT_FLOATS, NORM_CHUNK, NORM_SKIP_NONFINITE = 8, 16384, 1
@@ -68,6 +69,15 @@
                 [(n, C.c_void_p) for n in ("fold_fc1_w", "fold_fc1_s", "fold_fc1_b", "fc2_wt", "fc1_wt")] + [("attn_wt", C.c_void_p * 2)])
 
 
+class TransitionDesc(C.Structure):
+    _fields_ = ([(n, C.c_int32) for n in ("dtype", "B", "H", "W", "Cin", "Cout", "KP", "implicit", "gelu", "rows_c", "c_in", "c_hid", "c_out")] +
+                [(n, C.c_float) for n in ("momentum", "bn_eps", "eps1", "eps2")] +
+                [(n, C.c_void_p) for n in ("x", "wm", "conv_b", "patches", "y_conv", "bn_w", "bn_b", "running_mean", "running_var", "bn_stats", "y",
+                                           "c", "w1", "b1", "g1", "be1", "w2", "b2", "g2", "be2", "h1", "st1", "a1", "h2", "st2", "c_y",
+                                           "dy", "dc_y", "dx", "dc", "g_wm", "g_conv_b", "g_bn_w", "g_bn_b",
+                                           "g_w1", "g_b1", "g_g1", "g_be1", "g_w2", "g_b2", "g_g2", "g_be2")])
+
+
 class SStageBlockParams(C.Structure):
     _fields_ = ([(n, C.c_int32) for n in ("C", "heads", "hidden", "_pad")] +
                 [(n, C.c_void_p) for n in ("qkv_w", "proj_w", "fc1_w", "fc2_w", "n1_w", "n1_b", "qkv_b", "proj_b", "n2_w", "n2_b", "fc1_b", "fc2_b", "pos_w", "pos_b")])
@@ -85,6 +95,10 @@
 
 class TransposeSeg(C.Structure):
     _fields_ = [("src", C.c_void_p), ("dst", C.c_void_p), ("rows", C.c_int32), ("cols", C.c_int32)]
+
+
+class DeriveRec(C.Structure):
+    _fields_ = [("src", C.c_void_p), ("dst", C.c_void_p), ("n", C.c_int64)] + [(n, C.c_int32) for n in ("kind", "dst_dtype", "Co", "Ci", "KP", "_pad")]
 
 
 class NormSeg(C.Structure):
@@ -185,6 +199,11 @@
     "lmv_block_fwd_scratch_bytes": (_Z, [C.POINTER(BlockDesc)]),
     "lmv_block_fwd_range_scratch": (_I, [C.POINTER(BlockDesc), _P, _P, _P, _P, _P, _Z, _I, _I, _I, _P, _Z, _P]),
     "lmv_debug_wgrad_launches": (C.c_longlong, []),
+    "lmv_derive_batch": (_I, [C.POINTER(DeriveRec), _I, _P]),
+    "lmv_transition_fwd_workspace_bytes": (_Z, [C.POINTER(TransitionDesc)]),
+    "lmv_transition_bwd_workspace_bytes": (_Z, [C.POINTER(TransitionDesc)]),
+    "lmv_transition_fwd": (_I, [C.POINTER(TransitionDesc), _P, _Z, _P, _P]),
+    "lmv_transition_bwd": (_I, [C.POINTER(TransitionDesc), _P, _Z, _P, _P, _P]),
     "lmv_sstage_supported": (_I, [_I, _I, _I, _I, _I, _I, _I]),
     "lmv_sstage_wpk_bytes": (_Z, [_I, _I]),
     "lmv_sstage_vec_floats": (_Z, [_I, _I]),
diff --git a/lemevit_amd/csrc/block.hip b/lemevit_amd/csrc/block.hip
--- a/lemevit_amd/csrc/block.hip
+++ b/lemevit_amd/csrc/block.hip
@@ -1,17 +1,7 @@
 #include <math.h>
-#include <mutex>
-#include "common.h"
+#include "side.h"
 
 namespace {
-
-struct Bump {
-  unsigned char* base; size_t off, cap;
-  void* take(size_t n) {
-    const size_t a = (off + 255) & ~(size_t)255;
-    off = a + n;
-    return base ? (void*)(base + a) : (void*)(uintptr_t)256;
-  }
-};
 
 struct Dims {
   int kind, dtype, B, H, W, N, M, C, Hd, heads;
@@ -114,14 +104,6 @@
   a->dq = (unsigned char*)dq + qo * D.es; a->dk = (unsigned char*)dk + ko * D.es; a->dv = (unsigned char*)dv + vo * D.es;
 }
 
-lmv_linear_problem prob(const void* a, const void* w, void* out, int64_t rows) {
-  lmv_linear_problem p{};
-  p.a = a; p.w = w; p.out = out; p.rows = rows;
-  return p;
-}
-
-#define LMV_TRY(expr) do { const int rc__ = (expr); if (rc__) return rc__; } while (0)
-
 const float SDPA_SCALE = 0.17677669529663687f;
 inline void dca_scales(const Dims& D, float* sx, float* sc) {
   const double base = pow((double)D.C, -0.5);
@@ -177,63 +159,6 @@
   }
   return lmv_linear_fwd(p, ns, D.C, D.Hd, LMV_ACT_NONE, D.dtype, st);
 }
-
-struct Side {
-  hipStream_t main, side; hipEvent_t fork, join; bool used;
-  void* ws; size_t ws_bytes;
-  void* ws_tail; size_t ws_tail_bytes;
-  lmv_reduce_seg segs[LMV_REDUCE_MAX_SEGS]; int nsegs = 0;
-  bool dataonly = false;
-  hipStream_t begin() {
-    if (!side) return main;
-    lmv_count_wgrad();
-    (void)hipEventRecord(fork, main);
-    (void)hipStreamWaitEvent(side, fork, 0);
-    used = true;
-    return side;
-  }
-  void finish() {
-    if (side && used) { (void)hipEventRecord(join, side); (void)hipStreamWaitEvent(main, join, 0); used = false; }
-  }
-};
-
-struct EventPool {
-  std::mutex mu;
-  hipEvent_t free_ev[64][32];
-  int nfree[64] = {};
-  int take(hipEvent_t* fork, hipEvent_t* join) {
-    int dev = 0;
-    (void)hipGetDevice(&dev);
-    dev &= 63;
-    hipEvent_t out[2];
-    int got = 0;
-    {
-      std::lock_guard<std::mutex> lk(mu);
-      while (got < 2 && nfree[dev] > 0) out[got++] = free_ev[dev][--nfree[dev]];
-    }
-    for (; got < 2; ++got)
-      if (hipEventCreateWithFlags(&out[got], hipEventDisableTiming) != hipSuccess) {
-        give(dev, out, got);
-        LMV_FAIL(LMV_ERR_LAUNCH, "block_bwd: cannot create stream events");
-      }
-    *fork = out[0]; *join = out[1];
-    return LMV_OK;
-  }
-  void give(int dev, const hipEvent_t* ev, int n) {
-    std::lock_guard<std::mutex> lk(mu);
-    for (int i = 0; i < n; ++i) {
-      if (nfree[dev] < 32) free_ev[dev][nfree[dev]++] = ev[i];
-      else (void)hipEventDestroy(ev[i]);
-    }
-  }
-  void give(hipEvent_t fork, hipEvent_t join) {
-    int dev = 0;
-    (void)hipGetDevice(&dev);
-    const hipEvent_t ev[2] = {fork, join};
-    give(dev & 63, ev, 2);
-  }
-};
-EventPool& event_pool() { static EventPool p; return p; }
 
 int dw(Side& sd, const lmv_linear_problem* p, int np, int N, int K, int dtype) {
   lmv_count_wgrad();
@@ -589,7 +514,7 @@
   sd.main = (hipStream_t)stream; sd.side = (hipStream_t)side_stream; sd.ws = b.ws_side; sd.ws_bytes = b.ws_side_bytes;
   sd.ws_tail = b.ws_conv; sd.ws_tail_bytes = b.ws_conv_bytes;
   sd.dataonly = dataonly;
-  if (side_stream) LMV_TRY(event_pool().take(&sd.fork, &sd.join));
+  if (side_stream) LMV_TRY(lmv_event_pool().take(&sd.fork, &sd.join));
   hipStream_t st = sd.main;
   const int C = D.C, N = D.N, M = D.M;
   lmv_linear_problem p[2];
@@ -700,6 +625,6 @@
   };
   rc = body();
   if (rc || !(d->flags & LMV_BLOCK_NO_JOIN)) sd.finish();
-  if (side_stream) event_pool().give(sd.fork, sd.join);
+  if (side_stream) lmv_event_pool().give(sd.fork, sd.join);
   return rc;
 }
diff --git a/lemevit_amd/csrc/misc.hip b/lemevit_amd/csrc/misc.hip
--- a/lemevit_amd/csrc/misc.hip
+++ b/lemevit_amd/csrc/misc.hip
@@ -827,3 +827,59 @@
   LMV_CHECK_LAUNCH("transpose_batch");
   return LMV_OK;
 }
+
+namespace {
+struct DeriveRecDev { const float* src; void* dst; int64_t n; int kind, bf16, Ci, KP, blk0; };
+struct DeriveBatch { DeriveRecDev r[LMV_DERIVE_MAX_RECS]; int n; };
+__global__ __launch_bounds__(TPB) void derive_batch_kernel(const DeriveBatch tb) {
+  int ri = 0;
+#pragma unroll 1
+  for (int k = 1; k < tb.n; ++k) if ((int)blockIdx.x >= tb.r[k].blk0) ri = k;
+  const DeriveRecDev g = tb.r[ri];
+  const int nblk = (ri + 1 < tb.n ? tb.r[ri + 1].blk0 : (int)gridDim.x) - g.blk0;
+  for (int64_t i = (int64_t)(blockIdx.x - g.blk0) * TPB + threadIdx.x; i < g.n; i += (int64_t)nblk * TPB) {
+    float v;
+    if (g.kind == LMV_DERIVE_CAST) {
+      v = g.src[i];
+    } else {
+      const int64_t co = i / g.KP;
+      const int col = (int)(i - co * g.KP);
+      const int tap = col / g.Ci, ci = col - tap * g.Ci;
+      v = tap < 9 ? g.src[(co * g.Ci + ci) * 9 + tap] : 0.f;
+    }
+    if (g.bf16) ((bf16_t*)g.dst)[i] = f2bf(v);
+    else ((float*)g.dst)[i] = v;
+  }
+}
+}
+extern "C" int lmv_derive_batch(const lmv_derive_rec* recs, int nrecs, void* stream) {
+  if (nrecs <= 0) return LMV_OK;
+  if (!recs) LMV_FAIL(LMV_ERR_SHAPE, "derive_batch: recs is NULL");
+  for (int i = 0; i < nrecs; ++i) {
+    const lmv_derive_rec& q = recs[i];
+    if (!q.src || !q.dst || q.src == q.dst || (q.dst_dtype != LMV_F32 && q.dst_dtype != LMV_BF16)) LMV_FAIL(LMV_ERR_SHAPE, "derive_batch: bad record %d (null pointer / dtype)", i);
+    if (q.kind == LMV_DERIVE_CAST) {
+      if (q.n <= 0) LMV_FAIL(LMV_ERR_SHAPE, "derive_batch: record %d: n = %lld", i, (long long)q.n);
+    } else if (q.kind == LMV_DERIVE_CONV_MATRIX) {
+      if (q.Co <= 0 || q.Ci <= 0 || q.KP < 9 * q.Ci || (int64_t)q.Co * q.KP >= (1LL << 31)) LMV_FAIL(LMV_ERR_SHAPE, "derive_batch: record %d: Co=%d Ci=%d KP=%d", i, q.Co, q.Ci, q.KP);
+    } else LMV_FAIL(LMV_ERR_SHAPE, "derive_batch: record %d: kind %d", i, q.kind);
+  }
+  hipStream_t st = (hipStream_t)stream;
+  for (int r0 = 0; r0 < nrecs; r0 += LMV_DERIVE_MAX_RECS) {
+    DeriveBatch tb{};
+    tb.n = nrecs - r0 < LMV_DERIVE_MAX_RECS ? nrecs - r0 : LMV_DERIVE_MAX_RECS;
+    int blocks = 0;
+    for (int i = 0; i < tb.n; ++i) {
+      const lmv_derive_rec& q = recs[r0 + i];
+      DeriveRecDev& d = tb.r[i];
+      d.src = q.src; d.dst = q.dst; d.kind = q.kind; d.bf16 = q.dst_dtype == LMV_BF16; d.Ci = q.Ci; d.KP = q.KP;
+      d.n = q.kind == LMV_DERIVE_CAST ? q.n : (int64_t)q.Co * q.KP;
+      d.blk0 = blocks;
+      int64_t b = (d.n + 4 * TPB - 1) / (4 * TPB);
+      blocks += (int)(b > 256 ? 256 : b);
+    }
+    hipLaunchKernelGGL(derive_batch_kernel, dim3(blocks), dim3(TPB), 0, st, tb);
+  }
+  LMV_CHECK_LAUNCH("derive_batch");
+  return LMV_OK;
+}
diff --git a/lemevit_amd/csrc/side.h b/lemevit_amd/csrc/side.h
--- /dev/null
+++ b/lemevit_amd/csrc/side.h
@@ -0,0 +1,84 @@
+#pragma once
+#include <mutex>
+#include "common.h"
+
+#ifndef LMV_TRY
+#define LMV_TRY(expr) do { const int rc__ = (expr); if (rc__) return rc__; } while (0)
+#endif
+
+struct LmvEventPool {
+  std::mutex mu;
+  hipEvent_t free_ev[64][32];
+  int nfree[64] = {};
+  int take(hipEvent_t* fork, hipEvent_t* join) {
+    int dev = 0;
+    (void)hipGetDevice(&dev);
+    dev &= 63;
+    hipEvent_t out[2];
+    int got = 0;
+    {
+      std::lock_guard<std::mutex> lk(mu);
+      while (got < 2 && nfree[dev] > 0) out[got++] = free_ev[dev][--nfree[dev]];
+    }
+    for (; got < 2; ++got)
+      if (hipEventCreateWithFlags(&out[got], hipEventDisableTiming) != hipSuccess) {
+        give(dev, out, got);
+        LMV_FAIL(LMV_ERR_LAUNCH, "cannot create stream events");
+      }
+    *fork = out[0]; *join = out[1];
+    return LMV_OK;
+  }
+  void give(int dev, const hipEvent_t* ev, int n) {
+    std::lock_guard<std::mutex> lk(mu);
+    for (int i = 0; i < n; ++i) {
+      if (nfree[dev] < 32) free_ev[dev][nfree[dev]++] = ev[i];
+      else (void)hipEventDestroy(ev[i]);
+    }
+  }
+  void give(hipEvent_t fork, hipEvent_t join) {
+    int dev = 0;
+    (void)hipGetDevice(&dev);
+    const hipEvent_t ev[2] = {fork, join};
+    give(dev & 63, ev, 2);
+  }
+};
+inline LmvEventPool& lmv_event_pool() { static LmvEventPool p; return p; }
+
+namespace {
+
+struct Bump {
+  unsigned char* base; size_t off, cap;
+  void* take(size_t n) {
+    const size_t a = (off + 255) & ~(size_t)255;
+    off = a + n;
+    return base ? (void*)(base + a) : (void*)(uintptr_t)256;
+  }
+};
+
+inline lmv_linear_problem prob(const void* a, const void* w, void* out, int64_t rows) {
+  lmv_linear_problem p{};
+  p.a = a; p.w = w; p.out = out; p.rows = rows;
+  return p;
+}
+
+struct Side {
+  hipStream_t main, side; hipEvent_t fork, join; bool used;
+  void* ws; size_t ws_bytes;
+  void* ws_tail; size_t ws_tail_bytes;
+  lmv_reduce_seg segs[LMV_REDUCE_MAX_SEGS]; int nsegs = 0;
+  bool dataonly = false;
+  bool counted = true;
+  hipStream_t begin() {
+    if (!side) return main;
+    if (counted) lmv_count_wgrad();
+    (void)hipEventRecord(fork, main);
+    (void)hipStreamWaitEvent(side, fork, 0);
+    used = true;
+    return side;
+  }
+  void finish() {
+    if (side && used) { (void)hipEventRecord(join, side); (void)hipStreamWaitEvent(main, join, 0); used = false; }
+  }
+};
+
+}
diff --git a/lemevit_amd/csrc/transition.hip b/lemevit_amd/csrc/transition.hip
--- /dev/null
+++ b/lemevit_amd/csrc/transition.hip
@@ -0,0 +1,240 @@
+#include "side.h"
+
+namespace {
+
+struct TDims {
+  bool conv, meta;
+  int dtype; size_t es;
+  int Ho, Wo; int64_t rows;
+  int64_t R;
+};
+
+struct TBwdWs { void *bn, *dxbn, *dp, *cdw, *dh2, *da1, *dh1, *mws; size_t bn_b, cdw_b, mws_b; };
+
+inline bool ok16(const void* p) { return p && lmv_aligned16(p); }
+inline bool ok16n(const void* p) { return lmv_aligned16(p); }
+
+int tdims(const lmv_transition_desc* d, TDims* o, const char* who) {
+  if (!d) LMV_FAIL(LMV_ERR_SHAPE, "%s: null descriptor", who);
+  if (d->dtype != LMV_F32 && d->dtype != LMV_BF16) LMV_FAIL(LMV_ERR_DTYPE, "%s: unsupported dtype %d", who, d->dtype);
+  o->dtype = d->dtype; o->es = d->dtype == LMV_BF16 ? 2 : 4;
+  o->conv = d->Cout != 0; o->meta = d->rows_c != 0;
+  o->Ho = o->Wo = 0; o->rows = 0; o->R = d->rows_c;
+  if (!o->conv && !o->meta) LMV_FAIL(LMV_ERR_SHAPE, "%s: neither a convolution nor a meta-token part", who);
+  if (o->conv) {
+    if (d->B <= 0 || d->H <= 0 || d->W <= 0 || d->Cin <= 0 || d->Cout <= 0 || (d->Cin % 8) || (d->Cout % 8) || d->KP < 9 * d->Cin || (d->KP % 4))
+      LMV_FAIL(LMV_ERR_SHAPE, "%s: bad convolution dims B=%d H=%d W=%d Cin=%d Cout=%d KP=%d", who, d->B, d->H, d->W, d->Cin, d->Cout, d->KP);
+    if (d->implicit && (d->dtype != LMV_BF16 || (d->KP % 64))) LMV_FAIL(LMV_ERR_SHAPE, "%s: the implicit convolution is bf16 with KP a multiple of 64", who);
+    o->Ho = (d->H + 1) / 2; o->Wo = (d->W + 1) / 2; o->rows = (int64_t)d->B * o->Ho * o->Wo;
+    if (d->implicit && (o->rows % 64)) LMV_FAIL(LMV_ERR_SHAPE, "%s: the implicit convolution takes B Ho Wo a multiple of 64", who);
+    if (o->rows < 2) LMV_FAIL(LMV_ERR_SHAPE, "%s: BatchNorm over one value per channel", who);
+  }
+  if (o->meta && (d->rows_c < 0 || d->c_in <= 0 || d->c_hid <= 0 || d->c_out <= 0 || (d->c_in % 8) || (d->c_hid % 8) || (d->c_out % 8)))
+    LMV_FAIL(LMV_ERR_SHAPE, "%s: bad meta-token dims rows=%d %d -> %d -> %d", who, d->rows_c, d->c_in, d->c_hid, d->c_out);
+  return LMV_OK;
+}
+
+int check_fwd_ptrs(const lmv_transition_desc* d, const TDims& D, const char* who) {
+  if (D.conv) {
+    if (!ok16(d->x) || !ok16(d->wm) || !ok16n(d->conv_b) || !ok16(d->y_conv) || !ok16(d->bn_w) || !ok16(d->bn_b) || !ok16n(d->running_mean) || !ok16n(d->running_var) ||
+        !ok16(d->bn_stats) || !ok16(d->y) || (!d->implicit && !ok16(d->patches)))
+      LMV_FAIL(LMV_ERR_SHAPE, "%s: null / misaligned convolution or BatchNorm operand", who);
+  }
+  if (D.meta) {
+    if (!ok16(d->c) || !ok16(d->w1) || !ok16(d->b1) || !ok16(d->g1) || !ok16(d->be1) || !ok16(d->w2) || !ok16(d->b2) || !ok16(d->g2) || !ok16(d->be2) || !ok16(d->h1) ||
+        !ok16(d->st1) || !ok16(d->a1) || !ok16(d->h2) || !ok16(d->st2) || !ok16(d->c_y))
+      LMV_FAIL(LMV_ERR_SHAPE, "%s: null / misaligned meta-token operand", who);
+  }
+  return LMV_OK;
+}
+
+int check_bwd_ptrs(const lmv_transition_desc* d, const TDims& D, const char* who) {
+  if (D.conv) {
+    if (!ok16(d->wm) || !ok16(d->y_conv) || !ok16(d->bn_w) || !ok16(d->bn_b) || !ok16(d->bn_stats) || !ok16(d->dy) || !ok16(d->g_bn_w) || !ok16(d->g_bn_b) || !ok16n(d->dx) ||
+        !ok16(d->implicit ? d->x : d->patches))
+      LMV_FAIL(LMV_ERR_SHAPE, "%s: null / misaligned convolution or BatchNorm operand", who);
+    if ((d->g_wm == nullptr) != (d->g_conv_b == nullptr) || !ok16n(d->g_wm) || !ok16n(d->g_conv_b))
+      LMV_FAIL(LMV_ERR_SHAPE, "%s: g_wm and g_conv_b go together (both NULL: a frozen convolution), 16-byte aligned", who);
+  }
+  if (D.meta) {
+    if (!ok16(d->c) || !ok16(d->w1) || !ok16(d->g1) || !ok16(d->be1) || !ok16(d->w2) || !ok16(d->g2) || !ok16(d->h1) || !ok16(d->st1) || !ok16(d->a1) || !ok16(d->h2) ||
+        !ok16(d->st2) || !ok16(d->dc_y) || !ok16n(d->dc))
+      LMV_FAIL(LMV_ERR_SHAPE, "%s: null / misaligned meta-token operand", who);
+    const float* pairs[4][2] = {{d->g_w1, d->g_b1}, {d->g_g1, d->g_be1}, {d->g_w2, d->g_b2}, {d->g_g2, d->g_be2}};
+    for (auto& pr : pairs)
+      if ((pr[0] == nullptr) != (pr[1] == nullptr) || !ok16n(pr[0]) || !ok16n(pr[1]))
+        LMV_FAIL(LMV_ERR_SHAPE, "%s: the meta-token accumulators come in pairs (both NULL: frozen), 16-byte aligned", who);
+  }
+  return LMV_OK;
+}
+
+size_t dw_ws(int64_t rows, int N, int K, int dtype) {
+  lmv_linear_problem p{};
+  p.a = p.w = p.out = (void*)16; p.bias_grad = (float*)16; p.rows = rows;
+  return lmv_linear_dw_workspace_bytes(&p, 1, N, K, dtype);
+}
+
+void layout_bwd(const lmv_transition_desc* d, const TDims& D, Bump& a, TBwdWs* w) {
+  *w = TBwdWs{};
+  if (D.conv) {
+    w->bn_b = lmv_batchnorm_workspace_bytes(d->Cout); w->bn = a.take(w->bn_b);
+    w->dxbn = a.take((size_t)D.rows * d->Cout * D.es);
+    w->dp = d->dx ? a.take((size_t)D.rows * d->KP * D.es) : nullptr;
+    if (d->g_wm) {
+      w->cdw_b = d->implicit ? lmv_conv3x3s2_dw_workspace_bytes(d->B, d->H, d->W, d->Cin, d->Cout, d->KP, d->dtype) : dw_ws(D.rows, d->Cout, d->KP, d->dtype);
+      if (w->cdw_b < 256) w->cdw_b = 256;
+      w->cdw = a.take(w->cdw_b);
+    }
+  }
+  if (D.meta) {
+    w->dh2 = a.take((size_t)D.R * d->c_out * D.es);
+    w->da1 = a.take((size_t)D.R * d->c_hid * D.es);
+    w->dh1 = a.take((size_t)D.R * d->c_hid * D.es);
+    size_t m = 256, t;
+    if (d->g_g2 && (t = lmv_layernorm_bwd_workspace_bytes(D.R, d->c_out, d->dtype)) > m) m = t;
+    if (d->g_g1 && (t = lmv_layernorm_bwd_workspace_bytes(D.R, d->c_hid, d->dtype)) > m) m = t;
+    if (d->g_w2 && (t = dw_ws(D.R, d->c_out, d->c_hid, d->dtype)) > m) m = t;
+    if (d->g_w1 && (t = dw_ws(D.R, d->c_hid, d->c_in, d->dtype)) > m) m = t;
+    w->mws_b = m; w->mws = a.take(m);
+  }
+}
+
+int conv_bn_fwd(const lmv_transition_desc* d, const TDims& D, void* bn_ws, size_t bn_ws_bytes, hipStream_t st) {
+  if (d->implicit) {
+    LMV_TRY(lmv_conv3x3s2_fwd(d->x, d->wm, d->conv_b, d->y_conv, d->B, d->H, d->W, d->Cin, d->Cout, d->KP, LMV_ACT_NONE, d->dtype, st));
+  } else {
+    LMV_TRY(lmv_im2col3x3s2_nhwc(d->x, d->patches, d->B, d->H, d->W, d->Cin, d->KP, d->dtype, st));
+    lmv_linear_problem p = prob(d->patches, d->wm, d->y_conv, D.rows); p.bias = d->conv_b;
+    LMV_TRY(lmv_linear_fwd(&p, 1, d->Cout, d->KP, LMV_ACT_NONE, d->dtype, st));
+  }
+  return lmv_batchnorm_train_fwd(d->y_conv, d->bn_w, d->bn_b, d->running_mean, d->running_var, d->momentum, d->bn_eps, d->gelu ? LMV_ACT_GELU : LMV_ACT_NONE, d->y,
+                                 d->bn_stats, D.rows, d->Cout, bn_ws, bn_ws_bytes, d->dtype, st);
+}
+
+int meta_fwd(const lmv_transition_desc* d, const TDims& D, hipStream_t st) {
+  lmv_linear_problem p = prob(d->c, d->w1, d->h1, D.R); p.bias = d->b1;
+  LMV_TRY(lmv_linear_fwd(&p, 1, d->c_hid, d->c_in, LMV_ACT_NONE, d->dtype, st));
+  lmv_ln_segment seg{};
+  seg.x = d->h1; seg.y = d->a1; seg.stats = d->st1; seg.rows = D.R;
+  LMV_TRY(lmv_layernorm_gelu_fwd(&seg, 1, d->g1, d->be1, d->c_hid, d->eps1, d->dtype, st));
+  p = prob(d->a1, d->w2, d->h2, D.R); p.bias = d->b2;
+  LMV_TRY(lmv_linear_fwd(&p, 1, d->c_out, d->c_hid, LMV_ACT_NONE, d->dtype, st));
+  seg = lmv_ln_segment{};
+  seg.x = d->h2; seg.y = d->c_y; seg.stats = d->st2; seg.rows = D.R;
+  return lmv_layernorm_fwd(&seg, 1, d->g2, d->be2, d->c_out, d->eps2, d->dtype, st);
+}
+
+int meta_bwd(const lmv_transition_desc* d, const TDims& D, const TBwdWs& w, hipStream_t st) {
+  lmv_ln_segment seg{};
+  seg.x = d->h2; seg.dy = d->dc_y; seg.stats = d->st2; seg.dx = w.dh2; seg.rows = D.R;
+  if (d->g_g2) LMV_TRY(lmv_layernorm_bwd(&seg, 1, d->g2, d->g_g2, d->g_be2, d->c_out, w.mws, w.mws_b, d->dtype, st));
+  else LMV_TRY(lmv_layernorm_bwd_partial(&seg, 1, d->g2, d->c_out, nullptr, 0, nullptr, d->dtype, st));
+  lmv_linear_problem p;
+  if (d->g_w2) {
+    p = prob(w.dh2, d->a1, d->g_w2, D.R); p.bias_grad = d->g_b2;
+    LMV_TRY(lmv_linear_dw(&p, 1, d->c_out, d->c_hid, w.mws, w.mws_b, d->dtype, st));
+  }
+  p = prob(w.dh2, d->w2, w.da1, D.R);
+  LMV_TRY(lmv_linear_dx(&p, 1, d->c_out, d->c_hid, LMV_ACT_NONE, d->dtype, st));
+  seg = lmv_ln_segment{};
+  seg.x = d->h1; seg.dy = w.da1; seg.stats = d->st1; seg.dx = w.dh1; seg.rows = D.R;
+  if (d->g_g1) LMV_TRY(lmv_layernorm_gelu_bwd(&seg, 1, d->g1, d->be1, d->g_g1, d->g_be1, d->c_hid, w.mws, w.mws_b, d->dtype, st));
+  else LMV_TRY(lmv_layernorm_gelu_bwd(&seg, 1, d->g1, d->be1, nullptr, nullptr, d->c_hid, nullptr, 0, d->dtype, st));
+  if (d->g_w1) {
+    p = prob(w.dh1, d->c, d->g_w1, D.R); p.bias_grad = d->g_b1;
+    LMV_TRY(lmv_linear_dw(&p, 1, d->c_hid, d->c_in, w.mws, w.mws_b, d->dtype, st));
+  }
+  if (d->dc) {
+    p = prob(w.dh1, d->w1, d->dc, D.R);
+    LMV_TRY(lmv_linear_dx(&p, 1, d->c_hid, d->c_in, LMV_ACT_NONE, d->dtype, st));
+  }
+  return LMV_OK;
+}
+
+struct Chain {
+  Side sd{};
+  bool have = false;
+  int open(hipStream_t main, hipStream_t aux) {
+    sd.main = main; sd.side = aux; sd.counted = false;
+    if (aux) { LMV_TRY(lmv_event_pool().take(&sd.fork, &sd.join)); have = true; }
+    return LMV_OK;
+  }
+  hipStream_t fork() { return sd.begin(); }
+  void join() { sd.finish(); }
+  void close() { if (have) { lmv_event_pool().give(sd.fork, sd.join); have = false; } }
+};
+
+}
+
+extern "C" size_t lmv_transition_fwd_workspace_bytes(const lmv_transition_desc* d) {
+  TDims D;
+  if (tdims(d, &D, "transition_fwd")) return 0;
+  const size_t w = D.conv ? lmv_batchnorm_workspace_bytes(d->Cout) : 0;
+  return w < 256 ? 256 : w;
+}
+
+extern "C" size_t lmv_transition_bwd_workspace_bytes(const lmv_transition_desc* d) {
+  TDims D;
+  if (tdims(d, &D, "transition_bwd")) return 0;
+  Bump a{nullptr, 0, 0};
+  TBwdWs w;
+  layout_bwd(d, D, a, &w);
+  return (a.off + 255) & ~(size_t)255;
+}
+
+extern "C" int lmv_transition_fwd(const lmv_transition_desc* d, void* workspace, size_t workspace_bytes, void* stream, void* aux_stream) {
+  TDims D;
+  LMV_TRY(tdims(d, &D, "transition_fwd"));
+  LMV_TRY(check_fwd_ptrs(d, D, "transition_fwd"));
+  const size_t need = lmv_transition_fwd_workspace_bytes(d);
+  if (!ok16(workspace) || workspace_bytes < need) LMV_FAIL(LMV_ERR_WORKSPACE, "transition_fwd: workspace %zu < %zu bytes (or null / misaligned)", workspace_bytes, need);
+  hipStream_t st = (hipStream_t)stream;
+  Chain mc;
+  LMV_TRY(mc.open(st, D.conv && D.meta ? (hipStream_t)aux_stream : nullptr));
+  int rc = LMV_OK;
+  if (D.meta) rc = meta_fwd(d, D, mc.fork());
+  if (!rc && D.conv) rc = conv_bn_fwd(d, D, workspace, workspace_bytes, st);
+  mc.join();
+  mc.close();
+  return rc;
+}
+
+extern "C" int lmv_transition_bwd(const lmv_transition_desc* d, void* workspace, size_t workspace_bytes, void* stream, void* aux_stream0, void* aux_stream1) {
+  TDims D;
+  LMV_TRY(tdims(d, &D, "transition_bwd"));
+  LMV_TRY(check_bwd_ptrs(d, D, "transition_bwd"));
+  const size_t need = lmv_transition_bwd_workspace_bytes(d);
+  if (!ok16(workspace) || workspace_bytes < need) LMV_FAIL(LMV_ERR_WORKSPACE, "transition_bwd: workspace %zu < %zu bytes (or null / misaligned)", workspace_bytes, need);
+  Bump a{(unsigned char*)workspace, 0, workspace_bytes};
+  TBwdWs w;
+  layout_bwd(d, D, a, &w);
+  hipStream_t st = (hipStream_t)stream;
+  Chain mc, wc;
+  LMV_TRY(mc.open(st, D.conv && D.meta ? (hipStream_t)aux_stream1 : nullptr));
+  if (int rc0 = wc.open(st, D.conv && d->g_wm ? (hipStream_t)aux_stream0 : nullptr)) { mc.close(); return rc0; }
+  auto body = [&]() -> int {
+    if (D.meta) LMV_TRY(meta_bwd(d, D, w, mc.fork()));
+    if (!D.conv) return LMV_OK;
+    LMV_TRY(lmv_batchnorm_train_bwd(d->dy, d->y_conv, d->bn_w, d->bn_b, d->bn_stats, d->gelu ? LMV_ACT_GELU : LMV_ACT_NONE, w.dxbn, d->g_bn_w, d->g_bn_b, D.rows, d->Cout,
+                                    w.bn, w.bn_b, d->dtype, st));
+    if (d->g_wm) {
+      hipStream_t ws = wc.fork();
+      if (d->implicit) {
+        LMV_TRY(lmv_conv3x3s2_dw(w.dxbn, d->x, d->g_wm, d->g_conv_b, d->B, d->H, d->W, d->Cin, d->Cout, d->KP, w.cdw, w.cdw_b, d->dtype, ws));
+      } else {
+        lmv_linear_problem p = prob(w.dxbn, d->patches, d->g_wm, D.rows); p.bias_grad = d->g_conv_b;
+        LMV_TRY(lmv_linear_dw(&p, 1, d->Cout, d->KP, w.cdw, w.cdw_b, d->dtype, ws));
+      }
+    }
+    if (d->dx) {
+      lmv_linear_problem p = prob(w.dxbn, d->wm, w.dp, D.rows);
+      LMV_TRY(lmv_linear_dx(&p, 1, d->Cout, d->KP, LMV_ACT_NONE, d->dtype, st));
+      LMV_TRY(lmv_col2im3x3s2_nhwc(w.dp, d->dx, d->B, d->H, d->W, d->Cin, d->KP, d->dtype, st));
+    }
+    return LMV_OK;
+  };
+  const int rc = body();
+  wc.join(); mc.join();
+  wc.close(); mc.close();
+  return rc;
+}
diff --git a/lemevit_amd/model.py b/lemevit_amd/model.py
--- a/lemevit_amd/model.py
+++ b/lemevit_amd/model.py
@@ -420,6 +420,212 @@
             dc = dx.view(cshape).to(cdtype)
         ctx.saved = None
         return (dc, *[None if not nd else (g if dt == torch.float32 else g.to(dt)) for g, (_, dt), nd in zip(G, pmeta, need)], None, None, None)
+
+
+_TRANSITION = os.environ.get("LMV_TRANSITION", "1") != "0"
+
+
+def _transition_streams(dev, n: int) -> list:
+    from . import blocks as _blocks
+    from .blocks import aux_streams
+    if not _blocks._SIDE or torch.cuda.is_current_stream_capturing():
+        return [None] * n
+    return [s.cuda_stream for s in aux_streams(dev, n)]
+
+
+class _TransitionFn(torch.autograd.Function):
+
+    @staticmethod
+    def forward(ctx, x, c, conv_w, conv_b, bn_w, bn_b, w1, b1, g1, be1, w2, b2, g2, be2, bn, gelu, eps1, eps2, cd):
+        from ._lib import TransitionDesc, check, lib
+        f32 = lambda p: compute_copy(p, torch.float32)
+        d = TransitionDesc()
+        d.dtype = _lib_dtype(cd)
+        dev = (x if x is not None else c).device
+        keep, y, cy = [], None, None
+        ctx.conv = ctx.metashape = None
+        if x is not None:
+            B, Ci, H, W = x.shape
+            Co = conv_w.shape[0]
+            xh = x.detach().permute(0, 2, 3, 1).to(cd).contiguous()
+            KP = (9 * Ci + 63) // 64 * 64 if cd == torch.bfloat16 else 9 * Ci
+            Wm = _conv_matrix(conv_w, cd, KP)
+            cb32 = None if conv_b is None else f32(conv_b)
+            implicit = _CONV_IMPLICIT and ops.conv3x3s2_implicit_ok(xh, Co, KP)
+            Ho, Wo = (H + 1) // 2, (W + 1) // 2
+            rows = B * Ho * Wo
+            yc = torch.empty(rows, Co, device=dev, dtype=cd)
+            y = torch.empty_like(yc)
+            stats = torch.empty((2, Co), device=dev, dtype=torch.float32)
+            patches = None if implicit else torch.empty(rows, KP, device=dev, dtype=cd)
+            gb, bb = f32(bn_w), f32(bn_b)
+            if bn.num_batches_tracked is not None:
+                bn.num_batches_tracked.add_(1)
+            d.B, d.H, d.W, d.Cin, d.Cout, d.KP, d.implicit, d.gelu = B, H, W, Ci, Co, KP, int(implicit), int(gelu)
+            d.momentum, d.bn_eps = float(bn.momentum), float(bn.eps)
+            d.x, d.wm, d.conv_b, d.patches, d.y_conv = ops._ptr(xh), ops._ptr(Wm), ops._f32(cb32), ops._ptr(patches), ops._ptr(yc)
+            d.bn_w, d.bn_b, d.running_mean, d.running_var = ops._f32(gb), ops._f32(bb), ops._f32(bn.running_mean), ops._f32(bn.running_var)
+            d.bn_stats, d.y = ops._f32(stats), ops._ptr(y)
+            keep += [xh, Wm, cb32, patches, yc, gb, bb, stats]
+            ctx.conv = (tuple(x.shape), x.dtype, conv_w.dtype, None if conv_b is None else conv_b.dtype, bn_w.dtype, bn_b.dtype)
+        if c is not None:
+            cin, hid, cout = w1.shape[1], w1.shape[0], w2.shape[0]
+            xc = c.detach().to(cd).contiguous().view(-1, cin)
+            R = xc.shape[0]
+            W1, W2 = compute_copy(w1, cd), compute_copy(w2, cd)
+            vec = [f32(p) for p in (b1, g1, be1, b2, g2, be2)]
+            h1 = torch.empty(R, hid, device=dev, dtype=cd)
+            a1 = torch.empty_like(h1)
+            st1 = torch.empty((R, 2), device=dev, dtype=torch.float32)
+            h2 = torch.empty(R, cout, device=dev, dtype=cd)
+            cy = torch.empty_like(h2)
+            st2 = torch.empty((R, 2), device=dev, dtype=torch.float32)
+            d.rows_c, d.c_in, d.c_hid, d.c_out, d.eps1, d.eps2 = R, cin, hid, cout, float(eps1), float(eps2)
+            d.c, d.w1, d.w2 = ops._ptr(xc), ops._ptr(W1), ops._ptr(W2)
+            d.b1, d.g1, d.be1, d.b2, d.g2, d.be2 = (ops._f32(v) for v in vec)
+            d.h1, d.st1, d.a1, d.h2, d.st2, d.c_y = ops._ptr(h1), ops._f32(st1), ops._ptr(a1), ops._ptr(h2), ops._f32(st2), ops._ptr(cy)
+            keep += [xc, W1, W2, *vec, h1, st1, a1, h2, st2]
+            ctx.metashape = (c.shape, c.dtype, [(p.shape, p.dtype) for p in (w1, b1, g1, be1, w2, b2, g2, be2)])
+        ws = torch.empty(int(lib.lmv_transition_fwd_workspace_bytes(d)), device=dev, dtype=torch.uint8)
+        (aux,) = _transition_streams(dev, 1) if (x is not None and c is not None) else (None,)
+        check(lib.lmv_transition_fwd(d, ws.data_ptr(), ws.numel(), ops._stream(), aux), "lmv_transition_fwd")
+        ctx.d, ctx.keep = d, keep
+        if y is not None:
+            y = y.view(B, Ho, Wo, Co).permute(0, 3, 1, 2)
+        if cy is not None:
+            cy = cy.view(c.shape[:-1] + (cout,))
+        return y, cy
+
+    @staticmethod
+    def backward(ctx, dy, dcy):
+        from ._lib import check, lib
+        d, keep = ctx.d, ctx.keep
+        need = ctx.needs_input_grad
+        dev = keep[0].device
+        cd = keep[0].dtype
+        grads = [None] * 19
+        hold = []
+        sizes = {}
+        if ctx.conv is not None:
+            (B, Ci, H, W), xdt, wdt, bdt, gdt, bedt = ctx.conv
+            Co, KP = d.Cout, d.KP
+            need_w, need_b = need[2], bdt is not None and need[3]
+            if need_w or need_b:
+                sizes["wm"], sizes["cb"] = Co * KP, Co
+            sizes["bn_w"], sizes["bn_b"] = Co, Co
+        if ctx.metashape is not None:
+            cshape, cdtype, pmeta = ctx.metashape
+            mneed = need[6:14]
+            pairs = [any(mneed[i:i + 2]) for i in (0, 2, 4, 6)]
+            for i, (sh, _) in enumerate(pmeta):
+                if pairs[i // 2]:
+                    sizes[i] = int(torch.Size(sh).numel())
+        offs, total = {}, 0
+        for k, n in sizes.items():
+            offs[k] = total
+            total += (n + 3) // 4 * 4
+        flat = torch.zeros(total, device=dev, dtype=torch.float32)
+        G = {k: flat[offs[k]:offs[k] + n] for k, n in sizes.items()}
+        dx = dc = None
+        if ctx.conv is not None:
+            if dy is None:
+                dy = torch.zeros((B, Co, (H + 1) // 2, (W + 1) // 2), device=dev, dtype=cd)
+            g = dy.permute(0, 2, 3, 1).contiguous().view(-1, Co)
+            if g.dtype != cd:
+                g = g.to(cd)
+            if need[0]:
+                dx = torch.empty((B, H, W, Ci), device=dev, dtype=cd)
+            d.dy, d.dx = ops._ptr(g), ops._ptr(dx)
+            d.g_wm, d.g_conv_b = ops._f32(G.get("wm")), ops._f32(G.get("cb"))
+            d.g_bn_w, d.g_bn_b = ops._f32(G["bn_w"]), ops._f32(G["bn_b"])
+            hold += [g, dx]
+        if ctx.metashape is not None:
+            xc = keep[-14]
+            cout = d.c_out
+            if dcy is None:
+                dcy = torch.zeros((xc.shape[0], cout), device=dev, dtype=cd)
+            gc = dcy.contiguous().view(-1, cout)
+            if gc.dtype != cd:
+                gc = gc.to(cd)
+            if need[1]:
+                dc = torch.empty_like(xc)
+            d.dc_y, d.dc = ops._ptr(gc), ops._ptr(dc)
+            d.g_w1, d.g_b1, d.g_g1, d.g_be1, d.g_w2, d.g_b2, d.g_g2, d.g_be2 = (ops._f32(G.get(i)) for i in range(8))
+            hold += [gc, dc]
+        ws = torch.empty(int(lib.lmv_transition_bwd_workspace_bytes(d)), device=dev, dtype=torch.uint8)
+        aux0, aux1 = _transition_streams(dev, 2)
+        check(lib.lmv_transition_bwd(d, ws.data_ptr(), ws.numel(), ops._stream(), aux0, aux1), "lmv_transition_bwd")
+        if ctx.conv is not None:
+            if dx is not None:
+                grads[0] = dx.permute(0, 3, 1, 2).to(xdt)
+            if need_w:
+                grads[2] = G["wm"].view(Co, KP)[:, :9 * Ci].reshape(Co, 3, 3, Ci).permute(0, 3, 1, 2).to(wdt)
+            if need_b:
+                grads[3] = G["cb"].to(bdt)
+            grads[4], grads[5] = G["bn_w"].to(gdt) if need[4] else None, G["bn_b"].to(bedt) if need[5] else None
+        if ctx.metashape is not None:
+            if dc is not None:
+                grads[1] = dc.view(cshape).to(cdtype)
+            for i, ((sh, dt), nd) in enumerate(zip(pmeta, mneed)):
+                if nd:
+                    gi = G[i].view(sh)
+                    grads[6 + i] = gi if dt == torch.float32 else gi.to(dt)
+        return tuple(grads)
+
+
+def _lib_dtype(cd: torch.dtype) -> int:
+    from . import _lib
+    return _lib.LMV_BF16 if cd == torch.bfloat16 else _lib.LMV_F32
+
+
+def _bn_native_on(m: nn.Module, C: int, rows: int, cd: torch.dtype) -> bool:
+    return (isinstance(m, nn.BatchNorm2d) and m.training and m.affine and m.track_running_stats and m.momentum is not None and cd in (torch.float32, torch.bfloat16)
+            and C % 8 == 0 and C <= 1024 and rows > 1 and m.weight.dtype == torch.float32 and m.num_features == C)
+
+
+def _transition_parts(seq: nn.Module, x: Tensor, cd: torch.dtype):
+    if not isinstance(seq, nn.Sequential) or len(seq) not in (2, 5) or not x.is_cuda or cd not in (torch.float32, torch.bfloat16):
+        return None
+    mods = list(seq)
+    conv, bn = mods[-2], mods[-1]
+    if not (isinstance(conv, nn.Conv2d) and isinstance(bn, nn.BatchNorm2d)):
+        return None
+    if len(mods) == 5:
+        c1 = mods[0]
+        if not (_is_stem_conv1(c1, x) and isinstance(mods[1], nn.BatchNorm2d) and isinstance(mods[2], nn.GELU)):
+            return None
+        B, _, H, W = x.shape
+        shape = (B, c1.out_channels, (H + 1) // 2, (W + 1) // 2)
+    else:
+        shape = tuple(x.shape)
+    probe = torch.empty(shape, device="meta", dtype=cd)
+    B, Ci, H, W = shape
+    rows = B * ((H + 1) // 2) * ((W + 1) // 2)
+    if not (conv.in_channels == Ci and isinstance(conv, nn.Conv2d) and conv.kernel_size == (3, 3) and conv.stride == (2, 2) and conv.padding == (1, 1)
+            and conv.dilation == (1, 1) and conv.groups == 1 and conv.in_channels % 8 == 0 and conv.out_channels % 8 == 0 and conv.padding_mode == "zeros"
+            and probe.dtype in (torch.float32, torch.bfloat16) and conv.weight.dtype in (torch.float32, torch.bfloat16)):
+        return None
+    if not _bn_native_on(bn, conv.out_channels, rows, cd) or bn.bias.dtype != torch.float32:
+        return None
+    return mods[:-2], conv, bn
+
+
+def _transition_apply(seq: Optional[nn.Module], mlp: nn.Module, x: Optional[Tensor], c: Tensor, cd: torch.dtype):
+    if not _TRANSITION or not torch.is_grad_enabled() or not _is_meta_mlp(mlp, c, cd):
+        return None
+    l1, n1, _, l2, n2 = mlp
+    margs = (l1.weight, l1.bias, n1.weight, n1.bias, l2.weight, l2.bias, n2.weight, n2.bias)
+    if seq is None:
+        return _TransitionFn.apply(None, c, None, None, None, None, *margs, None, False, n1.eps, n2.eps, cd)
+    if (x.dtype if not torch.is_autocast_enabled() else torch.get_autocast_dtype("cuda")) != cd:
+        return None
+    parts = _transition_parts(seq, x, cd)
+    if parts is None:
+        return None
+    pre, conv, bn = parts
+    if pre:
+        x = _downsample_mods(pre, x, cd, False)
+    return _TransitionFn.apply(x, c, conv.weight, conv.bias, bn.weight, bn.bias, *margs, bn, False, n1.eps, n2.eps, cd)
 
 
 class _TailFn(torch.autograd.Function):
@@ -1716,6 +1922,8 @@
         B = x.shape[0]
         if torch.is_grad_enabled():
             new_training_pass()
+            if _TRANSITION and x.is_cuda and cd in (torch.float32, torch.bfloat16):
+                self._derive_nonblock(cd, head)
         hoist = c is None
         if hoist:
             c = self.meta_tokens.unsqueeze(0)
@@ -1730,6 +1938,42 @@
             self.__dict__.setdefault("_whole_seen", {})[st["key"]] = tuple(st["whole"])
         return out
 
+    def _derive_nonblock(self, cd: torch.dtype, head) -> None:
+        recs = []
+
+        def conv_matrix(w: Tensor, KP: int):
+            def build():
+                m = torch.empty(w.shape[0], KP, device=w.device, dtype=cd)
+                recs.append((w.detach(), m, "conv"))
+                return m
+            derived(w, ("conv", cd, KP), (w,), build)
+
+        def cast(p: Tensor):
+            shadow = getattr(p, "_lmv_shadow", None)
+            if p.dtype != torch.float32 or not p.is_cuda or (shadow is not None and shadow.dtype == cd and shadow.device == p.device):
+                return
+
+            def build():
+                t = torch.empty(p.shape, device=p.device, dtype=cd)
+                recs.append((p.detach().contiguous(), t))
+                return t
+            derived(p, ("cast", cd), (p,), build)
+
+        with torch.no_grad():
+            for seq in self.downsample_layers:
+                for m in (seq if isinstance(seq, nn.Sequential) else ()):
+                    if (isinstance(m, nn.Conv2d) and m.kernel_size == (3, 3) and m.in_channels % 8 == 0 and m.weight.dtype == torch.float32 and m.weight.is_cuda
+                            and m.weight.is_contiguous()):
+                        Ci = m.in_channels
+                        conv_matrix(m.weight, (9 * Ci + 63) // 64 * 64 if cd == torch.bfloat16 else 9 * Ci)
+            if cd != torch.float32:
+                for mlp in self.meta_token_downsample:
+                    if _is_meta_mlp(mlp, self.meta_tokens, cd):
+                        cast(mlp[0].weight); cast(mlp[3].weight)
+                if isinstance(head, nn.Linear):
+                    cast(head.weight)
+            ops.derive_batch(recs)
+
     def _meta_tokens_for(self, i: int, c: Tensor, hoist: bool, B: int, cd: torch.dtype) -> Tensor:
         mlp = self.meta_token_downsample[i]
         if hoist and not torch.is_grad_enabled() and not self.training:
@@ -1739,6 +1983,12 @@
         if hoist:
             c = c.expand(B, -1, -1)
         return c.to(cd).contiguous()
+
+    def _transition_node(self, i: int, down: bool, x: Optional[Tensor], xt: Optional[Tensor], H: int, W: int, c: Tensor, cd: torch.dtype, st: dict):
+        if st["infer"] or _map_pass.rec is not None or getattr(self, "grad_checkpointing", False):
+            return None
+        xin = None if not down else (x if xt is None else self._to_nchw(xt, H, W))
+        return _transition_apply(self.downsample_layers[i] if down else None, self.meta_token_downsample[i], xin, c, cd)
 
     def _stages_from(self, i0: int, x: Optional[Tensor], xt: Optional[Tensor], H: int, W: int, c: Tensor, hoist: bool, st: dict) -> Tensor:
         cd, head = st["cd"], st["head"]
@@ -1761,6 +2011,13 @@
                 xt, H, W = self._to_tokens(x, cd)
                 cur.wait_stream(side)
                 c.record_stream(cur)
+            elif (node := self._transition_node(i, down, x, xt, H, W, c, cd, st)) is not None:
+                x, c = node
+                if down:
+                    xt, H, W = self._to_tokens(x, cd)
+                if hoist:
+                    c = c.expand(B, -1, -1)
+                c = c.to(cd).contiguous()
             else:
                 if down:
                     x = self._run_downsample(self.downsample_layers[i], x if xt is None else self._to_nchw(xt, H, W))
diff --git a/lemevit_amd/ops.py b/lemevit_amd/ops.py
--- a/lemevit_amd/ops.py
+++ b/lemevit_amd/ops.py
@@ -593,6 +593,26 @@
     return [x if s is None else next(it) for x, s in zip(xs, scales)]
 
 
+def derive_batch(recs) -> None:
+    if not recs:
+        return
+    arr = (_lib.DeriveRec * len(recs))()
+    for r, (src, dst, *kind) in zip(arr, recs):
+        if src.dtype != torch.float32:
+            raise TypeError("derive_batch: fp32 sources")
+        r.src, r.dst, r.dst_dtype = _ptr(src), _ptr(dst), dtype_code(dst)
+        if kind:
+            Co, Ci = src.shape[0], src.shape[1]
+            if tuple(src.shape[2:]) != (3, 3) or dst.dim() != 2 or dst.shape[0] != Co:
+                raise ValueError(f"derive_batch: conv weight {tuple(src.shape)} -> {tuple(dst.shape)}")
+            r.kind, r.Co, r.Ci, r.KP = _lib.DERIVE_CONV_MATRIX, Co, Ci, dst.shape[1]
+        else:
+            if src.numel() != dst.numel():
+                raise ValueError("derive_batch: a cast keeps the number of elements")
+            r.kind, r.n = _lib.DERIVE_CAST, src.numel()
+    check(lib.lmv_derive_batch(arr, len(recs), _stream()), "lmv_derive_batch")
+
+
 def transpose_batch(pairs: Sequence[Tuple[Tensor, Tensor]]) -> None:
     if not pairs:
         return
```

After: 4304 images/sec. No clear change (-0.4%).
